# LANL-Bioinformatics/PCRamp

Measured on AMD Instinct MI355X. Metric: primer-pair x target amplification evals/sec, higher is better.
Workload: dtype u32

## Files before the change

pcramp_amd/csrc/pcr_device.hip:

```cpp
#include <hip/hip_runtime.h>
#include <cstring>
#include <rocprim/device/device_radix_sort.hpp>

#include <stdint.h>
#include <string.h>
#include <math.h>
#include <stdlib.h>
#include <string>
#include <vector>
#include <chrono>
#include <algorithm>
#include <unordered_map>
#include <type_traits>
#include <thread>
#include <mutex>
#include <condition_variable>
#include <functional>
#include <memory>
#include <atomic>
#include <cassert>
#include <sched.h>
#include <pthread.h>

#include "../../include/pcramp_hip.h"
// ... 450 lines not shown
	const uint32_t n = min(seq_count[seq], cap);
	uint32_t np2 = 1; while(np2 < n) np2 <<= 1;
	for(uint32_t i = tid;i < np2;i += FINBIG_THREADS){
		uint64_t k = ~0ull;
		if(i < n){
			const Hit h = hits[(size_t)seq*cap + i];
			if constexpr (ALL) k = h.key;
			else if(((epoch << 8) | h.cnt) == best[(size_t)seq*ncand + h.cand]) k = h.key;
		}
		fin_keys[i] = k;
	}
	__syncthreads();
	for(uint32_t k = 2;k <= np2;k <<= 1){
		for(uint32_t j = k >> 1;j > 0;j >>= 1){
			for(uint32_t i = tid;i < np2;i += FINBIG_THREADS){
				const uint32_t l = i ^ j;
				if(l > i){
					const uint64_t a = fin_keys[i], b = fin_keys[l];
					const bool up = ((i & k) == 0);
					if((a > b) == up){ fin_keys[i] = b; fin_keys[l] = a; }
				}
			}
			__syncthreads();
		}
	}
	const uint32_t chunk = (np2 + FINBIG_THREADS - 1)/FINBIG_THREADS;
	const uint32_t lo = min(np2, tid*chunk), hi = min(np2, lo + chunk);
	uint32_t cnt = 0;
	for(uint32_t i = lo;i < hi;++i){
		const uint64_t k = fin_keys[i];
		if(k != ~0ull && (i == 0 || fin_keys[i - 1] != k)) ++cnt;
	}
	part[tid] = cnt;
	__syncthreads();
	if(tid == 0){
		uint32_t run = 0;
		for(int t = 0;t < FINBIG_THREADS;++t){ const uint32_t c = part[t]; part[t] = run; run += c; }
		seg_hi[seq] = seq*cap + run;
	}
	__syncthreads();
	uint32_t rank = part[tid];
	for(uint32_t i = lo;i < hi;++i){
		const uint64_t k = fin_keys[i];
		if(k != ~0ull && (i == 0 || fin_keys[i - 1] != k)){
			DevEntry e;
			materialise_entry(k, planes, blk_off, irr, irr_off, e);
			db[(size_t)seq*cap + rank] = e;
			++rank;
		}
	}
}

#include "pcr_screen.inc"

#include "pcr_sw.inc"
#include "pcr_thermo.inc"

constexpr uint32_t N_TOUCHED_UNKNOWN = 0xFFFFFFFFu;
constexpr uint32_t EPOCH_LIMIT = (1u << 24) - 1;

struct SeqSet {
	uint32_t n = 0;
	std::vector<std::vector<uint8_t> > packed;
	std::vector<uint64_t> len, blk_off, nblk_real;
	std::vector<float> weight; DevBuf<float> d_weight; bool weight_dirty = true;
	std::vector<uint8_t> active;
	std::vector<std::vector<pcrhost::IrrEntry> > irr_host;
	uint64_t total_blocks = 0;
	uint32_t n_tiles = 0, n_irr = 0;
	bool ctrl_clean = false;
	bool touched_from_seg = false;
	uint32_t bucket_cap = 64;
	DevBuf<uint32_t> irr_perm; uint32_t irr_size_count[256];
	DevBuf<uint4> planes;
	DevBuf<uint32_t> valid, nib, tb, blk_seq, tile_seq, tile_pos0, irr_off, degen_tiles;
	uint32_t *valid_d() const { return valid.p + S2_VALID_FRONT; }
	uint32_t *tb_d() const { return tb.p + S2_TB_FRONT; }
	DevBuf<uint8_t> tile_degen; uint32_t n_degen_tiles = 0;
	DevBuf<TileDesc> tile_desc;
	DevBuf<uint64_t> d_len, d_blk_off, d_nblk_real;
	DevBuf<uint8_t> d_active;
	std::vector<uint8_t> has_eos; DevBuf<uint8_t> d_has_eos;
	DevBuf<IrrDev> irr;
	DevBuf<IrrScan> irr_scan;
	DevBuf<uint32_t> irx_first, irx_last, irx_words, irx_sums; bool irx_valid = false, irx_usable = false;
	uint32_t irr_n_multi = 0;
	DevBuf<uint32_t> pix_first, pix_last, pix_sums, blk_info, blk_local, blk_tile0; DevBuf<uint4> pix_ent; std::vector<uint32_t> pix_start_h; uint64_t pix_generation = 0; bool pix_valid = false, pix_usable = false;
	DevBuf<uint8_t> codes; DevBuf<uint64_t> d_code_off; bool have_codes = false;
	bool have_db = false;
	uint32_t n_entries = 0;
	uint32_t db_cap = 0;
	uint64_t n_slots = 0;
	DevBuf<DevEntry> db;
	DevBuf<uint32_t> touched;
	DevBuf<uint32_t> ctrl;
	uint32_t n_touched = 0;
	bool touched_built = false;
	uint32_t *d_seg_hi = nullptr;
};

}

struct HostPool {
	std::vector<std::thread> th;
	std::mutex m; std::condition_variable cv_go, cv_done;
	std::function<void(unsigned)> fn; unsigned n_parts = 0, next = 0, pending = 0; uint64_t gen = 0; bool stop = false;
	explicit HostPool(unsigned n_workers){ for(unsigned i = 0;i < n_workers;++i) th.emplace_back([this]{ work(); }); }
	~HostPool(){ { std::lock_guard<std::mutex> lk(m); stop = true; } cv_go.notify_all(); for(std::thread &t : th) t.join(); }
	unsigned size() const { return (unsigned)th.size(); }
	void work()
	{
		uint64_t seen = 0;
		std::unique_lock<std::mutex> lk(m);
		while(true){
			cv_go.wait(lk, [&]{ return stop || gen != seen; });
			if(stop) return;
			seen = gen;
			while(next < n_parts){ const unsigned p = next++; lk.unlock(); fn(p); lk.lock(); }
			if(--pending == 0) cv_done.notify_one();
		}
	}
	void run(unsigned parts, std::function<void(unsigned)> f)
	{
		std::unique_lock<std::mutex> lk(m);
		fn = std::move(f); n_parts = parts; next = 0; pending = (unsigned)th.size(); ++gen;
		cv_go.notify_all();
		while(next < n_parts){ const unsigned p = next++; lk.unlock(); fn(p); lk.lock(); }
		cv_done.wait(lk, [&]{ return pending == 0; });
	}
};

namespace { struct PassJob; struct Launcher; }

struct pcr_ctx {
	int device = 0;
	std::unique_ptr<HostPool> pool_;
	HostPool &host_pool()
	{
		if(!pool_){ const unsigned hw = std::max(1u, std::thread::hardware_concurrency()); pool_.reset(new HostPool(std::min(hw, 16u) - 1u)); }
		return *pool_;
	}
	Stream stream;
	Stream aux_stream;
	std::string design_text;
	DevBuf<uint64_t> split_where;
	pcr_params params;
	pcrhost::PackFilter filt;
	SeqSet sets[PCR_N_SETS];
	DevBuf<uint32_t> best, counters, mask, status;
	int scan_version = 3;
	bool force_seed1 = false;
	struct S2Key { uint32_t a, c, g, t, floor_; bool operator==(const S2Key &o) const { return a == o.a && c == o.c && g == o.g && t == o.t && floor_ == o.floor_; } };
	struct S2KeyHash { size_t operator()(const S2Key &k) const { uint64_t h = 0x9E3779B97F4A7C15ull; for(uint32_t v : {k.a, k.c, k.g, k.t, k.floor_}){ h ^= v; h *= 0x100000001B3ull; h ^= h >> 29; } return (size_t)h; } };
	struct S2Entry { std::vector<uint32_t> seeds;  uint32_t off_mask; bool seedable; uint4 mask;  };
	std::unordered_map<S2Key, S2Entry, S2KeyHash> s2_cache;
	std::vector<pcrhost::Seed> s2_tmp;
	static constexpr int S3_CHUNK_SETS = 4;
	struct S3Chunks { uint64_t gen = 0; uint32_t total = 0; std::vector<uint32_t> run; };
	struct S3Entry : S2Entry { std::vector<uint8_t> spans;  S3Chunks chunks[S3_CHUNK_SETS]; uint32_t next_slot = 0; };
	std::unordered_map<S2Key, S3Entry, S2KeyHash> s3_cache;
	std::vector<pcrhost::FoldSeed> s3_tmp;
	struct S3Launch { Seed3Slices W; uint32_t n_chunks, per_wg, slice_cap, n_irr_wg; };
	bool no_seed3 = false, s3_attr_set = false;
	bool s3_next = true;
	bool s2_attr_set = false; uint32_t s2_dbg = 0; bool no_irr_index = false;
	std::unordered_map<S2Key, S2Entry, S2KeyHash> s1_cache;
	DevBuf<uint32_t> s1_image, s1_heads, s1_multi, s1_part;
	bool host_seed_tables = false;
	DevBuf<Hit> hits;
	DevBuf<uint64_t> bits_fr, bits_rf;
	DevBuf<OligoDev> oligos;
	DevBuf<SwJob> sw_jobs; DevBuf<SwOut> sw_out; DevBuf<uint8_t> sw_q, sw_qlen, sw_t, entry_codes, entry_lens;
	DevBuf<AmpRec> amp_recs, amp_recs2; DevBuf<BgPairDev> bg_pairs;
	DevBuf<uint64_t> amp_keys; DevBuf<uint32_t> amp_pkeys, amp_pair_start; DevBuf<uint8_t> sort_tmp;
	DevBuf<thermo::Job> th_jobs; DevBuf<thermo::JobOut> th_out; DevBuf<int> th_dg; DevBuf<uint2> th_map; DevBuf<uint32_t> th_bad;
	float th_dg_salt = -1.0f;
	DevBuf<unsigned long long> th_dbg; bool th_attr_set = false;
	std::vector<thermo::Job> th_host_jobs; std::vector<thermo::JobOut> th_host_res;
	MappedBuf<uint8_t> sw_pin; Event sw_done[2];
	DevBuf<pcr_amplicon> mx_amp;
	DevBuf<OligoDev> opt_oligos; DevBuf<uint2> opt_jobs; DevBuf<float> opt_cov; DevBuf<uint32_t> opt_loc, opt_tasks;
	DevBuf<Planes> mx_keys; uint32_t mx_n_keys = 0; DevBuf<uint32_t> mx_count;
	DevBuf<uint8_t> pool_in, pool_tmp; DevBuf<uint32_t> pool_cnt, pool_ord; DevBuf<uint64_t> pool_eoff, pool_ioff, pool_keys; DevBuf<uint2> pool_items; DevBuf<pcr_product> pool_rec;
	DevBuf<uint8_t> site_in, site_tmp; DevBuf<uint32_t> site_cnt, site_ord, site_flag; DevBuf<uint64_t> site_eoff, site_joff, site_keys; DevBuf<uint2> site_items; DevBuf<float4> site_res; DevBuf<pcr_site> site_rec;
	bool site_attr_set = false;
	pcr_comm *shard_comm = nullptr; uint64_t shard_first = 0, shard_n_total = 0; int shard_mode = 0;
	DevBuf<uint64_t> sh_rec, sh_full; DevBuf<uint8_t> sh_stage;
	std::vector<uint64_t> shard_bounds; DevBuf<uint64_t> d_shard_bounds;
	bool design_ready = false; DevBuf<uint64_t> sh_bits;
	std::vector<std::vector<uint8_t> > samp_packed; std::vector<uint64_t> samp_len;
	void drop_shard(){ shard_comm = nullptr; shard_mode = 0; shard_bounds.clear(); design_ready = false; samp_packed.clear(); samp_len.clear(); }
	pcr_comm *trial_comm = nullptr;
	size_t amp_cap = size_t(1) << 20;
	uint32_t n_cu = 256;
	DevBuf<uint64_t> fin_scratch;
	std::vector<uint16_t> seed_count; std::vector<uint8_t> seed_fill, seed_own;
	uint32_t epoch = 0;
	uint32_t debug_epoch = 0;
	bool opt_pm_global = false;
	uint32_t opt_dbg_wg_tasks = 0, opt_dbg_task_cap = 0;
	uint64_t best_seen = 0;
	static constexpr int STAGE_RING = 4;
	struct StageSlot { MappedBuf<uint8_t> buf; Event done; bool busy = false;
	                   uint32_t guard_seq = 0;  };
	StageSlot stage[STAGE_RING]; int stage_next = 0;
	struct DirectSlot { DevBuf<uint8_t> buf{true}; uint32_t guard_seq = 0; };
	DirectSlot dstage[STAGE_RING]; int dstage_next = 0;
	bool direct_ok = false;
	typedef PassMail Mail;
	static constexpr uint32_t MAIL_RING = 8;
	MappedBuf<Mail> mail;
	uint32_t mail_seq = 0;
	MappedBuf<uint8_t> ret;
	MappedBuf<uint8_t> in;
	MappedBuf<uint32_t> ret_flag; uint32_t ret_seq = 0;
	struct Pending {
		uint32_t seq; int which; std::vector<pcr_pair> pairs; int opt5, opt3; float thr; uint32_t min_len;
		pcr_amplify_args args; uint64_t *d_fr, *d_rf;
	};
	std::vector<Pending> pending;
	bool launch_thread = true;
	Launcher *launcher = nullptr; pcrq::Client lq_client; uint64_t n_pipelined = 0;
	std::mutex job_m; std::vector<PassJob *> job_free, job_all;
	DevBuf<uint8_t> arena;
	const uint4 *d_cand_fwd = nullptr, *d_cand_rc = nullptr; const uint32_t *d_cand_floor = nullptr;
	const OligoDev *d_oligos = nullptr;
	bool debug_log = false;
	bool timing = false; double t_host[8] = {0, 0, 0, 0, 0, 0, 0, 0}; uint64_t n_timed = 0;
	bool prof = false; uint32_t prof_stride = 1, prof_pass = 0;
	std::vector<std::pair<Event, Event> > prof_events;
	double prof_ms = 0.0; uint64_t prof_launches = 0;
	std::vector<std::pair<Event, Event> > prof_events_k[PCR_PROF_KERNELS];
	double prof_ms_k[PCR_PROF_KERNELS] = {0.0, 0.0, 0.0}; uint64_t prof_launches_k[PCR_PROF_KERNELS] = {0, 0, 0};
};

namespace {

int drain(pcr_ctx *ctx);
int flush_launcher(pcr_ctx *ctx);
void detach_launcher(pcr_ctx *ctx);
void free_jobs(pcr_ctx *ctx);

struct ProfScope {
	pcr_ctx *ctx; int k; Event e0, e1;
	ProfScope(pcr_ctx *c, int kernel, bool on = true) : ctx(c), k(kernel)
	{
		if(!on || !ctx->prof || k < 0 || k >= PCR_PROF_KERNELS) return;
		if(e0.create() != hipSuccess || e1.create() != hipSuccess){ e0.release(); return; }
		(void)hipEventRecord(e0, ctx->stream);
	}
	void finish()
	{
		if(!e0) return;
		(void)hipEventRecord(e1, ctx->stream);
		((k == PCR_PROF_SCAN) ? ctx->prof_events : ctx->prof_events_k[k]).emplace_back(std::move(e0), std::move(e1));
	}
	~ProfScope() { finish(); }
};
constexpr int PCR_SET_SCRATCH = 3;
inline bool set_ok(pcr_set which) { return (unsigned)which <= (unsigned)PCR_SET_MULTIPLEX; }
#define CHECK_SET(which) do{ if(!set_ok(which)){ g_err = "unknown sequence set (PCR_SET_TARGET, PCR_SET_BACKGROUND or PCR_SET_MULTIPLEX)"; return PCR_ERR_ARG; } }while(0)
#define FLUSH(ctx) do{ if((ctx)->launcher){ const int frc_ = flush_launcher(ctx); if(frc_ != PCR_OK) return frc_; } }while(0)
#define DRAIN(ctx) do{ FLUSH(ctx); if(!(ctx)->pending.empty()){ const int drc_ = drain(ctx); if(drc_ != PCR_OK) return drc_; } }while(0)

struct HostTimer {
	pcr_ctx *ctx; int slot; std::chrono::steady_clock::time_point t0;
	HostTimer(pcr_ctx *c, int s) : ctx(c), slot(s) { if(ctx->timing) t0 = std::chrono::steady_clock::now(); }
	void next(int s)
	{
		if(!ctx->timing) return;
		const auto t1 = std::chrono::steady_clock::now();
		ctx->t_host[slot] += std::chrono::duration<double, std::micro>(t1 - t0).count();
		slot = s; t0 = t1;
	}
	~HostTimer() { next(slot); }
};

__global__ void k_apply_splits(const uint64_t *__restrict__ where, uint32_t n, uint32_t *__restrict__ planes , uint32_t *__restrict__ nib)
{
	const uint32_t i = blockIdx.x*blockDim.x + threadIdx.x;
	if(i >= n) return;
	const uint64_t gb = where[2*(size_t)i];
	const uint32_t bit = (uint32_t)where[2*(size_t)i + 1];
	const uint32_t m = ~(1u << bit);
	for(int k = 0;k < 4;++k) atomicAnd(&planes[gb*4 + k], m);
	atomicAnd(&nib[gb*4 + (bit >> 3)], ~(0xFu << ((bit & 7u)*4u)));
}

int upload_irregular(pcr_ctx *ctx, SeqSet &S)
{
	const auto tu0 = std::chrono::steady_clock::now();
	auto ms_since = [&](){ return std::chrono::duration<double, std::milli>(std::chrono::steady_clock::now() - tu0).count(); };
	double t_flat = 0, t_sort = 0, t_scan = 0, t_copy1 = 0;
	size_t total = 0;
	for(uint32_t s = 0;s < S.n;++s) total += S.irr_host[s].size();
	std::vector<IrrDev> flat(total);
	std::vector<uint32_t> off(S.n + 1, 0);
	for(int k = 0;k < 256;++k) S.irr_size_count[k] = 0;
	{
		size_t at = 0;
		for(uint32_t s = 0;s < S.n;++s){
			off[s] = (uint32_t)at;
			const std::vector<pcrhost::IrrEntry> &v = S.irr_host[s];
			for(size_t k = 0;k < v.size();++k){
				const pcrhost::IrrEntry &e = v[k];
				IrrDev &d = flat[at++];
				d.w = e.w; d.loc = e.loc; d.seq = s;
				d.meta = (uint32_t)e.strand | ((uint32_t)e.cws << 8) | ((uint32_t)e.ord << 16);
				d.local_id = (uint32_t)k;
				++S.irr_size_count[e.cws & 0xFF];
			}
		}
	}
	off[S.n] = (uint32_t)flat.size();
	S.n_irr = (uint32_t)flat.size();
	t_flat = ms_since();
	std::vector<uint32_t> perm(flat.size());
	t_sort = ms_since();
	int rc;
	{
		auto spread = [](uint64_t v) -> uint64_t {
			v = (v | (v << 16)) & 0x0000FFFF0000FFFFull; v = (v | (v << 8)) & 0x00FF00FF00FF00FFull; v = (v | (v << 4)) & 0x0F0F0F0F0F0F0F0Full;
			v = (v | (v << 2)) & 0x3333333333333333ull; v = (v | (v << 1)) & 0x5555555555555555ull; return v;
		};
		uint32_t start[256];
		uint32_t run = 0;
		for(int k = 255;k >= 0;--k){ start[k] = run; run += S.irr_size_count[k]; }
		std::vector<IrrScan> scan(perm.size());
		uint32_t n_multi = 0;
		for(size_t i = 0;i < flat.size();++i){
			const IrrDev &d = flat[i];
			const uint32_t at = start[(d.meta >> 8) & 0xFF]++;
			perm[at] = (uint32_t)i;
			const uint32_t multi = (d.w.a & d.w.c) | (d.w.a & d.w.g) | (d.w.a & d.w.t) | (d.w.c & d.w.g) | (d.w.c & d.w.t) | (d.w.g & d.w.t);
			if(multi) ++n_multi;
			const uint32_t lo = d.w.c | d.w.t, hi = d.w.g | d.w.t;
			const uint64_t code = spread(lo) | (spread(hi) << 1);
			IrrScan r; r.w0 = (uint32_t)code; r.w1 = (uint32_t)(code >> 32); r.idx_flags = (uint32_t)i | (multi ? 0x80000000u : 0u); r.seq = d.seq;
			scan[at] = r;
		}
		S.irr_n_multi = n_multi; S.irx_valid = false;
		t_scan = ms_since();
		if((rc = S.irr_scan.ensure_slack(scan.size() + 1)) != PCR_OK) return rc;
		if(!scan.empty()) HIP_TRY(hipMemcpy(S.irr_scan.p, scan.data(), scan.size()*sizeof(IrrScan), hipMemcpyHostToDevice));
	}
	t_copy1 = ms_since();
	if((rc = S.irr_perm.ensure_slack(perm.size() + 1)) != PCR_OK) return rc;
	if(!perm.empty()) HIP_TRY(hipMemcpyAsync(S.irr_perm.p, perm.data(), perm.size()*sizeof(uint32_t), hipMemcpyHostToDevice, ctx->stream));
	if((rc = S.irr.ensure_slack(flat.size())) != PCR_OK) return rc;
	if((rc = S.irr_off.ensure(off.size())) != PCR_OK) return rc;
	if(!flat.empty()) HIP_TRY(hipMemcpyAsync(S.irr.p, flat.data(), flat.size()*sizeof(IrrDev), hipMemcpyHostToDevice, ctx->stream));
	HIP_TRY(hipMemcpyAsync(S.irr_off.p, off.data(), off.size()*sizeof(uint32_t), hipMemcpyHostToDevice, ctx->stream));
	HIP_TRY(hipStreamSynchronize(ctx->stream));
	if(ctx->timing && flat.size() > 100000) fprintf(stderr, "[pcramp] irregular list of %zu words: flat %.1f  order %.1f  scan records %.1f  first copy %.1f  other copies %.1f ms\n", flat.size(), t_flat, t_sort - t_flat, t_scan - t_sort, t_copy1 - t_scan, ms_since() - t_copy1);
	return PCR_OK;
}

void launch_exclusive_scan(pcr_ctx *ctx, uint32_t *counts, uint32_t *starts, uint32_t n, uint32_t *sums)
{
	const uint32_t n_blocks = (n + 4095u)/4096u;
	hipLaunchKernelGGL(k_scan_blocks, dim3(n_blocks), dim3(1024), 0, ctx->stream, counts, starts, n, sums);
	hipLaunchKernelGGL(k_scan_sums, dim3(1), dim3(1024), 0, ctx->stream, sums, n_blocks);
	hipLaunchKernelGGL(k_scan_add, dim3(n_blocks), dim3(1024), 0, ctx->stream, starts, counts, n, sums);
}

constexpr uint32_t IRX_MAX_RUN = 1024;
int ensure_irr_index(pcr_ctx *ctx, SeqSet &S)
{
	if(S.irx_valid) return PCR_OK;
	int rc;
	if((rc = S.irx_first.ensure(IRX_KEYS + 4)) != PCR_OK) return rc;
	if((rc = S.irx_last.ensure(IRX_KEYS + 4)) != PCR_OK) return rc;
	if((rc = S.irx_words.ensure_slack((size_t)24*S.n_irr + 4)) != PCR_OK) return rc;
	const uint32_t n_blocks = (IRX_KEYS + 4095u)/4096u;
	if((rc = S.irx_sums.ensure(n_blocks + 4)) != PCR_OK) return rc;
	HIP_TRY(hipMemsetAsync(S.irx_last.p, 0, (size_t)IRX_KEYS*sizeof(uint32_t), ctx->stream));
	if(S.n_irr){
		hipLaunchKernelGGL(k_irx_count, dim3((S.n_irr + 255)/256), dim3(256), 0, ctx->stream, S.irr.p, S.n_irr, S.irx_last.p);
		HIP_TRY(hipGetLastError());
	}
	{
// ... 26 lines not shown
	const uint32_t n_blocks = (PIX_KEYS + 4095u)/4096u;
	if((rc = S.pix_sums.ensure(n_blocks + 4)) != PCR_OK) return rc;
	if((rc = S.pix_ent.ensure(S.total_blocks*32 + 64)) != PCR_OK) return rc;
	{
		if(S.n >= (1u << 30)){ return PCR_OK; }
		if((rc = S.blk_info.ensure(S.total_blocks + 1)) != PCR_OK) return rc;
		if((rc = S.blk_local.ensure(S.total_blocks + 1)) != PCR_OK) return rc;
		std::vector<uint32_t> tile0((size_t)S.n + 1);
		uint64_t t0 = 0;
		for(uint32_t q = 0;q < S.n;++q){ tile0[q] = (uint32_t)t0; t0 += (S.len[q] >= 32) ? (S.len[q] - 7 + TILE_POS - 1)/TILE_POS : 0; }
		tile0[S.n] = (uint32_t)t0;
		if(t0 >= (uint64_t(1) << 32)) return PCR_OK;
		if((rc = S.blk_tile0.ensure((size_t)S.n + 1)) != PCR_OK) return rc;
		HIP_TRY(hipMemcpyAsync(S.blk_tile0.p, tile0.data(), ((size_t)S.n + 1)*sizeof(uint32_t), hipMemcpyHostToDevice, ctx->stream));
		hipLaunchKernelGGL(k_blk_info, dim3((unsigned)((S.total_blocks + 255)/256)), dim3(256), 0, ctx->stream, S.blk_seq.p, S.d_blk_off.p, S.d_len.p,
			S.blk_tile0.p, S.tile_degen.p, S.d_active.p, S.total_blocks, S.blk_info.p, S.blk_local.p);
		HIP_TRY(hipGetLastError());
		HIP_TRY(hipStreamSynchronize(ctx->stream));
	}
	HIP_TRY(hipMemsetAsync(S.pix_last.p, 0, (size_t)PIX_KEYS*sizeof(uint32_t), ctx->stream));
	const unsigned grid = (unsigned)((S.total_blocks + 255)/256);
	hipLaunchKernelGGL(k_pix_build<false>, dim3(grid), dim3(256), 0, ctx->stream, S.tb_d(), S.blk_seq.p, S.d_blk_off.p, S.d_len.p, S.total_blocks, S.pix_last.p, (uint4 *)nullptr);
	launch_exclusive_scan(ctx, S.pix_last.p, S.pix_first.p, PIX_KEYS, S.pix_sums.p);
	hipLaunchKernelGGL(k_pix_build<true>, dim3(grid), dim3(256), 0, ctx->stream, S.tb_d(), S.blk_seq.p, S.d_blk_off.p, S.d_len.p, S.total_blocks, S.pix_last.p, S.pix_ent.p);
	HIP_TRY(hipGetLastError());
	{
		S.pix_start_h.resize((size_t)PIX_KEYS + 1);
		HIP_TRY(hipMemcpyAsync(S.pix_start_h.data(), S.pix_first.p, (size_t)PIX_KEYS*sizeof(uint32_t), hipMemcpyDeviceToHost, ctx->stream));
		HIP_TRY(hipMemcpyAsync(S.pix_start_h.data() + PIX_KEYS, S.pix_last.p + (PIX_KEYS - 1), sizeof(uint32_t), hipMemcpyDeviceToHost, ctx->stream));
		HIP_TRY(hipStreamSynchronize(ctx->stream));
		static uint64_t generations = 0;
		S.pix_generation = ++generations;
	}
	S.pix_usable = true;
	return PCR_OK;
}

int run_valid(pcr_ctx *ctx, SeqSet &S, uint64_t first_block, uint64_t n_blocks)
{
	if(n_blocks == 0) return PCR_OK;
	const unsigned threads = 256;
	const unsigned grid = (unsigned)((n_blocks + threads - 1)/threads);
	hipLaunchKernelGGL(k_valid, dim3(grid), dim3(threads), 0, ctx->stream, S.planes.p, S.d_blk_off.p, S.blk_seq.p,
		S.d_nblk_real.p, S.valid_d(), S.total_blocks, ctx->filt.max_degen, ctx->filt.gc_ok, first_block, n_blocks);
	HIP_TRY(hipGetLastError());
	return PCR_OK;
}

int build_tile_desc(pcr_ctx *ctx, SeqSet &S)
{
	if(S.n_tiles == 0) return PCR_OK;
	int rc = S.tile_desc.ensure(S.n_tiles);
	if(rc != PCR_OK) return rc;
	hipLaunchKernelGGL(k_tile_desc, dim3((S.n_tiles + 255)/256), dim3(256), 0, ctx->stream, S.d_blk_off.p, S.d_len.p, S.d_active.p, S.tile_seq.p,
		S.tile_pos0.p, S.tile_degen.p, S.n_tiles, S.tile_desc.p);
	HIP_TRY(hipGetLastError());
	return PCR_OK;
}

void fill_oligo_planes(OligoDev &o, const Planes &m, float thr2)
{
	o.m = m;
	const unsigned size = (unsigned)pcrhost::planes_size(o.m);
	o.floor2 = (unsigned)((float)size*thr2);
	o.norm = (size > 0) ? (float)(1.0/size) : 0.0f;
	o.start = pcrhost::planes_start(o.m);
	o.stop = pcrhost::planes_stop(o.m);
	o.p1 = (o.stop >= 1) ? pcrhost::planes_nibble(o.m, o.stop - 1) : 0;
	o.p2 = (o.stop >= 0) ? pcrhost::planes_nibble(o.m, o.stop) : 0;
}

void fill_oligo(OligoDev &o, const uint64_t w[2], float thr2) { fill_oligo_planes(o, pcrhost::planes_of_word(w), thr2); }

__global__ void k_stage(const uint4 *__restrict__ src, uint4 *__restrict__ dst, uint32_t n16,
	uint4 *__restrict__ z0, uint32_t n0, uint4 *__restrict__ z1, uint32_t n1, uint4 *__restrict__ z2, uint32_t n2)
{
	const uint32_t i = blockIdx.x*blockDim.x + threadIdx.x, stride = gridDim.x*blockDim.x;
	for(uint32_t k = i;k < n16;k += stride) dst[k] = src[k];
	const uint4 zero = make_uint4(0, 0, 0, 0);
	for(uint32_t k = i;k < n0;k += stride) z0[k] = zero;
	for(uint32_t k = i;k < n1;k += stride) z1[k] = zero;
	for(uint32_t k = i;k < n2;k += stride) z2[k] = zero;
}

enum SpinEnd { SPIN_SEEN, SPIN_IDLE, SPIN_ERROR };
template<class Seen> inline SpinEnd spin_until(hipStream_t stream, Seen seen, hipError_t &err)
{
	for(uint64_t spins = 1;!seen();++spins){
		__builtin_ia32_pause();
		if((spins & 0x3FFF) == 0){
			err = hipStreamQuery(stream);
			if(err == hipSuccess) return SPIN_IDLE;
			if(err != hipErrorNotReady) return SPIN_ERROR;
		}
	}
	return SPIN_SEEN;
}

int wait_published(pcr_ctx *ctx, uint32_t seq)
{
	const PassMail *const slot = ctx->mail.host + (seq % pcr_ctx::MAIL_RING);
	hipError_t e = hipSuccess;
	const SpinEnd end = spin_until(ctx->stream, [&]{
		const uint32_t v = __atomic_load_n((const uint32_t *)&slot->seq, __ATOMIC_ACQUIRE);
		return v >= seq && (v - seq) % pcr_ctx::MAIL_RING == 0; }, e);
	if(end == SPIN_ERROR){ g_err = std::string("device pass failed: ") + hipGetErrorString(e); return PCR_ERR_DEVICE; }
	return PCR_OK;
}

struct Stager {
	pcr_ctx *ctx; size_t used = 0; bool direct = false;
	explicit Stager(pcr_ctx *c) : ctx(c) {}
	pcr_ctx::StageSlot *slot = nullptr; pcr_ctx::DirectSlot *dslot = nullptr;
	uint8_t *host = nullptr, *dev = nullptr;
	int begin_direct(size_t bytes)
	{
		direct = true;
		dslot = &ctx->dstage[ctx->dstage_next];
		ctx->dstage_next = (ctx->dstage_next + 1) % pcr_ctx::STAGE_RING;
		if(dslot->guard_seq){ const int grc = wait_published(ctx, dslot->guard_seq); if(grc != PCR_OK) return grc; dslot->guard_seq = 0; }
		if(bytes + 256 > dslot->buf.cap){
			if(dslot->buf.p) HIP_TRY(hipStreamSynchronize(ctx->stream));
			const int rc = dslot->buf.ensure(std::max<size_t>((bytes + 256)*2, 1 << 17));
			if(rc != PCR_OK) return rc;
		}
		host = dev = dslot->buf.p;
		used = 0;
		return PCR_OK;
	}
	void seal(uint32_t pass_seq)
	{
		__builtin_ia32_sfence();
		dslot->guard_seq = pass_seq + 1;
	}
	int begin(size_t bytes)
	{
		slot = &ctx->stage[ctx->stage_next];
		ctx->stage_next = (ctx->stage_next + 1) % pcr_ctx::STAGE_RING;
		if(slot->busy){ HIP_TRY(hipEventSynchronize(slot->done)); slot->busy = false; }
		if(slot->guard_seq){ const int grc = wait_published(ctx, slot->guard_seq); if(grc != PCR_OK) return grc; slot->guard_seq = 0; }
		int rc = slot->buf.ensure(bytes, std::max<size_t>(bytes*2, 1 << 16));
		if(rc != PCR_OK) return rc;
		host = slot->buf.host; dev = slot->buf.dev;
		if(!slot->done) HIP_TRY(slot->done.create(hipEventDisableTiming));
		rc = ctx->arena.ensure(bytes + 256);
		used = 0;
		return rc;
	}
	template<class T> T *put(const T *src, size_t n)
	{
		used = (used + 15) & ~size_t(15);
		memcpy(host + used, src, n*sizeof(T));
		T *at = (T *)((direct ? dev : ctx->arena.p) + used);
		used += n*sizeof(T);
		return at;
	}
	int ship(void *z0 = nullptr, size_t bytes0 = 0, void *z1 = nullptr, size_t bytes1 = 0, void *z2 = nullptr, size_t bytes2 = 0, uint32_t guard_seq = 0)
	{
		const uint32_t n16 = (uint32_t)((used + 15)/16), n0 = (uint32_t)((bytes0 + 15)/16), n1 = (uint32_t)((bytes1 + 15)/16), n2 = (uint32_t)((bytes2 + 15)/16);
		const uint32_t most = std::max(std::max(n16, n2), std::max(n0, n1));
		if(most){
			const unsigned grid = std::min<unsigned>((most + 255)/256, 512u);
			hipLaunchKernelGGL(k_stage, dim3(grid), dim3(256), 0, ctx->stream, (const uint4 *)dev, (uint4 *)ctx->arena.p, n16,
				(uint4 *)z0, n0, (uint4 *)z1, n1, (uint4 *)z2, n2);
			HIP_TRY(hipGetLastError());
		}
		if(guard_seq) slot->guard_seq = guard_seq;
		else{
			HIP_TRY(hipEventRecord(slot->done, ctx->stream));
			slot->busy = true;
		}
		return PCR_OK;
	}
};

__global__ void k_publish(const uint32_t *__restrict__ counters, pcr_ctx::Mail *mail, uint32_t seq)
{
	if(threadIdx.x < 4) mail->counters[threadIdx.x] = counters[threadIdx.x];
	__threadfence_system();
	__syncthreads();
	if(threadIdx.x == 0) __hip_atomic_store((uint32_t *)&mail->seq, seq, __ATOMIC_RELEASE, __HIP_MEMORY_SCOPE_SYSTEM);
}

int mail_wait(pcr_ctx *ctx, uint32_t seq, uint32_t out[4])
{
	pcr_ctx::Mail *const slot = ctx->mail.host + (seq % pcr_ctx::MAIL_RING);
	auto seen = [&]{ return __atomic_load_n((const uint32_t *)&slot->seq, __ATOMIC_ACQUIRE) == seq; };
	hipError_t e = hipSuccess;
	const SpinEnd end = spin_until(ctx->stream, seen, e);
	if(end == SPIN_ERROR){ g_err = std::string("device pass failed: ") + hipGetErrorString(e); return PCR_ERR_DEVICE; }
	if(end == SPIN_IDLE && !seen()){ g_err = "device pass finished without publishing its counters"; return PCR_ERR_DEVICE; }
	for(int i = 0;i < 4;++i) out[i] = slot->counters[i];
	return PCR_OK;
}

__global__ void k_return(const uint4 *__restrict__ s0, uint32_t n0, const uint4 *__restrict__ s1, uint32_t n1,
	const uint4 *__restrict__ s2, uint32_t n2, uint4 *__restrict__ dst)
{
	const uint32_t stride = gridDim.x*blockDim.x, t = blockIdx.x*blockDim.x + threadIdx.x;
	for(uint32_t i = t;i < n0;i += stride) dst[i] = s0[i];
	for(uint32_t i = t;i < n1;i += stride) dst[n0 + i] = s1[i];
	for(uint32_t i = t;i < n2;i += stride) dst[n0 + n1 + i] = s2[i];
}

__global__ void k_return_flag(uint32_t *flag, uint32_t seq)
{
	__threadfence_system();
	__hip_atomic_store(flag, seq, __ATOMIC_RELEASE, __HIP_MEMORY_SCOPE_SYSTEM);
}

int return_to_host(pcr_ctx *ctx, const void *s0, size_t b0, const void *s1, size_t b1, const void *s2, size_t b2, const uint8_t *out[3])
{
	const uint32_t n0 = (uint32_t)((b0 + 15)/16), n1 = (uint32_t)((b1 + 15)/16), n2 = (uint32_t)((b2 + 15)/16);
	const size_t need = ((size_t)n0 + n1 + n2)*16;
	int rc;
	if(!ctx->ret_flag.host){
		if((rc = ctx->ret_flag.ensure(64)) != PCR_OK) return rc;
		*ctx->ret_flag.host = 0;
	}
	if(need > ctx->ret.cap){
		HIP_TRY(hipStreamSynchronize(ctx->stream));
		if((rc = ctx->ret.ensure(need, std::max<size_t>(need*2, 1 << 20))) != PCR_OK) return rc;
	}
	const uint32_t most = std::max(n0, std::max(n1, n2));
	if(most){
		const unsigned grid = std::min<unsigned>((most + 255)/256, 1024u);
		hipLaunchKernelGGL(k_return, dim3(grid), dim3(256), 0, ctx->stream, (const uint4 *)s0, n0, (const uint4 *)s1, n1, (const uint4 *)s2, n2, (uint4 *)ctx->ret.dev);
		HIP_TRY(hipGetLastError());
	}
	const uint32_t seq = ++ctx->ret_seq;
	hipLaunchKernelGGL(k_return_flag, dim3(1), dim3(1), 0, ctx->stream, ctx->ret_flag.dev, seq);
	HIP_TRY(hipGetLastError());
	auto seen = [&]{ return __atomic_load_n((const uint32_t *)ctx->ret_flag.host, __ATOMIC_ACQUIRE) == seq; };
	hipError_t e = hipSuccess;
	const SpinEnd end = spin_until(ctx->stream, seen, e);
	if(end == SPIN_ERROR){ g_err = std::string("device work failed: ") + hipGetErrorString(e); return PCR_ERR_DEVICE; }
	if(end == SPIN_IDLE && !seen()){ g_err = "device work finished without raising the return flag"; return PCR_ERR_DEVICE; }
	out[0] = ctx->ret.host; out[1] = ctx->ret.host + (size_t)n0*16; out[2] = ctx->ret.host + ((size_t)n0 + n1)*16;
	return PCR_OK;
}

int mapped_input(pcr_ctx *ctx, const void *src, size_t bytes, const void **dev_out)
{
	if(bytes > ctx->in.cap){
		HIP_TRY(hipStreamSynchronize(ctx->stream));
		const int rc = ctx->in.ensure(bytes, std::max<size_t>(bytes*2, 1 << 18));
		if(rc != PCR_OK) return rc;
	}
	memcpy(ctx->in.host, src, bytes);
	*dev_out = ctx->in.dev;
	return PCR_OK;
}

struct FusedAmp {
	const pcr_pair *pairs; uint32_t n_pairs; const pcr_amplify_args *a; uint64_t *d_fr, *d_rf;
	bool staged = false; const OligoDev *d_oligos = nullptr; uint32_t pub_seq = 0; const uint32_t *pub_counters = nullptr;
	bool posted = false;
};

void build_oligos(const pcr_pair *pairs, uint32_t n_pairs, const pcr_amplify_args *a, std::vector<OligoDev> &ol)
{
	const float thr2 = a->collect_threshold*a->collect_threshold;
	ol.resize(2*(size_t)n_pairs);
	for(uint32_t i = 0;i < n_pairs;++i){
		fill_oligo(ol[2*i], pairs[i].f.w, thr2);
		fill_oligo(ol[2*i + 1], pairs[i].r.w, thr2);
	}
}

int ensure_touched(pcr_ctx *ctx, SeqSet &S)
{
	if(S.touched_built || !S.have_db || !S.ctrl.p) return PCR_OK;
	if(S.touched_from_seg) hipLaunchKernelGGL(k_touched_seg, dim3((S.n + 255)/256), dim3(256), 0, ctx->stream, S.d_seg_hi, S.n, S.ctrl.p, S.touched.p);
	else hipLaunchKernelGGL(k_touched, dim3((S.n + 255)/256), dim3(256), 0, ctx->stream, S.ctrl.p + 8, S.n, S.ctrl.p, S.touched.p);
	HIP_TRY(hipGetLastError());
	uint32_t n = 0;
	HIP_TRY(hipMemcpyAsync(&n, S.ctrl.p + 3, sizeof(uint32_t), hipMemcpyDeviceToHost, ctx->stream));
	HIP_TRY(hipStreamSynchronize(ctx->stream));
	S.n_touched = n; S.n_entries = n ? 1 : 0; S.touched_built = true;
	return PCR_OK;
}

int amplify_launch(pcr_ctx *ctx, SeqSet &S, const pcr_pair *pairs, uint32_t n_pairs, const pcr_amplify_args *a,
	uint64_t *d_fr, uint64_t *d_rf, const FusedAmp *fa = nullptr)
{
	{ const int erc = ensure_touched(ctx, S); if(erc != PCR_OK) return erc; }
	if(!S.have_db){ g_err = "pcr_amplify: no word DB (call pcr_select_words first)"; return PCR_ERR_STATE; }
	const uint64_t words = (S.n + 63)/64;
	const size_t bits_bytes = (size_t)n_pairs*words*sizeof(uint64_t);
	if(S.n_entries == 0 || n_pairs == 0){
		if(bits_bytes){
			HIP_TRY(hipMemsetAsync(d_fr, 0, bits_bytes, ctx->stream));
			HIP_TRY(hipMemsetAsync(d_rf, 0, bits_bytes, ctx->stream));
		}
		return PCR_OK;
	}
	HostTimer timer(ctx, 4);
	int rc;
	const bool prestaged = fa && fa->staged;
	if(prestaged) ctx->d_oligos = fa->d_oligos;
	else{
		std::vector<OligoDev> ol;
		build_oligos(pairs, n_pairs, a, ol);
		Stager st(ctx);
		if((rc = st.begin(ol.size()*sizeof(OligoDev) + 64)) != PCR_OK) return rc;
		ctx->d_oligos = st.put(ol.data(), ol.size());
// ... 28 lines not shown

template<int NSLOT, int KLO>
int launch_scan2_nw(pcr_ctx *ctx, SeqSet &S, uint32_t nw, uint32_t group0, uint32_t n_groups, uint32_t gw, uint32_t ncand, const HitSink &sink,
	const uint32_t *d_tab, const uint32_t *d_bias, const uint32_t *tile_ids, uint32_t n_tiles, const uint32_t *orient_ids)
{
#define SCAN2_ARGS S.nib.p, S.planes.p, S.valid_d(), S.d_blk_off.p, S.d_len.p, S.d_active.p, S.tile_seq.p, S.tile_pos0.p, \
	d_tab, d_bias, group0, gw, tile_ids, orient_ids, ctx->d_cand_fwd, ctx->d_cand_rc, ctx->d_cand_floor, ncand, sink
	const dim3 grid(n_tiles, n_groups), block(SCAN2_THREADS);
	switch(nw){
		case 1: hipLaunchKernelGGL((k_scan2<1, NSLOT, KLO>), grid, block, 0, ctx->stream, SCAN2_ARGS); break;
		case 2: hipLaunchKernelGGL((k_scan2<2, NSLOT, KLO>), grid, block, 0, ctx->stream, SCAN2_ARGS); break;
		case 3: hipLaunchKernelGGL((k_scan2<3, NSLOT, KLO>), grid, block, 0, ctx->stream, SCAN2_ARGS); break;
		case 4: hipLaunchKernelGGL((k_scan2<4, NSLOT, KLO>), grid, block, 0, ctx->stream, SCAN2_ARGS); break;
		case 5: hipLaunchKernelGGL((k_scan2<5, NSLOT, KLO>), grid, block, 0, ctx->stream, SCAN2_ARGS); break;
		case 6: hipLaunchKernelGGL((k_scan2<6, NSLOT, KLO>), grid, block, 0, ctx->stream, SCAN2_ARGS); break;
		case 7: hipLaunchKernelGGL((k_scan2<7, NSLOT, KLO>), grid, block, 0, ctx->stream, SCAN2_ARGS); break;
		default: hipLaunchKernelGGL((k_scan2<8, NSLOT, KLO>), grid, block, 0, ctx->stream, SCAN2_ARGS); break;
	}
#undef SCAN2_ARGS
	HIP_TRY(hipGetLastError());
	return PCR_OK;
}

int launch_scan2(pcr_ctx *ctx, SeqSet &S, const Scan2Tables &T, uint32_t ncand, const HitSink &sink,
	const uint32_t *d_tab, const uint32_t *d_bias, const uint32_t *tile_ids, uint32_t n_tiles, const uint32_t *orient_ids)
{
	if(n_tiles == 0 || T.n_groups == 0) return PCR_OK;
	const uint32_t full = (T.last_words == T.gw) ? T.n_groups : T.n_groups - 1;
	int rc = PCR_OK;
	if(full){
		rc = (T.nslot == 26) ? launch_scan2_nw<26, 3>(ctx, S, T.gw, 0, full, T.gw, ncand, sink, d_tab, d_bias, tile_ids, n_tiles, orient_ids)
			: launch_scan2_nw<32, 0>(ctx, S, T.gw, 0, full, T.gw, ncand, sink, d_tab, d_bias, tile_ids, n_tiles, orient_ids);
		if(rc != PCR_OK) return rc;
	}
	if(full < T.n_groups){
		rc = (T.nslot == 26) ? launch_scan2_nw<26, 3>(ctx, S, T.last_words, full, 1, T.gw, ncand, sink, d_tab, d_bias, tile_ids, n_tiles, orient_ids)
			: launch_scan2_nw<32, 0>(ctx, S, T.last_words, full, 1, T.gw, ncand, sink, d_tab, d_bias, tile_ids, n_tiles, orient_ids);
	}
	return rc;
}

int count_entries(pcr_ctx *ctx, SeqSet &S)
{
	uint64_t total = 0;
	if(S.n_touched){
		std::vector<uint32_t> hi(S.n);
		HIP_TRY(hipMemcpyAsync(hi.data(), S.d_seg_hi, S.n*sizeof(uint32_t), hipMemcpyDeviceToHost, ctx->stream));
		HIP_TRY(hipStreamSynchronize(ctx->stream));
		for(uint32_t q = 0;q < S.n;++q){ if(hi[q]) total += hi[q] - (uint64_t)q*S.db_cap; }
	}
	S.n_entries = (uint32_t)total;
	return PCR_OK;
}

}

extern "C" {

const char *pcr_last_error(void) { return g_err.c_str(); }

pcr_ctx *pcr_create(int device, void *hip_stream, const pcr_params *params)
{
	int count = 0;
	if(hipGetDeviceCount(&count) != hipSuccess || count <= 0){
		g_err = "pcr_create: no HIP device available (this library has no CPU fallback)";
		return nullptr;
	}
	if(device < 0 || device >= count){ g_err = "pcr_create: bad device index"; return nullptr; }
	if(hipSetDevice(device) != hipSuccess){ g_err = "pcr_create: hipSetDevice failed"; return nullptr; }
	hipDeviceProp_t prop;
	if(hipGetDeviceProperties(&prop, device) != hipSuccess){ g_err = "pcr_create: hipGetDeviceProperties failed"; return nullptr; }
	if(std::string(prop.gcnArchName).find("gfx950") == std::string::npos){
		g_err = std::string("pcr_create: device is ") + prop.gcnArchName + ", this build targets gfx950 only";
		return nullptr;
	}
	pcr_ctx *ctx = new pcr_ctx();
	ctx->device = device;
	if(hip_stream) ctx->stream.borrow((hipStream_t)hip_stream);
	else if(ctx->stream.create() != hipSuccess){ g_err = "pcr_create: hipStreamCreate failed"; delete ctx; return nullptr; }
	if(params){ ctx->params = *params; }
	else{ ctx->params.pack_max_degen = 256; ctx->params.pack_min_gc = 0.0f; ctx->params.pack_max_gc = 1.0f; }
	{ hipDeviceProp_t prop; if(hipGetDeviceProperties(&prop, device) == hipSuccess && prop.multiProcessorCount > 0) ctx->n_cu = (uint32_t)prop.multiProcessorCount; }
	if(const char *v = getenv("PCRAMP_TIMING")) ctx->timing = v[0] == '1';
	ctx->debug_log = getenv("PCRAMP_DEBUG") != nullptr;
	if(const char *v = getenv("PCRAMP_DEBUG_EPOCH")) ctx->debug_epoch = (uint32_t)strtoul(v, nullptr, 0);
	if(const char *v = getenv("PCRAMP_OPT_PM")) ctx->opt_pm_global = v[0] == 'g';
	if(const char *v = getenv("PCRAMP_DEBUG_OPT_TASKS")){ unsigned a = 0, b = 0; if(sscanf(v, "%u,%u", &a, &b) >= 1){ ctx->opt_dbg_wg_tasks = a; ctx->opt_dbg_task_cap = b; } }
	if(const char *v = getenv("PCRAMP_SEED")) ctx->force_seed1 = v[0] == '1';
	if(const char *v = getenv("PCRAMP_SEED_TABLES")) ctx->host_seed_tables = v[0] == 'h';
	if(const char *v = getenv("PCRAMP_S2DBG")) ctx->s2_dbg = (uint32_t)atoi(v);
	if(const char *v = getenv("PCRAMP_IRR_INDEX")) ctx->no_irr_index = v[0] == '0';
	if(const char *v = getenv("PCRAMP_SEED3")) ctx->no_seed3 = v[0] == '0';
	if(const char *v = getenv("PCRAMP_S3_NEXT")) ctx->s3_next = v[0] != '0';
	if(const char *v = getenv("PCRAMP_LAUNCH_THREAD")) ctx->launch_thread = v[0] != '0';
	if(const char *v = getenv("PCRAMP_SCAN")){ if(v[0] == '1') ctx->scan_version = 1; else if(v[0] == '2') ctx->scan_version = 2; }
	{
		const char *v = getenv("PCRAMP_STAGE");
		if(!(v && v[0] == 'k') && prop.isLargeBar){
			DevBuf<uint32_t> probe(true); MappedBuf<uint32_t> back; const std::string err_before = g_err;
			constexpr uint32_t PROBE_WORDS = 1024;
			if(probe.ensure(PROBE_WORDS) == PCR_OK && back.ensure(PROBE_WORDS*sizeof(uint32_t)) == PCR_OK){
				hipPointerAttribute_t at;
				bool ok = hipPointerGetAttributes(&at, probe.p) == hipSuccess;
				for(int round = 0;ok && round < 2;++round){
					volatile uint32_t *w = (volatile uint32_t *)probe.p;
					for(uint32_t i = 0;i < PROBE_WORDS;++i){ w[i] = 0x9E3779B9u*(i + 1) + (uint32_t)round; back.host[i] = 0; }
					__builtin_ia32_sfence();
					hipLaunchKernelGGL(k_stage, dim3(1), dim3(256), 0, ctx->stream, (const uint4 *)probe.p, (uint4 *)back.dev, PROBE_WORDS/4,
						(uint4 *)nullptr, 0u, (uint4 *)nullptr, 0u, (uint4 *)nullptr, 0u);
					ok = hipGetLastError() == hipSuccess && hipStreamSynchronize(ctx->stream) == hipSuccess;
					for(uint32_t i = 0;ok && i < PROBE_WORDS;++i) ok = back.host[i] == 0x9E3779B9u*(i + 1) + (uint32_t)round;
				}
				ctx->direct_ok = ok;
			}
			else{ (void)hipGetLastError(); g_err = err_before; }
		}
	}
	ctx->filt.max_degen = ctx->params.pack_max_degen;
	ctx->filt.set_gc(ctx->params.pack_min_gc, ctx->params.pack_max_gc);
	if(hipMemcpyToSymbol(HIP_SYMBOL(c_taq_mama), h_taq_mama, sizeof(h_taq_mama)) != hipSuccess ||
	   hipMemcpyToSymbol(HIP_SYMBOL(thermo::c_H), PCR_NN_H, sizeof(PCR_NN_H)) != hipSuccess ||
	   hipMemcpyToSymbol(HIP_SYMBOL(thermo::c_S), PCR_NN_S, sizeof(PCR_NN_S)) != hipSuccess ||
	   hipMemcpyToSymbol(HIP_SYMBOL(thermo::c_loop_S), PCR_LOOP_S, sizeof(PCR_LOOP_S)) != hipSuccess ||
	   hipMemcpyToSymbol(HIP_SYMBOL(thermo::c_bulge_S), PCR_BULGE_S, sizeof(PCR_BULGE_S)) != hipSuccess ||
	   hipMemcpyToSymbol(HIP_SYMBOL(thermo::c_hairpin_S), PCR_HAIRPIN_S, sizeof(PCR_HAIRPIN_S)) != hipSuccess ||
	   hipMemcpyToSymbol(HIP_SYMBOL(thermo::c_special_H), PCR_SPECIAL_H, sizeof(PCR_SPECIAL_H)) != hipSuccess ||
	   hipMemcpyToSymbol(HIP_SYMBOL(thermo::c_special_S), PCR_SPECIAL_S, sizeof(PCR_SPECIAL_S)) != hipSuccess ||
	   hipMemcpyToSymbol(HIP_SYMBOL(thermo::c_special_key), PCR_SPECIAL_KEY, sizeof(PCR_SPECIAL_KEY)) != hipSuccess ||
	   hipMemcpyToSymbol(HIP_SYMBOL(thermo::c_wc), PCR_WC, sizeof(PCR_WC)) != hipSuccess){
		g_err = "pcr_create: hipMemcpyToSymbol failed"; delete ctx; return nullptr;
	}
	if(ctx->mail.ensure(sizeof(pcr_ctx::Mail)*pcr_ctx::MAIL_RING) != PCR_OK){ g_err = "pcr_create: mapped host allocation failed"; delete ctx; return nullptr; }
	memset((void *)ctx->mail.host, 0, sizeof(pcr_ctx::Mail)*pcr_ctx::MAIL_RING);
	return ctx;
}

void pcr_destroy(pcr_ctx *ctx)
{
	if(!ctx) return;
	(void)hipSetDevice(ctx->device);
	(void)flush_launcher(ctx);
	detach_launcher(ctx);
	(void)hipStreamSynchronize(ctx->stream);
	if(ctx->aux_stream) (void)hipStreamSynchronize(ctx->aux_stream);
	ctx->pending.clear();
	free_jobs(ctx);
	if(ctx->timing && ctx->n_timed){
		const double n = (double)ctx->n_timed;
		fprintf(stderr, "[pcramp] host us/pass by stage: A (plan, caller's thread) %.1f  B (stage + launch, %s) %.1f  (%llu of %llu passes pipelined, queue depth <= %u)\n",
			ctx->t_host[0]/n, ctx->n_pipelined ? "launcher thread" : "caller's thread", (ctx->t_host[1] + ctx->t_host[2])/n,
			(unsigned long long)ctx->n_pipelined, (unsigned long long)ctx->n_timed, ctx->lq_client.max_depth);
		fprintf(stderr, "[pcramp] host us/pass: plan %.1f  stage %.1f  launch %.1f  wait %.1f | amplify prep %.1f  launch %.1f  (%llu passes)\n",
			ctx->t_host[0]/n, ctx->t_host[1]/n, ctx->t_host[2]/n, ctx->t_host[3]/n, ctx->t_host[4]/n, ctx->t_host[5]/n, (unsigned long long)ctx->n_timed);
	}
	delete ctx;
}

uint32_t pcr_num_sequences(pcr_ctx *ctx, pcr_set which) { return (ctx && set_ok(which)) ? ctx->sets[which].n : 0; }
uint64_t pcr_bitset_words(pcr_ctx *ctx, pcr_set which) { return (ctx && set_ok(which)) ? (ctx->sets[which].n + 63)/64 : 0; }

int pcr_staging_mode(pcr_ctx *ctx) { return (ctx && ctx->direct_ok) ? 1 : 0; }

int pcr_launcher_stats(pcr_ctx *ctx, uint64_t *passes_pipelined, uint32_t *max_queue_depth)
{
	if(!ctx){ g_err = "null ctx"; return PCR_ERR_ARG; }
	if(passes_pipelined) *passes_pipelined = ctx->n_pipelined;
	if(max_queue_depth) *max_queue_depth = ctx->lq_client.max_depth;
	return PCR_OK;
}

int pcr_live_resources(uint64_t out[4])
{
	if(!out){ g_err = "pcr_live_resources: bad argument"; return PCR_ERR_ARG; }
	for(int k = 0;k < 4;++k) out[k] = pcrown::g_live[k].load();
	return PCR_OK;
}

int pcr_synchronize(pcr_ctx *ctx)
{
	if(!ctx){ g_err = "null ctx"; return PCR_ERR_ARG; }
	HIP_TRY(hipSetDevice(ctx->device));
	DRAIN(ctx);
	HIP_TRY(hipStreamSynchronize(ctx->stream));
	return PCR_OK;
}

static int load_sequences_impl(pcr_ctx *ctx, int which, const uint8_t *packed4, const uint64_t *byte_offsets,
	const uint64_t *lengths, const float *weights, uint32_t n);

int pcr_load_sequences(pcr_ctx *ctx, pcr_set which, const uint8_t *packed4, const uint64_t *byte_offsets,
	const uint64_t *lengths, const float *weights, uint32_t n)
{
	if(!set_ok(which)){ g_err = "pcr_load_sequences: unknown sequence set"; return PCR_ERR_ARG; }
	return load_sequences_impl(ctx, (int)which, packed4, byte_offsets, lengths, weights, n);
}

static int load_sequences_impl(pcr_ctx *ctx, int which, const uint8_t *packed4, const uint64_t *byte_offsets,
	const uint64_t *lengths, const float *weights, uint32_t n)
{
	if(!ctx || which < 0 || which >= PCR_N_SETS || (n && (!packed4 || !byte_offsets || !lengths))){
		g_err = "pcr_load_sequences: bad argument"; return PCR_ERR_ARG;
	}
	DRAIN(ctx);
	if(n >= (1u << 24)){ g_err = "pcr_load_sequences: at most 2^24-1 sequences per GPU shard"; return PCR_ERR_CAPACITY; }
	HIP_TRY(hipSetDevice(ctx->device));
	HIP_TRY(hipStreamSynchronize(ctx->stream));
	SeqSet &S = ctx->sets[which];
	S.have_db = false; S.n_entries = 0; S.have_codes = false;
	S.n = n;
	S.packed.assign(n, std::vector<uint8_t>());
	S.len.assign(lengths, lengths + n);
	if(which == PCR_SET_TARGET) ctx->drop_shard();
	if(which == PCR_SET_TARGET || which == PCR_SET_BACKGROUND) ctx->trial_comm = nullptr;
	S.weight.assign(n, 1.0f);
	if(weights) S.weight.assign(weights, weights + n);
	S.weight_dirty = true;
	S.ctrl_clean = false; S.touched_from_seg = false;
	S.active.assign(n, 1);
	S.has_eos.assign(n, 0);
	S.blk_off.assign(n + 1, 0);
	S.nblk_real.assign(n, 0);
	S.irr_host.assign(n, std::vector<pcrhost::IrrEntry>());
	uint64_t total_bytes = 0, total_blocks = 0, n_tiles = 0;
	std::vector<uint64_t> dev_byte_off(n);
	for(uint32_t s = 0;s < n;++s){
		if(lengths[s] >= (uint64_t(1) << 31)){ g_err = "pcr_load_sequences: sequence longer than 2^31-1 bases"; return PCR_ERR_CAPACITY; }
		const uint64_t nb = (lengths[s] + 1)/2;
		S.packed[s].assign(packed4 + byte_offsets[s], packed4 + byte_offsets[s] + nb);
		if((lengths[s] & 1) && nb) S.packed[s][nb - 1] &= 0xF0;
		{
			const std::vector<uint8_t> &b = S.packed[s];
			bool eos = false;
			const uint64_t full = lengths[s]/2;
			for(uint64_t k = 0;k < full && !eos;++k) eos = ((b[k] & 0xF0) == 0) || ((b[k] & 0x0F) == 0);
			if(!eos && (lengths[s] & 1)) eos = ((b[full] & 0xF0) == 0);
			S.has_eos[s] = eos ? 1 : 0;
		}
		dev_byte_off[s] = total_bytes;
		total_bytes += nb;
		S.blk_off[s] = total_blocks;
		S.nblk_real[s] = (lengths[s] + 31)/32;
		total_blocks += S.nblk_real[s] + 2;
		if(lengths[s] >= 32) n_tiles += (lengths[s] - 7 + TILE_POS - 1)/TILE_POS;
	}
	S.blk_off[n] = total_blocks;
	S.total_blocks = total_blocks;
	if(n_tiles >= (uint64_t(1) << 31)){ g_err = "pcr_load_sequences: too many tiles"; return PCR_ERR_CAPACITY; }
	S.n_tiles = (uint32_t)n_tiles;

	std::vector<uint32_t> blk_seq(total_blocks), tile_seq(n_tiles), tile_pos0(n_tiles);
	uint64_t t = 0;
	S.pix_valid = false; S.pix_usable = false;
	for(uint32_t s = 0;s < n;++s){
		for(uint64_t b = S.blk_off[s];b < S.blk_off[s + 1];++b) blk_seq[b] = s;
		if(lengths[s] >= 32){
			const uint64_t nt = (lengths[s] - 7 + TILE_POS - 1)/TILE_POS;
			for(uint64_t k = 0;k < nt;++k, ++t){ tile_seq[t] = s; tile_pos0[t] = (uint32_t)(k*TILE_POS); }
		}
		pcrhost::PackedSeq q; q.buf = S.packed[s].data(); q.len = lengths[s];
		if(!pcrhost::irregular_words(q, ctx->filt, S.irr_host[s])){
			g_err = "pcr_load_sequences: more than 64 irregular words share one (loc, strand)"; return PCR_ERR_CAPACITY;
		}
	}

	int rc;
	DevBuf<uint8_t> d_packed; DevBuf<uint64_t> d_byte_off;
	if((rc = d_packed.ensure(total_bytes)) != PCR_OK) return rc;
	if((rc = d_byte_off.ensure(n)) != PCR_OK) return rc;
	if((rc = S.planes.ensure(total_blocks)) != PCR_OK) return rc;
	if((rc = S.valid.ensure(S2_VALID_FRONT + total_blocks + S2_TAIL_BLOCKS)) != PCR_OK) return rc;
	if((rc = S.nib.ensure(total_blocks*4 + 8)) != PCR_OK) return rc;
	if((rc = S.tb.ensure(S2_TB_FRONT + (total_blocks + S2_TAIL_BLOCKS)*2 + 8)) != PCR_OK) return rc;
	if((rc = S.tile_degen.ensure(n_tiles + 1)) != PCR_OK) return rc;
	if((rc = S.degen_tiles.ensure(n_tiles + 1)) != PCR_OK) return rc;
	if((rc = S.blk_seq.ensure(total_blocks)) != PCR_OK) return rc;
	if((rc = S.tile_seq.ensure(n_tiles)) != PCR_OK) return rc;
	if((rc = S.tile_pos0.ensure(n_tiles)) != PCR_OK) return rc;
	if((rc = S.d_len.ensure(n)) != PCR_OK) return rc;
	if((rc = S.d_blk_off.ensure(n + 1)) != PCR_OK) return rc;
	if((rc = S.d_nblk_real.ensure(n)) != PCR_OK) return rc;
	if((rc = S.d_active.ensure(n)) != PCR_OK) return rc;
	if((rc = S.d_has_eos.ensure(n)) != PCR_OK) return rc;
#define H2D(dst, src, bytes) do{ if((bytes) > 0){ hipError_t e_ = hipMemcpy(dst, src, bytes, hipMemcpyHostToDevice); \
	if(e_ != hipSuccess){ g_err = std::string("hipMemcpy: ") + hipGetErrorString(e_); return PCR_ERR_DEVICE; } } }while(0)
	{
		std::vector<uint8_t> flat(total_bytes);
		for(uint32_t s = 0;s < n;++s){ if(!S.packed[s].empty()) memcpy(flat.data() + dev_byte_off[s], S.packed[s].data(), S.packed[s].size()); }
		H2D(d_packed.p, flat.data(), flat.size());
	}
	H2D(d_byte_off.p, dev_byte_off.data(), n*sizeof(uint64_t));
	H2D(S.blk_seq.p, blk_seq.data(), total_blocks*sizeof(uint32_t));
	H2D(S.tile_seq.p, tile_seq.data(), n_tiles*sizeof(uint32_t));
	H2D(S.tile_pos0.p, tile_pos0.data(), n_tiles*sizeof(uint32_t));
	H2D(S.d_len.p, S.len.data(), n*sizeof(uint64_t));
	H2D(S.d_blk_off.p, S.blk_off.data(), (n + 1)*sizeof(uint64_t));
	H2D(S.d_nblk_real.p, S.nblk_real.data(), n*sizeof(uint64_t));
	H2D(S.d_active.p, S.active.data(), n);
	H2D(S.d_has_eos.p, S.has_eos.data(), n);
#undef H2D
	{
		hipError_t e_ = hipMemsetAsync(S.valid.p, 0, S2_VALID_FRONT*sizeof(uint32_t), ctx->stream);
		if(e_ == hipSuccess) e_ = hipMemsetAsync(S.valid_d() + total_blocks, 0, S2_TAIL_BLOCKS*sizeof(uint32_t), ctx->stream);
		if(e_ == hipSuccess) e_ = hipMemsetAsync(S.tb.p, 0, S2_TB_FRONT*sizeof(uint32_t), ctx->stream);
		if(e_ == hipSuccess) e_ = hipMemsetAsync(S.tb_d() + total_blocks*2, 0, (S2_TAIL_BLOCKS*2 + 8)*sizeof(uint32_t), ctx->stream);
		if(e_ != hipSuccess){ g_err = std::string("load: padding memset: ") + hipGetErrorString(e_); return PCR_ERR_DEVICE; }
	}
// ... 434 lines not shown
```

pcramp_amd/csrc/pcr_host.hpp:

```cpp
#ifndef PCR_HOST_HPP
#define PCR_HOST_HPP

#include <stdint.h>
#include <algorithm>
#include <deque>
#include <vector>

namespace pcrhost {

struct Planes {
	uint32_t a, c, g, t;
};

inline uint32_t bitrev32(uint32_t v)
{
	v = ((v >> 1) & 0x55555555u) | ((v & 0x55555555u) << 1);
	v = ((v >> 2) & 0x33333333u) | ((v & 0x33333333u) << 2);
	v = ((v >> 4) & 0x0F0F0F0Fu) | ((v & 0x0F0F0F0Fu) << 4);
	v = ((v >> 8) & 0x00FF00FFu) | ((v & 0x00FF00FFu) << 8);
	return (v >> 16) | (v << 16);
}

inline unsigned word_get(const uint64_t w[2], int k) { return (unsigned)(w[k >> 4] >> ((15 - (k & 15))*4)) & 0xF; }

inline void word_set(uint64_t w[2], int k, unsigned v)
{
	const int sh = (15 - (k & 15))*4;
	w[k >> 4] = (w[k >> 4] & ~(uint64_t(0xF) << sh)) | (uint64_t(v) << sh);
}

inline uint32_t gather_every_4th(uint64_t x)
{
	x &= 0x1111111111111111ull;
	x = (x | (x >> 3)) & 0x0303030303030303ull;
	x = (x | (x >> 6)) & 0x000F000F000F000Full;
	x = (x | (x >> 12)) & 0x000000FF000000FFull;
	return (uint32_t)((x | (x >> 24)) & 0xFFFFu);
}

inline Planes planes_of_word(const uint64_t w[2])
{
	uint64_t r[2];
	for(int h = 0;h < 2;++h){
		const uint64_t b = __builtin_bswap64(w[h]);
		r[h] = ((b >> 4) & 0x0F0F0F0F0F0F0F0Full) | ((b & 0x0F0F0F0F0F0F0F0Full) << 4);
	}
	Planes p;
	p.a = gather_every_4th(r[0]) | (gather_every_4th(r[1]) << 16);
	p.c = gather_every_4th(r[0] >> 1) | (gather_every_4th(r[1] >> 1) << 16);
	p.g = gather_every_4th(r[0] >> 2) | (gather_every_4th(r[1] >> 2) << 16);
	p.t = gather_every_4th(r[0] >> 3) | (gather_every_4th(r[1] >> 3) << 16);
	return p;
}

inline void word_of_planes(const Planes &p, uint64_t w[2])
{
	w[0] = w[1] = 0;
	for(int k = 0;k < 32;++k){
		const unsigned v = ((p.a >> k) & 1) | (((p.c >> k) & 1) << 1) | (((p.g >> k) & 1) << 2) | (((p.t >> k) & 1) << 3);
		word_set(w, k, v);
	}
}

inline Planes planes_revcomp(const Planes &p)
{
	Planes r;
	r.a = bitrev32(p.t);
	r.t = bitrev32(p.a);
	r.c = bitrev32(p.g);
	r.g = bitrev32(p.c);
	return r;
}

inline uint32_t planes_occupied(const Planes &p) { return p.a | p.c | p.g | p.t; }
inline int planes_size(const Planes &p) { return __builtin_popcount(planes_occupied(p)); }
inline int planes_start(const Planes &p) { const uint32_t o = planes_occupied(p); return o ? __builtin_ctz(o) : 32; }
inline int planes_stop(const Planes &p) { const uint32_t o = planes_occupied(p); return o ? 31 - __builtin_clz(o) : -1; }

inline unsigned planes_nibble(const Planes &p, int k)
{
	return ((p.a >> k) & 1) | (((p.c >> k) & 1) << 1) | (((p.g >> k) & 1) << 2) | (((p.t >> k) & 1) << 3);
}

inline Planes planes_shift_left(const Planes &p) { Planes r = {p.a >> 1, p.c >> 1, p.g >> 1, p.t >> 1}; return r; }
inline Planes planes_shift_right(const Planes &p) { Planes r = {p.a << 1, p.c << 1, p.g << 1, p.t << 1}; return r; }

struct PackFilter {
	uint32_t max_degen;
	uint64_t gc_ok;
	bool gc_on;

	void set_gc(float min_gc, float max_gc)
	{
		gc_on = (min_gc > 0.0f) || (max_gc < 1.0f);
		gc_ok = 0;
		const float norm = 1.0f/32;
		for(unsigned n = 0;n <= 32;++n){
			const float f = n*norm;
			const bool skip = gc_on && ((f < min_gc) || (f > max_gc));
			if(!skip){ gc_ok |= (uint64_t(1) << n); }
		}
	}
};

inline bool degeneracy_exceeds(unsigned n2, unsigned n3, unsigned n4, uint32_t thr)
{
	const unsigned e = n2 + 2*n4;
	if(e >= 33){ return true; }
	uint64_t p3 = 1;
	for(unsigned i = 0;i < n3;++i){ p3 *= 3; }
	return p3 > (uint64_t(thr) >> e);
}

struct IrrEntry {
	Planes w;
	int32_t loc;
	uint8_t strand;
	uint8_t cws;
	uint8_t ord;
	uint8_t pad;
};

struct PackedSeq {
	const uint8_t *buf;
	uint64_t len;
	unsigned at(uint64_t i) const
	{
		if(i >= len){ return 0; }
		const uint8_t v = buf[i >> 1];
		return (i & 1) ? (v & 0xF) : (v >> 4);
	}
};

class PackMachine {
public:
	PackMachine(const PackFilter &f, std::vector<IrrEntry> &out) : filt(f), dst(out) { reset(); }

	void reset()
	{
		for(int k = 0;k < 32;++k){ s[k] = 0; }
		cws = 0;
		gc.clear();
		num_gc = 0;
	}

	void seed_after_regular(const uint8_t bases[32])
	{
		for(int k = 0;k < 32;++k){ s[k] = bases[k]; }
		cws = 31;
		gc.clear();
		num_gc = 0;
		for(int k = 0;k < 32;++k){ gc.push_back(bases[k]); num_gc += ((bases[k] & 6) != 0); }
	}

	void push(unsigned b, int loc, bool record)
	{
		push_back(b);
		cws += (b != 0);
// ... 390 lines not shown
	}
};

inline bool orientation_seeds(const Planes &m, uint32_t floor_, uint32_t orient, std::vector<Seed> &out, int *max_exact_pos = nullptr, int Q = SEED_Q)
{
	if(max_exact_pos) *max_exact_pos = -1;
	const uint32_t occ = m.a | m.c | m.g | m.t;
	const int size = __builtin_popcount(occ);
	if(size == 0 || floor_ == 0 || floor_ > (uint32_t)size) return floor_ > (uint32_t)size;
	const int k = size - (int)floor_;
	const int first = __builtin_ctz(occ);
	if((occ >> first) != ((size == 32) ? 0xFFFFFFFFu : ((1u << size) - 1u))) return false;
	unsigned slot_set[32];
	for(int j = 0;j < first;++j) slot_set[j] = 0;
	for(int j = first;j < first + size;++j) slot_set[j] = planes_nibble(m, j);
	for(int j = first + size;j < 32;++j) slot_set[j] = 0;

	auto window = [&](int pos, int len, unsigned *sets) -> int {
		const int ws = std::min(pos, 32 - Q);
		for(int j = 0;j < Q;++j){ const int sl = ws + j; sets[j] = (sl >= pos && sl < pos + len) ? slot_set[sl] : 15u; }
		return ws;
	};
	SeedLayout best = { 0, 0, 0, 0 }; bool have = false; unsigned best_codes = 0;
	for(int n2 = 0;3*(n2 - 1) < k + 1;++n2){
		for(int n1 = 0;3*n2 + 2*(n1 - 1) < k + 1;++n1){
			const int n0 = std::max(0, k + 1 - 3*n2 - 2*n1);
			if(n0 + n1 + n2 == 0) continue;
			for(int n1s = 0;n1s <= n1;++n1s){
				const int rest = size - Q*(n1 - n1s) - (Q - 1)*n1s - Q*n2;
				if(rest < 0 || (n0 > 0 && rest/n0 < MIN_SEED_BLOCK)) continue;
				const SeedLayout lay = { n0, n1, n1s, n2 };
				unsigned codes = 0;
				lay.each(first, size, Q, [&](int pos, int len, int budget){
					unsigned sets[SEED_Q_MAX];
					window(pos, len, sets);
					if(codes <= MAX_SEED_CODES) codes += seed_block_codes(sets, Q, budget);
				});
				if(codes > MAX_SEED_CODES) continue;
				if(!have || codes < best_codes){ have = true; best = lay; best_codes = codes; }
			}
		}
	}
	if(!have) return false;
	best.each(first, size, Q, [&](int pos, int len, int budget){
		unsigned sets[SEED_Q_MAX];
		const int ws = window(pos, len, sets);
		seed_emit_block(sets, Q, orient, (uint32_t)ws, budget, out);
		if(len < Q && max_exact_pos) *max_exact_pos = std::max(*max_exact_pos, pos);
	});
	return true;
}

struct FoldSeed { uint32_t code; uint8_t off, lo, hi; };

inline unsigned seed_block_fold_cost(const unsigned *sets, int budget, unsigned &n_seeds)
{
	unsigned d[9], n[3] = { 1, 0, 0 };
	for(int j = 0;j < 9;++j){ d[j] = (unsigned)__builtin_popcount(sets[j]); n[0] *= d[j]; }
	if(n[0] == 0 || sets[9] == 0){ n_seeds = 0; return 0; }
	if(budget >= 1){
		for(int j = 0;j < 9;++j){
			if(d[j] == 4) continue;
			const unsigned cj = n[0]/d[j]*(4 - d[j]);
			n[1] += cj;
			if(budget >= 2){ for(int i = j + 1;i < 9;++i){ if(d[i] < 4) n[2] += cj/d[i]*(4 - d[i]); } }
		}
	}
	const unsigned last = sets[9];
	const unsigned span = (unsigned)(32 - __builtin_clz(last)) - (unsigned)__builtin_ctz(last);
	unsigned cost = 0; n_seeds = 0;
	for(int m = 0;m <= budget;++m){ n_seeds += n[m]; cost += n[m]*((m < budget && last != 15u) ? 4u : span); }
	return cost;
}

inline void fold_seeds(const std::vector<Seed> &q10, std::vector<FoldSeed> &out)
{
	std::vector<uint32_t> key(q10.size());
	for(size_t i = 0;i < q10.size();++i) key[i] = ((uint32_t)q10[i].off << 20) | ((q10[i].code & 0x3FFFFu) << 2) | (q10[i].code >> 18);
	std::sort(key.begin(), key.end());
	for(size_t i = 0;i < key.size();){
		unsigned set = 0; size_t j = i;
		for(;j < key.size() && (key[j] >> 2) == (key[i] >> 2);++j) set |= 1u << (key[j] & 3u);
		FoldSeed f; f.code = (key[i] >> 2) & 0x3FFFFu; f.off = (uint8_t)(key[i] >> 20);
		f.lo = (uint8_t)__builtin_ctz(set); f.hi = (uint8_t)(31 - __builtin_clz(set));
		out.push_back(f);
		i = j;
	}
}

inline bool orientation_fold_seeds(const Planes &m, uint32_t floor_, std::vector<FoldSeed> &out, std::vector<Seed> &tmp, unsigned *cost4 = nullptr)
{
	const int Q = 10;
	if(cost4) *cost4 = 0;
	const uint32_t occ = m.a | m.c | m.g | m.t;
	const int size = __builtin_popcount(occ);
	if(size == 0 || floor_ == 0 || floor_ > (uint32_t)size) return floor_ > (uint32_t)size;
	const int k = size - (int)floor_, first = __builtin_ctz(occ);
	if(size < Q || (occ >> first) != ((size == 32) ? 0xFFFFFFFFu : ((1u << size) - 1u))) return false;
	unsigned slot_set[32];
	for(int j = 0;j < 32;++j) slot_set[j] = (j >= first && j < first + size) ? planes_nibble(m, j) : 0u;
	auto window = [&](int pos, int len, unsigned *sets) -> int {
		const int ws = std::min(pos, 32 - Q);
		for(int j = 0;j < Q;++j){ const int sl = ws + j; sets[j] = (sl >= pos && sl < pos + len) ? slot_set[sl] : 15u; }
		return ws;
	};
	SeedLayout best = { 0, 0, 0, 0 }; bool have = false; unsigned best_cost = 0;
	for(int n2 = 0;3*(n2 - 1) < k + 1;++n2){
		for(int n1 = 0;3*n2 + 2*(n1 - 1) < k + 1;++n1){
			const int n0 = std::max(0, k + 1 - 3*n2 - 2*n1);
			if(n0 + n1 + n2 == 0) continue;
			for(int n1s = 0;n1s <= n1;++n1s){
				const int rest = size - Q*(n1 - n1s) - (Q - 1)*n1s - Q*n2;
				if(rest < 0 || (n0 > 0 && rest/n0 < MIN_SEED_BLOCK)) continue;
				const SeedLayout lay = { n0, n1, n1s, n2 };
				unsigned seeds = 0, cost = 0;
				lay.each(first, size, Q, [&](int pos, int len, int budget){
					unsigned sets[SEED_Q_MAX], ns = 0;
					window(pos, len, sets);
					if(seeds <= MAX_SEED_CODES){ cost += seed_block_fold_cost(sets, budget, ns); seeds += ns; }
				});
				if(seeds > MAX_SEED_CODES) continue;
				if(!have || cost < best_cost){ have = true; best = lay; best_cost = cost; }
			}
		}
	}
	if(!have) return false;
	tmp.clear();
	best.each(first, size, Q, [&](int pos, int len, int budget){
		unsigned sets[SEED_Q_MAX];
		const int ws = window(pos, len, sets);
		seed_emit_block(sets, Q, 0, (uint32_t)ws, budget, tmp);
	});
	fold_seeds(tmp, out);
	if(cost4) *cost4 = best_cost;
	return true;
}

inline bool orientation_index_seeds(const Planes &m, uint32_t floor_, bool fold, std::vector<FoldSeed> &out, std::vector<Seed> &tmp, unsigned *cost4 = nullptr)
{
	tmp.clear();
	if(!orientation_seeds(m, floor_, 0, tmp, nullptr, 9)) return false;
	const size_t at = out.size();
	const unsigned plain_cost = 4u*(unsigned)tmp.size();
	for(const Seed &sd : tmp){ FoldSeed f; f.code = sd.code; f.off = sd.off; f.lo = 0; f.hi = 3; out.push_back(f); }
	if(cost4) *cost4 = plain_cost;
	if(!fold || tmp.empty()) return true;
	std::vector<FoldSeed> folded; unsigned c4 = 0;
	if(orientation_fold_seeds(m, floor_, folded, tmp, &c4) && c4 < plain_cost){
		out.resize(at);
		out.insert(out.end(), folded.begin(), folded.end());
		if(cost4) *cost4 = c4;
	}
	return true;
}

inline bool move_trials(const Planes &cur, int move, double max_degen, int primer_min, int primer_max, std::vector<Planes> &out)
{
	const int first = planes_start(cur), last = planes_stop(cur), len = planes_size(cur);
	auto with_nibble = [](Planes w, int k, unsigned v){
		const uint32_t bit = 1u << k;
		w.a = (w.a & ~bit) | ((v & 1u) ? bit : 0u); w.c = (w.c & ~bit) | ((v & 2u) ? bit : 0u);
		w.g = (w.g & ~bit) | ((v & 4u) ? bit : 0u); w.t = (w.t & ~bit) | ((v & 8u) ? bit : 0u);
		return w;
	};
	switch(move){
		case 0:
			if(planes_degeneracy(cur) >= max_degen) return true;
			for(int i = first;i <= last;++i){
				const unsigned c = planes_nibble(cur, i);
				for(unsigned b = 1;b <= 8;b <<= 1){
					if(c & b) continue;
					const Planes w = with_nibble(cur, i, c | b);
					if(planes_degeneracy(w) > max_degen) continue;
					out.push_back(w);
				}
			}
			return true;
		case 1:
			for(int i = first;i <= last;++i){
				const unsigned c = planes_nibble(cur, i);
				for(unsigned b = 1;b <= 8;b <<= 1){
					const unsigned d = c & ~b;
					if(!d || d == c) continue;
					out.push_back(with_nibble(cur, i, d));
				}
			}
			return true;
		case 2: if(len != primer_min){ out.push_back(first < 32 ? with_nibble(cur, first, 0) : cur); } return true;
		case 3: if(len != primer_min){ out.push_back(last >= 0 ? with_nibble(cur, last, 0) : cur); } return true;
		case 4:
			if(len == primer_max) return true;
			for(unsigned b = 1;b <= 8;b <<= 1) out.push_back(first - 1 >= 0 && first < 32 ? with_nibble(cur, first - 1, b) : cur);
			return true;
		case 5:
			if(len == primer_max) return true;
			for(unsigned b = 1;b <= 8;b <<= 1) out.push_back(last + 1 < 32 ? with_nibble(cur, last + 1, b) : cur);
			return true;
		default: return false;
	}
}

}
#endif
```

pcramp_amd/csrc/pcr_scan_seed3.inc:

```

constexpr uint32_t PIX_CODES = 1u << 18;
constexpr uint32_t PIX_KEYS = PIX_CODES << 2;
constexpr uint32_t S3_BATCH = 8;

template<bool SCATTER>
__global__ void k_pix_build(const uint32_t *__restrict__ tb, const uint32_t *__restrict__ blk_seq, const uint64_t *__restrict__ blk_off,
	const uint64_t *__restrict__ len, uint64_t total_blocks, uint32_t *__restrict__ count_or_cursor, uint4 *__restrict__ ent)
{
	const uint64_t b = (uint64_t)blockIdx.x*blockDim.x + threadIdx.x;
	if(b >= total_blocks) return;
	const uint32_t seq = blk_seq[b];
	const int64_t p0 = (int64_t)(b - blk_off[seq])*32, L = (int64_t)len[seq];
	uint32_t w[8];
#pragma unroll
	for(int k = 0;k < 8;++k) w[k] = tb[(int64_t)2*(int64_t)b - 2 + k];
#pragma unroll
	for(int i = 0;i < 32;++i){
		if(p0 + i + 9 > L) break;
		const uint32_t ten = (i < 16) ? funnel(w[2], w[3], 2*i) : funnel(w[3], w[4], 2*(i - 16));
		const uint32_t code = ((ten & S2_CODE_MASK) << 2) | ((ten >> 18) & 3u);
		if(SCATTER){
			const uint32_t at = atomicAdd(&count_or_cursor[code], 1u);
			const int jl = (i + 9) >> 4, sl = 2*((i + 9) & 15);
			const int jr = (i + 41) >> 4, sr = 2*((i + 41) & 15);
			const uint32_t l_lo = funnel(w[jl], w[jl + 1], sl), l_hi = funnel(w[jl + 1], w[jl + 2], sl) & 0x3FFFu;
			const uint32_t r_lo = funnel(w[jr], w[jr + 1], sr), r_hi = funnel(w[jr + 1], w[jr + 2], sr) & 0x3FFFu;
			ent[at] = make_uint4((uint32_t)(b*32 + (uint64_t)i), l_lo, l_hi | (r_lo << 14), (r_lo >> 18) | (r_hi << 14));
		}
		else atomicAdd(&count_or_cursor[code], 1u);
	}
}

struct Seed3Tables {
	const uint32_t *seeds;
	const uint32_t *chunk_prefix;
	const uint8_t *spans;
	const uint4 *masks; const uint8_t *floors;
	uint32_t n_seeds, n_or, or_base;
	const uint32_t *pix_first, *pix_last; const uint4 *pix_ent;
	uint32_t n_chunks, per_wg, slice_cap;
	uint32_t n_irr_wg;
};
constexpr uint32_t S3_MAX_WG = 512;
constexpr uint32_t S3_MAX_OR = 448, S3_MAX_SEEDS = 1u << 16;
struct Seed3Slices { uint32_t start[S3_MAX_WG + 1]; };
struct Seed3Set {
	const uint32_t *valid, *blk_info, *blk_local; const uint8_t *active;
};
constexpr uint32_t BLK_SEQ_MASK = 0x3FFFFFFFu, BLK_INACTIVE = 0x40000000u, BLK_DEGEN = 0x80000000u;

__global__ void k_blk_info(const uint32_t *__restrict__ blk_seq, const uint64_t *__restrict__ blk_off, const uint64_t *__restrict__ len,
	const uint32_t *__restrict__ tile0, const uint8_t *__restrict__ tile_degen, const uint8_t *__restrict__ active, uint64_t total_blocks,
	uint32_t *__restrict__ blk_info, uint32_t *__restrict__ blk_local)
{
	const uint64_t b = (uint64_t)blockIdx.x*blockDim.x + threadIdx.x;
	if(b >= total_blocks) return;
	const uint32_t q = blk_seq[b];
	const uint64_t bl = b - blk_off[q], tile = bl >> 5;
	const uint32_t nt = tile0[q + 1] - tile0[q];
	const bool degen = tile < nt && tile_degen[tile0[q] + tile];
	blk_info[b] = q | (degen ? 0x80000000u : 0u) | (active[q] ? 0u : 0x40000000u);
	blk_local[b] = (uint32_t)bl;
}

__global__ void k_blk_active(uint32_t *__restrict__ blk_info, const uint32_t *__restrict__ blk_seq, const uint8_t *__restrict__ active, uint64_t total_blocks)
{
	const uint64_t b = (uint64_t)blockIdx.x*blockDim.x + threadIdx.x;
	if(b >= total_blocks) return;
	const uint32_t v = blk_info[b] & ~BLK_INACTIVE;
	blk_info[b] = v | (active[blk_seq[b]] ? 0u : BLK_INACTIVE);
}

__device__ __forceinline__ void s3_irregular(const Seed3Tables &T3, const Seed3Set &Q, const IrrArgs2 &IA, const uint4 *__restrict__ cand_fwd,
	const uint32_t *__restrict__ cand_floor, HitSink sink, uint32_t gw, uint32_t n_gw, uint32_t lane)
{
	for(uint32_t i0 = gw*16u;i0 < T3.n_seeds;i0 += n_gw*16u){
		const uint32_t i = i0 + lane;
		const uint32_t sdv = (lane < 16u && i < T3.n_seeds) ? T3.seeds[i] : S2_END;
		const uint32_t orient = T3.or_base + (sdv & 0x1FFu);
		uint32_t first = 0, cnt = 0;
		if(sdv != S2_END && !(orient & 1u)){
			const uint32_t key = (((sdv >> 9) & 31u) << 18) | (sdv >> 14);
			first = IA.ix_first[key]; cnt = IA.ix_last[key] - first;
		}
		const uint32_t incl = s2_scan(cnt);
		const uint32_t total = s2_rl(incl, 63);
		for(uint32_t t0 = 0;t0 < total;t0 += 64u){
			const uint32_t t = t0 + lane;
			uint32_t lo = 0;
#pragma unroll
			for(uint32_t stp = 32u;stp;stp >>= 1){ if((uint32_t)__shfl((int)incl, (int)(lo + stp - 1u)) <= t) lo += stp; }
			const int sl = (int)min(lo, 63u);
			const uint32_t s_incl = (uint32_t)__shfl((int)incl, sl), s_cnt = (uint32_t)__shfl((int)cnt, sl), s_first = (uint32_t)__shfl((int)first, sl);
			const uint32_t c = (uint32_t)__shfl((int)orient, sl) >> 1;
			if(t >= total) continue;
			const IrrDev e = IA.irr[IA.ix_words[s_first + (t - (s_incl - s_cnt))]];
			if(((e.meta >> 8) & 0xFFu) < IA.min_cws || !Q.active[e.seq]) continue;
			const uint32_t n = match_count(e.w.a, e.w.c, e.w.g, e.w.t, cand_fwd[c]);
			if(n >= cand_floor[c]) record_hit(sink, e.seq, c, make_key(e.seq, e.loc, e.meta & 0xFF, 1, (e.meta >> 16) & 0xFF), n);
		}
	}
}

template<uint32_t S3_THREADS>
__global__ __launch_bounds__(S3_THREADS) __attribute__((amdgpu_waves_per_eu(8, 8))) void k_seed3(Seed3Tables T3, Seed3Set Q, IrrArgs2 IA, const uint4 *__restrict__ cand_fwd, const uint32_t *__restrict__ cand_floor,
	HitSink sink, S2Clear Z, Seed3Slices W)
{
	extern __shared__ uint4 s3_dyn[];
	uint4 *const masks = s3_dyn;
	uint32_t *const prefix = (uint32_t *)(masks + T3.n_or);
	uint32_t *const seeds = prefix + T3.slice_cap;
	uint8_t *const floors = (uint8_t *)(seeds + T3.slice_cap);
	uint8_t *const spans = floors + ((T3.n_or + 15u) & ~15u);
	const uint32_t wave = threadIdx.x >> 6, lane = threadIdx.x & 63u;
	for(uint32_t i = blockIdx.x*S3_THREADS + threadIdx.x;i < Z.n0;i += gridDim.x*S3_THREADS) Z.z0[i] = make_uint4(0, 0, 0, 0);
	for(uint32_t i = blockIdx.x*S3_THREADS + threadIdx.x;i < Z.n1;i += gridDim.x*S3_THREADS) Z.z1[i] = make_uint4(0, 0, 0, 0);
	if(Z.ctrl && blockIdx.x == 0 && threadIdx.x == 0){ Z.ctrl[1] = 0; Z.ctrl[3] = 0; }
	for(uint32_t i = threadIdx.x;i < T3.n_or;i += S3_THREADS){ masks[i] = T3.masks[i]; floors[i] = T3.floors[i]; }
	constexpr uint32_t S3_WAVES = S3_THREADS/64;
	if(blockIdx.x < T3.n_irr_wg){
		if(IA.ix_first) s3_irregular(T3, Q, IA, cand_fwd, cand_floor, sink, blockIdx.x*S3_WAVES + wave, T3.n_irr_wg*S3_WAVES, lane);
		return;
	}
	const uint32_t wg = blockIdx.x - T3.n_irr_wg, n_wg = gridDim.x - T3.n_irr_wg;
	const uint32_t s_lo = W.start[wg];
	const uint32_t n_slice = min(min(W.start[wg + 1] + 2u, T3.n_seeds + 1u) - s_lo, T3.slice_cap);
	for(uint32_t i = threadIdx.x;i < n_slice;i += S3_THREADS){ prefix[i] = T3.chunk_prefix[s_lo + i]; const bool in = s_lo + i < T3.n_seeds; seeds[i] = in ? T3.seeds[s_lo + i] : 0u; spans[i] = in ? T3.spans[s_lo + i] : (uint8_t)0; }
	__syncthreads();
	const uint32_t gw = wg*S3_WAVES + wave, n_gw = n_wg*S3_WAVES;
	const uint32_t q_lo = wg*T3.per_wg, q_hi = min(q_lo + T3.per_wg, T3.n_chunks);
	for(uint32_t q0 = q_lo + wave;q0 < q_hi;q0 += S3_WAVES*S3_BATCH){
		uint32_t c_first = 0, c_cnt = 0, c_sd = 0;
		{
			const uint32_t q = q0 + lane*S3_WAVES;
			if(lane < S3_BATCH && q < q_hi){
				uint32_t lo = 0, hi = n_slice - 1u;
				while(hi - lo > 1u){ const uint32_t mid = (lo + hi) >> 1; if(prefix[mid] <= q) lo = mid; else hi = mid; }
				c_sd = seeds[lo];
				const uint32_t key = (c_sd >> 14) << 2, sp = spans[lo];
				const uint32_t f = T3.pix_first[key + (sp & 3u)], e = T3.pix_last[key + (sp >> 2)], j0 = (q - prefix[lo])*64u;
				c_first = f + j0; c_cnt = (e - f) - j0;
			}
		}
		uint4 en[S3_BATCH];
#pragma unroll
		for(int b = 0;b < (int)S3_BATCH;++b){
			const uint32_t first = s2_rl(c_first, b), cnt = s2_rl(c_cnt, b);
			en[b] = make_uint4(0xFFFFFFFFu, 0, 0, 0);
			if(lane < cnt) en[b] = T3.pix_ent[first + lane];
		}
		uint32_t cnt_b[S3_BATCH], g[S3_BATCH]; bool pass_b[S3_BATCH];
#pragma unroll
		for(int b = 0;b < (int)S3_BATCH;++b){
			const uint32_t sdv = s2_rl(c_sd, b);
			const uint32_t off = (sdv >> 9) & 31u, local = sdv & 0x1FFu, code = sdv >> 14;
			g[b] = en[b].x;
			const uint32_t r_lo = funnel(en[b].z, en[b].w, 14);
			const uint4 cx = make_uint4(en[b].y << 2, (funnel(en[b].y, en[b].z, 30) & 0xFFFFu) | (code << 16), (code >> 16) | (r_lo << 2), en[b].w >> 12);
			const uint32_t in = 24u - off, sh = 2u*(in & 15u);
			const uint32_t a0 = (in < 16u) ? funnel(cx.x, cx.y, sh) : funnel(cx.y, cx.z, sh);
			const uint32_t a1 = (in < 16u) ? funnel(cx.y, cx.z, sh) : funnel(cx.z, cx.w, sh);
			cnt_b[b] = (uint32_t)__popc(s2_mux(a0, a1, masks[local]));
			pass_b[b] = g[b] != 0xFFFFFFFFu && cnt_b[b] >= floors[local] && g[b] >= off;
		}
		uint32_t vw[S3_BATCH], info[S3_BATCH], bl[S3_BATCH];
#pragma unroll
		for(int b = 0;b < (int)S3_BATCH;++b){
			vw[b] = 0; info[b] = 0; bl[b] = 0;
			if(pass_b[b]){
				const uint32_t ws = g[b] - ((s2_rl(c_sd, b) >> 9) & 31u);
				vw[b] = Q.valid[ws >> 5]; info[b] = Q.blk_info[ws >> 5]; bl[b] = Q.blk_local[ws >> 5];
			}
		}
#pragma unroll
		for(int b = 0;b < (int)S3_BATCH;++b){
			if(!pass_b[b]) continue;
			const uint32_t sdv = s2_rl(c_sd, b);
			const uint32_t ws = g[b] - ((sdv >> 9) & 31u), seq = info[b] & BLK_SEQ_MASK;
			if(!((vw[b] >> (ws & 31u)) & 1u) || (info[b] & (BLK_DEGEN | BLK_INACTIVE))) continue;
			const uint32_t p_local = bl[b]*32u + (ws & 31u);
			const uint32_t orient = T3.or_base + (sdv & 0x1FFu), c = orient >> 1;
			if(orient & 1u) record_hit(sink, seq, c, make_key(seq, (int32_t)p_local + 31, 2, 0, 0), cnt_b[b]);
			else record_hit(sink, seq, c, make_key(seq, (int32_t)p_local, 1, 0, 0), cnt_b[b]);
		}
	}
	if(IA.ix_first && T3.n_irr_wg == 0) s3_irregular(T3, Q, IA, cand_fwd, cand_floor, sink, gw, n_gw, lane);
}
```

pcramp_amd/csrc/pcr_select.inc:

```
namespace {

struct PlanLists {
	std::vector<uint32_t> s2_seeds; std::vector<uint4> s2_masks; std::vector<uint8_t> s2_floors;
	std::vector<uint32_t> s2_group_end, s2_group_offmask, s2_group_or, s2_group_nor;
	std::vector<pcr_ctx::S3Launch> s3_launch;
	std::vector<uint32_t> s3_prefix;
	std::vector<uint8_t> s3_spans;
	std::vector<uint32_t> s1_seeds;
	void clear()
	{
		s2_seeds.clear(); s2_masks.clear(); s2_floors.clear(); s2_group_end.clear(); s2_group_offmask.clear(); s2_group_or.clear(); s2_group_nor.clear();
		s3_launch.clear(); s3_prefix.clear(); s3_spans.clear(); s1_seeds.clear();
	}
};

inline uint32_t spread16(uint32_t v)
{
	v &= 0xFFFFu;
	v = (v | (v << 8)) & 0x00FF00FFu; v = (v | (v << 4)) & 0x0F0F0F0Fu;
	v = (v | (v << 2)) & 0x33333333u; return (v | (v << 1)) & 0x55555555u;
}

constexpr uint32_t S2_MAX_GROUPS = 4096;
bool plan_seed2(pcr_ctx *ctx, PlanLists &L, const std::vector<pcrhost::Candidate> &cand, std::vector<uint32_t> &or_seed, std::vector<uint32_t> &or_plain, uint32_t &irr_off_mask,
	const SeqSet *S3 = nullptr)
{
	std::vector<uint32_t> &pf = L.s3_prefix;
	pf.clear();
	uint32_t pf_run = 0;
	const uint32_t n_or = 2*(uint32_t)cand.size();
	std::vector<uint32_t> &out = L.s2_seeds;
	out.clear(); L.s2_group_end.clear(); L.s2_group_offmask.clear(); L.s2_group_or.clear(); L.s2_group_nor.clear();
	irr_off_mask = 0;
	L.s2_masks.resize(n_or);
	if(ctx->s2_cache.size() > 16384) ctx->s2_cache.clear();
	size_t group_begin = 0; uint32_t group_mask = 0, group_or0 = 0, group_last = 0;
	auto fits = [&](size_t n, uint32_t g_or){
		if(S3) return g_or <= S3_MAX_OR && n <= S3_MAX_SEEDS;
		return g_or <= S2_MAX_OR && n <= S2_MAX_SEEDS && sizeof(S2Shared) + 17*(size_t)g_or + 8*n + 1024 <= 160*1024;
	};
	auto mask_of = [](const Planes &m){
		return make_uint4(spread16(m.a) | (spread16(m.a >> 16) << 1), spread16(m.c) | (spread16(m.c >> 16) << 1),
		                  spread16(m.g) | (spread16(m.g >> 16) << 1), spread16(m.t) | (spread16(m.t >> 16) << 1));
	};
	std::vector<uint8_t> &spans = L.s3_spans;
	spans.clear();
	if(ctx->s3_cache.size() > 16384) ctx->s3_cache.clear();
	for(uint32_t o = 0;o < n_or;++o){
		const pcrhost::Candidate &c = cand[o >> 1];
		const Planes &m = (o & 1u) ? c.rc : c.fwd;
		const pcr_ctx::S2Key key = {m.a, m.c, m.g, m.t, c.floor_};
		pcr_ctx::S3Entry *e3 = nullptr; const pcr_ctx::S2Entry *e2 = nullptr;
		if(S3){
			auto it = ctx->s3_cache.find(key);
			if(it == ctx->s3_cache.end()){
				pcr_ctx::S3Entry e; e.off_mask = 0;
				ctx->s3_tmp.clear(); ctx->s2_tmp.clear();
				e.seedable = pcrhost::orientation_index_seeds(m, c.floor_, ctx->s3_next, ctx->s3_tmp, ctx->s2_tmp);
				e.mask = mask_of(m);
				e.seeds.reserve(ctx->s3_tmp.size()); e.spans.reserve(ctx->s3_tmp.size());
				for(const pcrhost::FoldSeed &sd : ctx->s3_tmp){
					e.seeds.push_back((sd.code << 14) | ((uint32_t)sd.off << 9)); e.spans.push_back((uint8_t)(sd.lo | (sd.hi << 2))); e.off_mask |= 1u << sd.off;
				}
				it = ctx->s3_cache.emplace(key, std::move(e)).first;
			}
			e3 = &it->second; e2 = e3;
		}
		else{
			auto it = ctx->s2_cache.find(key);
			if(it == ctx->s2_cache.end()){
				pcr_ctx::S2Entry e; e.off_mask = 0;
				ctx->s2_tmp.clear();
				e.seedable = pcrhost::orientation_seeds(m, c.floor_, 0, ctx->s2_tmp, nullptr, S2_Q);
				e.mask = mask_of(m);
				e.seeds.reserve(ctx->s2_tmp.size());
				for(const pcrhost::Seed &sd : ctx->s2_tmp){ e.seeds.push_back((sd.code << 14) | ((uint32_t)sd.off << 9)); e.off_mask |= 1u << sd.off; }
				it = ctx->s2_cache.emplace(key, std::move(e)).first;
			}
			e2 = &it->second;
		}
		const pcr_ctx::S2Entry &e = *e2;
		L.s2_masks[o] = e.mask;
		if(!e.seedable){ or_plain.push_back(o); continue; }
		or_seed.push_back(o);
		if(!fits(out.size() - group_begin + e.seeds.size(), o - group_or0 + 1)){
			if(!fits(e.seeds.size(), 1) || L.s2_group_end.size() + 1 >= S2_MAX_GROUPS) return false;
			L.s2_group_end.push_back((uint32_t)out.size()); L.s2_group_offmask.push_back(group_mask); L.s2_group_or.push_back(group_or0); L.s2_group_nor.push_back(group_last - group_or0 + 1);
			group_begin = out.size(); group_mask = 0; group_or0 = o;
			if(S3){ pf.push_back(pf_run); pf_run = 0; }
		}
		group_last = o;
		const size_t at = out.size();
		out.resize(at + e.seeds.size());
		for(size_t k = 0;k < e.seeds.size();++k) out[at + k] = e.seeds[k] | (o - group_or0);
		if(S3){
			spans.insert(spans.end(), e3->spans.begin(), e3->spans.end());
			pcr_ctx::S3Chunks *ch = nullptr;
			for(pcr_ctx::S3Chunks &x : e3->chunks){ if(x.gen == S3->pix_generation){ ch = &x; break; } }
			if(!ch){
				ch = &e3->chunks[e3->next_slot]; e3->next_slot = (e3->next_slot + 1u) % pcr_ctx::S3_CHUNK_SETS;
				ch->run.resize(e.seeds.size());
				const uint32_t *const start = S3->pix_start_h.data();
				uint32_t run = 0;
				for(size_t k = 0;k < e.seeds.size();++k){
					const uint32_t key4 = (e.seeds[k] >> 14) << 2, sp = e3->spans[k];
					ch->run[k] = run; run += (start[key4 + (sp >> 2) + 1u] - start[key4 + (sp & 3u)] + 63u) >> 6;
				}
				ch->total = run; ch->gen = S3->pix_generation;
			}
			const size_t pa = pf.size();
			pf.resize(pa + ch->run.size());
			for(size_t k = 0;k < ch->run.size();++k) pf[pa + k] = pf_run + ch->run[k];
			pf_run += ch->total;
		}
		if(!(o & 1u)){ irr_off_mask |= e.off_mask; group_mask |= e.off_mask; }
	}
	L.s2_group_end.push_back((uint32_t)out.size()); L.s2_group_offmask.push_back(group_mask); L.s2_group_or.push_back(group_or0);
	L.s2_group_nor.push_back(or_seed.empty() ? 0u : group_last - group_or0 + 1);
	if(S3) pf.push_back(pf_run);
	return true;
}

constexpr size_t S3_LDS_BUDGET = 120*1024;
constexpr uint32_t S3_WG_THREADS = 1024;
uint32_t seed3_grid(const pcr_ctx *ctx) { return std::min<uint32_t>(2*ctx->n_cu, S3_MAX_WG); }
bool plan_seed3_slices(pcr_ctx *ctx, PlanLists &PL, bool with_irr)
{
	const uint32_t G_all = seed3_grid(ctx), seeds_per_turn = 16u*(S3_WG_THREADS/64);
	PL.s3_launch.resize(PL.s2_group_end.size());
	size_t g_begin = 0, g_prefix = 0;
	for(size_t g = 0;g < PL.s2_group_end.size();++g){
		const uint32_t ns = PL.s2_group_end[g] - (uint32_t)g_begin;
		g_begin = PL.s2_group_end[g];
		const uint32_t *P = PL.s3_prefix.data() + g_prefix;
		g_prefix += (size_t)ns + 1;
		pcr_ctx::S3Launch &L = PL.s3_launch[g];
		L.n_irr_wg = with_irr ? std::min<uint32_t>((ns + seeds_per_turn - 1u)/seeds_per_turn, G_all/4u) : 0u;
		const uint32_t G = G_all - L.n_irr_wg;
		L.n_chunks = P[ns]; L.per_wg = std::max<uint32_t>(1u, (L.n_chunks + G - 1u)/G); L.slice_cap = 2;
		if(ns == 0) continue;
		uint32_t at = 0;
		for(uint32_t w = 0;w <= G;++w){
			const uint64_t target = (uint64_t)w*L.per_wg;
			while(at + 1u < ns && P[at + 1u] <= target) ++at;
			L.W.start[w] = at;
		}
		for(uint32_t w = G + 1;w <= S3_MAX_WG;++w) L.W.start[w] = at;
		for(uint32_t w = 0;w < G;++w) L.slice_cap = std::max(L.slice_cap, std::min(L.W.start[w + 1] + 2u, ns + 1u) - L.W.start[w]);
		if(17*(size_t)PL.s2_group_nor[g] + 9*(size_t)L.slice_cap + 64 > S3_LDS_BUDGET) return false;
	}
	return true;
}

void plan_seed1(pcr_ctx *ctx, PlanLists &L, const std::vector<pcrhost::Candidate> &cand, std::vector<uint32_t> &or_seed, std::vector<uint32_t> &or_plain, uint32_t &irr_off_mask)
{
	const uint32_t n_or = 2*(uint32_t)cand.size();
	std::vector<uint32_t> &out = L.s1_seeds;
	out.clear();
	irr_off_mask = 0;
	if(ctx->s1_cache.size() > 16384) ctx->s1_cache.clear();
	std::vector<const pcr_ctx::S2Entry *> ent(n_or);
	size_t total = 0;
	for(uint32_t o = 0;o < n_or;++o){
		const pcrhost::Candidate &c = cand[o >> 1];
		const Planes &m = (o & 1u) ? c.rc : c.fwd;
		const pcr_ctx::S2Key key = {m.a, m.c, m.g, m.t, c.floor_};
		auto it = ctx->s1_cache.find(key);
		if(it == ctx->s1_cache.end()){
			pcr_ctx::S2Entry e; e.off_mask = 0;
			ctx->s2_tmp.clear();
			e.seedable = pcrhost::orientation_seeds(m, c.floor_, 0, ctx->s2_tmp);
			e.seeds.reserve(ctx->s2_tmp.size());
			for(const pcrhost::Seed &sd : ctx->s2_tmp){ e.seeds.push_back(sd.code | ((uint32_t)sd.off << 16)); e.off_mask |= 1u << sd.off; }
			it = ctx->s1_cache.emplace(key, std::move(e)).first;
		}
		ent[o] = &it->second;
		if(ent[o]->seedable) total += ent[o]->seeds.size();
	}
	std::vector<uint8_t> drop(n_or, 0);
	if(total > S1_MAX_SEEDS){
		std::vector<uint32_t> by_len;
		for(uint32_t o = 0;o < n_or;++o){ if(ent[o]->seedable) by_len.push_back(o); }
		std::stable_sort(by_len.begin(), by_len.end(), [&](uint32_t x, uint32_t y){ return ent[x]->seeds.size() > ent[y]->seeds.size(); });
		for(size_t i = 0;i < by_len.size() && total > S1_MAX_SEEDS;++i){ drop[by_len[i]] = 1; total -= ent[by_len[i]]->seeds.size(); }
	}
	out.resize(total);
	size_t at = 0;
	for(uint32_t o = 0;o < n_or;++o){
		const pcr_ctx::S2Entry &e = *ent[o];
		if(!e.seedable || drop[o]){ or_plain.push_back(o); continue; }
		or_seed.push_back(o);
		const uint32_t tag = o << 21;
		for(size_t k = 0;k < e.seeds.size();++k) out[at + k] = e.seeds[k] | tag;
		at += e.seeds.size();
		if(!(o & 1u)) irr_off_mask |= e.off_mask;
	}
}

struct HostSeedPlan {
	std::vector<pcrhost::Seed> seeds;
	std::vector<std::vector<std::pair<uint16_t, int8_t> > > inheritors;
	size_t n_inherited = 0;
	std::vector<uint32_t> image, heads, multi;
};

int plan_seed_host(pcr_ctx *ctx, const std::vector<pcrhost::Candidate> &cand, HostSeedPlan &H, std::vector<uint32_t> &or_seed, std::vector<uint32_t> &or_plain,
	uint32_t &irr_off_mask)
{
	const uint32_t n_or = 2*(uint32_t)cand.size();
	struct OrientInfo { uint32_t begin, end; int max_exact_pos; bool seeded; };
	std::vector<OrientInfo> info;
	std::vector<pcrhost::Seed> &seeds = H.seeds;
	std::vector<std::vector<std::pair<uint16_t, int8_t> > > &inheritors = H.inheritors;
	size_t &n_inherited = H.n_inherited;
	std::vector<uint32_t> &image = H.image, &heads = H.heads, &multi = H.multi;
	info.assign(n_or, OrientInfo());
	inheritors.assign(n_or, std::vector<std::pair<uint16_t, int8_t> >());
	seeds.reserve((size_t)n_or*32);
	for(uint32_t o = 0;o < n_or;++o){
		const pcrhost::Candidate &c = cand[o >> 1];
		OrientInfo &me = info[o];
		me.begin = (uint32_t)seeds.size(); me.max_exact_pos = -1;
		const uint32_t bo = 2*c.base + (o & 1u);
		const int32_t sh = (o & 1u) ? -c.shift : c.shift;
		if(c.base != (o >> 1) && info[bo].seeded && info[bo].max_exact_pos <= 24 && info[bo].max_exact_pos + sh <= 24){
			inheritors[bo].push_back(std::make_pair((uint16_t)o, (int8_t)sh));
			n_inherited += info[bo].end - info[bo].begin;
			me.seeded = true; me.max_exact_pos = (info[bo].max_exact_pos < 0) ? -1 : info[bo].max_exact_pos + sh;
		}
		else me.seeded = pcrhost::orientation_seeds((o & 1) ? c.rc : c.fwd, c.floor_, o, seeds, &me.max_exact_pos);
		me.end = (uint32_t)seeds.size();
		if(me.seeded) or_seed.push_back(o); else or_plain.push_back(o);
	}
	if(or_seed.empty()) return PCR_OK;
	if(ctx->seed_count.size() != 65536){ ctx->seed_count.assign(65536, 0); ctx->seed_own.assign(65536, 0); }
	std::vector<uint16_t> &count = ctx->seed_count;
	bool overflow = false;
	uint32_t distinct = 0;
	std::vector<uint8_t> &own = ctx->seed_own;
	for(;;){
		image.assign(SEED_IMAGE_WORDS, 0u);
		overflow = false; distinct = 0;
		for(const pcrhost::Seed &sd : seeds){
			uint16_t &c = count[sd.code];
			if(c == 0){ image[sd.code >> 5] |= 1u << (sd.code & 31); ++distinct; }
			c = (uint16_t)(c + 1 + (inheritors.empty() ? 0 : inheritors[sd.orient].size()));
			if(c > 255){ overflow = true; break; }
			++own[sd.code];
		}
		if(distinct > SEED_MAX_DISTINCT) overflow = true;
		if(!overflow || n_inherited || or_seed.size() < 2) break;
		for(const pcrhost::Seed &sd : seeds){ count[sd.code] = 0; own[sd.code] = 0; }
		std::vector<uint32_t> by_len(or_seed);
		std::stable_sort(by_len.begin(), by_len.end(), [&](uint32_t x, uint32_t y){ return info[x].end - info[x].begin > info[y].end - info[y].begin; });
		const size_t n_drop = (by_len.size() + 3)/4;
		std::vector<uint8_t> drop(n_or, 0);
		for(size_t i = 0;i < n_drop;++i) drop[by_len[i]] = 1;
		std::vector<pcrhost::Seed> kept; kept.reserve(seeds.size());
		for(uint32_t o = 0;o < n_or;++o){
			const uint32_t b = info[o].begin, e = info[o].end;
			info[o].begin = (uint32_t)kept.size();
			if(!drop[o]) kept.insert(kept.end(), seeds.begin() + b, seeds.begin() + e);
			info[o].end = (uint32_t)kept.size();
			if(drop[o]) info[o].seeded = false;
		}
		seeds.swap(kept);
		or_seed.clear(); or_plain.clear();
		for(uint32_t o = 0;o < n_or;++o){ if(info[o].seeded) or_seed.push_back(o); else or_plain.push_back(o); }
	}
	for(const pcrhost::Seed &sd : seeds){
		if(sd.orient & 1u) continue;
		irr_off_mask |= 1u << sd.off;
		if(!inheritors.empty()){ for(const std::pair<uint16_t, int8_t> &in : inheritors[sd.orient]) irr_off_mask |= 1u << (sd.off + in.second); }
	}
	if(overflow){
		or_plain.clear(); or_seed.clear(); image.clear();
		for(uint32_t o = 0;o < n_or;++o) or_plain.push_back(o);
	}
	else{
		uint16_t *rank16 = (uint16_t *)(image.data() + SEED_BITMAP_WORDS);
		uint32_t run = 0;
		for(uint32_t w = 0;w < SEED_BITMAP_WORDS;++w){ rank16[w] = (uint16_t)run; run += (uint32_t)__builtin_popcount(image[w]); }
		heads.assign(distinct, 0u);
		uint32_t n_multi = 0;
		for(const pcrhost::Seed &sd : seeds){
			const uint32_t h = rank16[sd.code >> 5] + (uint32_t)__builtin_popcount(image[sd.code >> 5] & ((1u << (sd.code & 31)) - 1u));
			if(count[sd.code] == 1){ heads[h] = SEED_SINGLE | ((uint32_t)sd.orient << 8) | sd.off; continue; }
			if(heads[h] == 0){ heads[h] = 0x40000000u | n_multi; n_multi += own[sd.code]; }
		}
		std::vector<uint32_t> raw(n_multi, 0u);
		std::vector<uint8_t> &fill = ctx->seed_fill; fill.assign(distinct, 0);
		for(const pcrhost::Seed &sd : seeds){
			if(count[sd.code] == 1) continue;
			const uint32_t h = rank16[sd.code >> 5] + (uint32_t)__builtin_popcount(image[sd.code >> 5] & ((1u << (sd.code & 31)) - 1u));
			const uint32_t start = heads[h] & 0x3FFFFFFFu;
			raw[start + fill[h]++] = (uint32_t)sd.orient | ((uint32_t)sd.off << 24);
		}
		multi.clear(); multi.reserve(n_multi + n_multi/2 + 16);
		for(uint32_t h = 0;h < distinct;++h){
			if(heads[h] & SEED_SINGLE) continue;
			const uint32_t start = heads[h] & 0x3FFFFFFFu, n = fill[h];
			const uint32_t out0 = (uint32_t)multi.size();
			uint32_t header_at = 0, members = 0, cur_base = 0xFFFFFFFFu; int32_t cur_boff = -1;
			for(uint32_t e = 0;e < n;++e){
				const uint32_t sd = raw[start + e], orient = sd & 0xFFFFu, off = sd >> 24;
				const pcrhost::Candidate &c = cand[orient >> 1];
				const int32_t sh = (orient & 1u) ? -c.shift : c.shift;
				int32_t boff = (int32_t)off - sh;
				uint32_t base_orient = 2*c.base + (orient & 1u);
				if(boff < 0 || boff > 24){ boff = (int32_t)off; base_orient = orient; }
				if(members && base_orient == cur_base && boff == cur_boff && members < 256){
					multi.push_back(sd); ++members;
					multi[header_at] = SEED_GROUP | cur_base | ((uint32_t)cur_boff << 16) | ((members - 1) << 21);
				}
				else{
					header_at = (uint32_t)multi.size(); members = 1; cur_base = base_orient; cur_boff = boff;
					multi.push_back(SEED_GROUP | cur_base | ((uint32_t)cur_boff << 16));
					multi.push_back(sd);
				}
				if(!inheritors.empty()){
					for(const std::pair<uint16_t, int8_t> &in : inheritors[orient]){
						if(members == 256){
							header_at = (uint32_t)multi.size(); members = 0;
							multi.push_back(SEED_GROUP | cur_base | ((uint32_t)cur_boff << 16));
						}
						multi.push_back((uint32_t)in.first | ((uint32_t)((int32_t)off + in.second) << 24)); ++members;
						multi[header_at] = SEED_GROUP | cur_base | ((uint32_t)cur_boff << 16) | ((members - 1) << 21);
					}
				}
			}
			heads[h] = (out0 << 9) | ((uint32_t)multi.size() - out0);
		}
		n_multi = (uint32_t)multi.size();
		if(n_multi >= (1u << 22)){ ctx->seed_count.clear(); g_err = "pcr_select_words: seed table too large"; return PCR_ERR_CAPACITY; }
	}
	return PCR_OK;
}


enum class ScanForm { Popcount, BitSliced, Seed1Host, Seed1Dev, Seed2, Seed3 };
inline const char *form_name(ScanForm f)
{
	static const char *const names[] = { "popcount", "bitsliced", "seed1-host", "seed1-dev", "seed2", "seed3" };
	return names[(int)f];
}
inline bool is_seed1(ScanForm f) { return f == ScanForm::Seed1Host || f == ScanForm::Seed1Dev; }
inline bool is_seed2(ScanForm f) { return f == ScanForm::Seed2 || f == ScanForm::Seed3; }

struct ScanPlan {
	ScanForm form = ScanForm::BitSliced;
	std::vector<uint32_t> or_seed, or_plain;
	uint32_t irr_off_mask = 0;
	HostSeedPlan H;
	bool s3_with_irr = false;
	bool need_plain = false, need_seedset = false;
	size_t n_seeds = 0;
	uint32_t n_live = 0, min_len = 0;
	void reset()
	{
		form = ScanForm::BitSliced; or_seed.clear(); or_plain.clear(); irr_off_mask = 0;
		H.seeds.clear(); H.inheritors.clear(); H.n_inherited = 0; H.image.clear(); H.heads.clear(); H.multi.clear();
		s3_with_irr = need_plain = need_seedset = false; n_seeds = 0; n_live = min_len = 0;
	}
};

inline uint32_t live_irregular(const SeqSet &S, uint32_t min_oligo_length)
{
	uint32_t n_live = 0;
	for(uint32_t k = std::min<uint32_t>(min_oligo_length, 256);k < 256;++k) n_live += S.irr_size_count[k];
	return n_live;
}

int irr_index_usable(pcr_ctx *ctx, SeqSet &S, bool &usable)
{
	usable = false;
	if(S.irr_n_multi != 0 || (uint64_t)24*S.n_irr >= (uint64_t(1) << 32)) return PCR_OK;
	const int rc = ensure_irr_index(ctx, S);
	usable = rc == PCR_OK && S.irx_usable;
	return rc;
}

int choose_scan_form(pcr_ctx *ctx, SeqSet &S, const std::vector<pcrhost::Candidate> &cand, int optimize_5, int optimize_3, uint32_t min_oligo_length, ScanPlan &P, PlanLists &L)
{
	const uint32_t n_or = 2*(uint32_t)cand.size();
	std::vector<uint32_t> &or_seed = P.or_seed, &or_plain = P.or_plain;
	P.min_len = min_oligo_length; P.n_live = live_irregular(S, min_oligo_length);
	int rc;
	const bool no_shifts = ctx->scan_version == 3 && !optimize_5 && !optimize_3;
	const bool seed2_ok = no_shifts && !ctx->force_seed1 && n_or <= 65535;
	bool want_seed3 = false;
	if(seed2_ok && !ctx->no_seed3 && !ctx->no_irr_index && ctx->s2_dbg == 0){
		bool worth = true;
		if(!S.pix_valid){
			std::vector<uint32_t> os, op; uint32_t om = 0;
			worth = plan_seed2(ctx, L, cand, os, op, om, nullptr) && op.empty() && !os.empty();
		}
		if(worth){
			if((rc = ensure_pos_index(ctx, S)) != PCR_OK) return rc;
			bool irr_ok = P.n_live == 0;
			if(S.pix_usable && !irr_ok && (rc = irr_index_usable(ctx, S, irr_ok)) != PCR_OK) return rc;
			want_seed3 = S.pix_usable && irr_ok; P.s3_with_irr = P.n_live > 0;
		}
	}
	bool use_seed2 = false;
	if(seed2_ok){
		use_seed2 = plan_seed2(ctx, L, cand, or_seed, or_plain, P.irr_off_mask, want_seed3 ? &S : nullptr);
		if(want_seed3 && !(use_seed2 && or_plain.empty() && !or_seed.empty() && plan_seed3_slices(ctx, L, P.s3_with_irr))){
			or_seed.clear(); or_plain.clear();
			use_seed2 = plan_seed2(ctx, L, cand, or_seed, or_plain, P.irr_off_mask, nullptr);
		}
		if(use_seed2 && !or_plain.empty() && (n_or <= S1_MAX_OR || or_seed.empty())) use_seed2 = false;
		if(!use_seed2){ or_seed.clear(); or_plain.clear(); P.irr_off_mask = 0; }
	}
	const bool use_seed3 = use_seed2 && want_seed3 && or_plain.empty() && !or_seed.empty()
		&& L.s3_prefix.size() == L.s2_seeds.size() + L.s2_group_end.size() && L.s3_spans.size() == L.s2_seeds.size();
	if(use_seed2){ P.form = use_seed3 ? ScanForm::Seed3 : ScanForm::Seed2; P.n_seeds = L.s2_seeds.size(); }
	else if(no_shifts && !ctx->host_seed_tables && n_or <= S1_MAX_OR){
		plan_seed1(ctx, L, cand, or_seed, or_plain, P.irr_off_mask);
		P.form = ScanForm::Seed1Dev; P.n_seeds = L.s1_seeds.size();
	}
	else if(ctx->scan_version == 3 && n_or <= 65535){
		const int prc = plan_seed_host(ctx, cand, P.H, or_seed, or_plain, P.irr_off_mask);
		if(ctx->seed_count.size() == 65536){ for(const pcrhost::Seed &sd : P.H.seeds){ ctx->seed_count[sd.code] = 0; ctx->seed_own[sd.code] = 0; } }
		if(prc != PCR_OK) return prc;
		P.form = ScanForm::Seed1Host; P.n_seeds = P.H.seeds.size() + P.H.n_inherited;
	}
	else{
		for(uint32_t o = 0;o < n_or;++o) or_plain.push_back(o);
		P.form = (ctx->scan_version == 1) ? ScanForm::Popcount : ScanForm::BitSliced;
	}
	if(or_seed.empty() && P.form != ScanForm::Popcount) P.form = ScanForm::BitSliced;
	P.need_plain = (ctx->scan_version != 1) && !or_plain.empty();
	P.need_seedset = !or_seed.empty() && S.n_degen_tiles > 0;
	return PCR_OK;
}

struct PassJob {
	pcr_ctx *ctx = nullptr; int which = 0, opt5 = 0, opt3 = 0; float thr = 0.0f; uint32_t min_len = 0; bool async = false;
	pcr_amplify_args args = {}; FusedAmp fa = {}; bool has_fa = false;
	uint32_t seq = 0;
	bool begun = false, ctrl_was_clean = false;
	std::vector<pcrhost::Candidate> cand; ScanPlan P; PlanLists L;
	std::vector<uint4> hf, hr; std::vector<uint32_t> hfl;
	std::vector<OligoDev> ol;
	bool fuse = false; size_t bits_bytes = 0;
	void reset()
	{
		seq = 0; begun = ctrl_was_clean = false; has_fa = false; fa = FusedAmp(); async = false;
		cand.clear(); P.reset(); L.clear(); hf.clear(); hr.clear(); hfl.clear(); ol.clear(); fuse = false; bits_bytes = 0;
	}
};

struct Scan2Staged { Scan2Tables T; const uint32_t *d_tab = nullptr, *d_bias = nullptr, *d_map = nullptr; };
struct StagedTables {
	SeedTables ST = {};
	Seed2Tables ST2 = {};
	const uint32_t *d_s3_prefix = nullptr; const uint8_t *d_s3_spans = nullptr;
	Scan2Staged plain, seedset;
	bool lean = false, fuse = false;
	size_t bits_bytes = 0;
};

void stage_scan2(Stager &st, const std::vector<uint32_t> &orients, Scan2Staged &B)
{
	B.d_tab = st.put(B.T.tab.data(), B.T.tab.size());
	B.d_bias = st.put(B.T.bias.data(), B.T.bias.size());
	std::vector<uint32_t> m(orients);
	m.resize((m.size() + 255) & ~size_t(255), 0xFFFFFFFFu);
	B.d_map = st.put(m.data(), m.size());
}

void prepare_tables(const SeqSet &S, PassJob &J, FusedAmp *fa)
{
	const std::vector<pcrhost::Candidate> &cand = J.cand;
	const uint32_t ncand = (uint32_t)cand.size(), n_or = 2*ncand;
	J.hf.resize(ncand); J.hr.resize(ncand); J.hfl.resize(ncand);
	for(uint32_t c = 0;c < ncand;++c){
		J.hf[c] = make_uint4(cand[c].fwd.a, cand[c].fwd.c, cand[c].fwd.g, cand[c].fwd.t);
		J.hr[c] = make_uint4(cand[c].rc.a, cand[c].rc.c, cand[c].rc.g, cand[c].rc.t);
		J.hfl[c] = cand[c].floor_;
	}
	if(is_seed2(J.P.form)){
		std::vector<uint8_t> &floors2 = J.L.s2_floors;
		floors2.assign(((size_t)n_or + 15) & ~size_t(15), 0);
		for(uint32_t o = 0;o < n_or;++o) floors2[o] = (uint8_t)std::min<uint32_t>(cand[o >> 1].floor_, 255u);
	}
	J.fuse = false; J.bits_bytes = 0; J.ol.clear();
	if(fa && fa->n_pairs){
		J.bits_bytes = (size_t)fa->n_pairs*((S.n + 63)/64)*sizeof(uint64_t);
		J.fuse = ((uintptr_t)fa->d_fr % 16 == 0) && ((uintptr_t)fa->d_rf % 16 == 0) && (J.bits_bytes % 16 == 0);
		if(J.fuse) build_oligos(fa->pairs, fa->n_pairs, fa->a, J.ol);
	}
}

int stage_tables(pcr_ctx *ctx, SeqSet &S, const PassJob &J, FusedAmp *fa, bool async, bool ctrl_was_clean, StagedTables &T)
{
	const std::vector<pcrhost::Candidate> &cand = J.cand;
	const ScanPlan &P = J.P; const PlanLists &L = J.L;
	const uint32_t ncand = (uint32_t)cand.size(), n_or = 2*ncand;
	const bool seed2 = is_seed2(P.form), seed3 = P.form == ScanForm::Seed3;
	const bool build_tables = P.form == ScanForm::Seed1Dev;
	const HostSeedPlan &H = P.H;
	int rc;
	if(P.need_plain) build_scan2_tables(cand, P.or_plain, T.plain.T);
	if(P.need_seedset) build_scan2_tables(cand, P.or_seed, T.seedset.T);
	size_t bytes = ncand*(2*sizeof(uint4) + sizeof(uint32_t)) + 1024;
	bytes += (T.plain.T.tab.size() + T.plain.T.bias.size() + P.or_plain.size() + 256)*sizeof(uint32_t);
	bytes += (T.seedset.T.tab.size() + T.seedset.T.bias.size() + P.or_seed.size() + 256)*sizeof(uint32_t);
	bytes += (H.image.size() + H.heads.size() + H.multi.size() + 64)*sizeof(uint32_t);
	if(seed2){
		bytes += L.s2_masks.size()*sizeof(uint4) + L.s2_floors.size() + L.s2_seeds.size()*sizeof(uint32_t) + 512;
		if(seed3) bytes += L.s3_prefix.size()*sizeof(uint32_t) + L.s3_spans.size() + 128;
	}
	if(build_tables) bytes += L.s1_seeds.size()*sizeof(uint32_t) + 256;
	T.bits_bytes = J.bits_bytes; T.fuse = J.fuse;
	if(T.fuse) bytes += J.ol.size()*sizeof(OligoDev) + 64;
	const uint32_t guard_seq = J.seq ? J.seq : ctx->mail_seq + 1;
	const uint64_t gen = S.ctrl.generation;
	if((rc = S.ctrl.ensure(8 + 2*(size_t)S.n + 4)) != PCR_OK) return rc;
	T.lean = ctx->direct_ok && async && T.fuse && seed2 && !P.or_seed.empty() && ctrl_was_clean && gen == S.ctrl.generation
		&& S.bucket_cap == POST_CAP && 2*fa->n_pairs <= 32*POST_MASK_WORDS;
	if(ctx->debug_log) fprintf(stderr, "[pcramp] staging: %s\n", T.lean ? "lean (tables written into device memory, no staging launch)" : "k_stage");
	Stager st(ctx);
	if((rc = T.lean ? st.begin_direct(bytes) : st.begin(bytes)) != PCR_OK) return rc;
	ctx->d_cand_fwd = st.put(J.hf.data(), ncand);
	ctx->d_cand_rc = st.put(J.hr.data(), ncand);
	ctx->d_cand_floor = st.put(J.hfl.data(), ncand);
	if(P.need_plain) stage_scan2(st, P.or_plain, T.plain);
	if(P.need_seedset) stage_scan2(st, P.or_seed, T.seedset);
	if(!H.image.empty()){
		T.ST.image = st.put(H.image.data(), H.image.size());
		T.ST.heads = st.put(H.heads.data(), H.heads.size());
		T.ST.multi = H.multi.empty() ? T.ST.heads : st.put(H.multi.data(), H.multi.size());
	}
	const uint32_t *d_s1_seeds = nullptr;
	if(build_tables){
		d_s1_seeds = st.put(L.s1_seeds.data(), L.s1_seeds.size());
		if((rc = ctx->s1_image.ensure(SEED_IMAGE_WORDS)) != PCR_OK) return rc;
		if((rc = ctx->s1_heads.ensure(2*(size_t)S1_MAX_SEEDS)) != PCR_OK) return rc;
		if((rc = ctx->s1_multi.ensure(S1_MAX_SEEDS)) != PCR_OK) return rc;
		T.ST.image = ctx->s1_image.p; T.ST.heads = ctx->s1_heads.p; T.ST.multi = ctx->s1_multi.p; T.ST.flat = 1;
	}
	if(seed2){
		T.ST2.seeds = st.put(L.s2_seeds.data(), L.s2_seeds.size());
		T.ST2.masks = st.put(L.s2_masks.data(), L.s2_masks.size());
		T.ST2.floors = st.put(L.s2_floors.data(), L.s2_floors.size());
		T.ST2.n_seeds = (uint32_t)L.s2_seeds.size(); T.ST2.n_or = n_or;
		if(seed3){ T.d_s3_prefix = st.put(L.s3_prefix.data(), L.s3_prefix.size()); T.d_s3_spans = st.put(L.s3_spans.data(), L.s3_spans.size()); }
	}
	const size_t ctrl_bytes = (8 + 2*(size_t)S.n)*sizeof(uint32_t);
	if(T.fuse){
		fa->d_oligos = st.put(J.ol.data(), J.ol.size());
		fa->staged = true;
		if(T.lean) st.seal(guard_seq);
		else if((rc = st.ship(S.ctrl.p, ctrl_bytes, fa->d_fr, T.bits_bytes, fa->d_rf, T.bits_bytes, guard_seq)) != PCR_OK) return rc;
	}
	else if((rc = st.ship(S.ctrl.p, ctrl_bytes, nullptr, 0, nullptr, 0, guard_seq)) != PCR_OK) return rc;
	if(build_tables){
		if((rc = ctx->s1_part.ensure(2*S1_GROUPS)) != PCR_OK) return rc;
		hipLaunchKernelGGL(k_seed_tables<false>, dim3(S1_GROUPS), dim3(S1_BUILD_THREADS), 0, ctx->stream, d_s1_seeds, (uint32_t)L.s1_seeds.size(),
			ctx->s1_part.p, ctx->s1_image.p, ctx->s1_heads.p, ctx->s1_multi.p);
		hipLaunchKernelGGL(k_seed_tables<true>, dim3(S1_GROUPS), dim3(S1_BUILD_THREADS), 0, ctx->stream, d_s1_seeds, (uint32_t)L.s1_seeds.size(),
			ctx->s1_part.p, ctx->s1_image.p, ctx->s1_heads.p, ctx->s1_multi.p);
		HIP_TRY(hipGetLastError());
	}
	return PCR_OK;
}


int launch_popcount(pcr_ctx *ctx, SeqSet &S, const HitSink &sink)
{
	hipLaunchKernelGGL(k_scan, dim3(S.n_tiles), dim3(SCAN_THREADS), 0, ctx->stream, S.planes.p, S.valid_d(),
		S.d_blk_off.p, S.d_len.p, S.d_active.p, S.tile_seq.p, S.tile_pos0.p, ctx->d_cand_fwd, ctx->d_cand_rc,
		ctx->d_cand_floor, sink.ncand, sink);
	HIP_TRY(hipGetLastError());
	return PCR_OK;
}

int launch_seed1(pcr_ctx *ctx, SeqSet &S, const ScanPlan &P, const StagedTables &T, const HitSink &sink)
{
	const uint32_t ncand = sink.ncand;
	const bool cand_lds = ncand <= SEED_CAND_LDS;
	const auto kernel = cand_lds ? k_seed<true> : k_seed<false>;
	const size_t dyn = cand_lds ? (size_t)ncand*(2*sizeof(uint4) + sizeof(uint32_t)) : 0;
	int per_cu = 0;
	const hipError_t oe = hipOccupancyMaxActiveBlocksPerMultiprocessor(&per_cu, kernel, SEED_THREADS, dyn);
	const size_t lds_wg = ((sizeof(SeedShared) + dyn + 4095)/4096)*4096;
	per_cu = std::max(1, std::min<int>(per_cu, (int)((160*1024)/lds_wg)));
	const uint32_t resident = (oe == hipSuccess) ? (uint32_t)per_cu*ctx->n_cu : SEED_MAX_GRID;
	const uint32_t tiles_per_wg = SEED_WAVES*SEED_TILES_PER_WAVE;
	const dim3 sgrid(std::min<uint32_t>((S.n_tiles + tiles_per_wg - 1)/tiles_per_wg, resident)), sblock(SEED_THREADS);
	IrrArgs IA; IA.irr = S.irr.p; IA.perm = S.irr_perm.p; IA.n_live = P.n_live; IA.off_mask = P.or_plain.empty() ? P.irr_off_mask : 0u;
	const uint32_t irr_wgs = (P.n_live + IRR_THREADS*IRR_PER_LANE - 1)/(IRR_THREADS*IRR_PER_LANE);
	const dim3 fgrid(sgrid.x + irr_wgs);
	if(ctx->debug_log) fprintf(stderr, "[pcramp] k_seed: %d workgroups per CU x %u CUs\n", per_cu, ctx->n_cu);
	hipLaunchKernelGGL(kernel, fgrid, sblock, dyn, ctx->stream, S.tb_d(), S.planes.p, S.valid_d(), S.d_blk_off.p, S.d_nblk_real.p, S.d_len.p, S.d_active.p,
		S.tile_seq.p, S.tile_pos0.p, S.tile_degen.p, S.n_tiles, T.ST, ctx->d_cand_fwd, ctx->d_cand_rc, ctx->d_cand_floor, ncand, IA, sgrid.x, sink);
	HIP_TRY(hipGetLastError());
	return PCR_OK;
}

int launch_seed3_group(pcr_ctx *ctx, SeqSet &S, const Seed2Tables &Tg, const uint32_t *d_chunk_prefix, const uint8_t *d_spans, const pcr_ctx::S3Launch &L3, const IrrArgs2 &IA,
	const HitSink &sink, const S2Clear &Z)
{
	Seed3Tables T3; T3.seeds = Tg.seeds; T3.spans = d_spans; T3.chunk_prefix = d_chunk_prefix; T3.masks = Tg.masks; T3.floors = Tg.floors;
	T3.n_seeds = Tg.n_seeds; T3.n_or = Tg.n_or; T3.or_base = Tg.or_base;
	T3.pix_first = S.pix_first.p; T3.pix_last = S.pix_last.p; T3.pix_ent = S.pix_ent.p;
	Seed3Set Q3 = { S.valid_d(), S.blk_info.p, S.blk_local.p, S.d_active.p };
	T3.n_chunks = L3.n_chunks; T3.per_wg = L3.per_wg; T3.slice_cap = L3.slice_cap;
	T3.n_irr_wg = IA.ix_first ? L3.n_irr_wg : 0u;
	const size_t dyn3 = (size_t)Tg.n_or*sizeof(uint4) + 2*(size_t)T3.slice_cap*sizeof(uint32_t) + (((size_t)Tg.n_or + 15) & ~size_t(15)) + (((size_t)T3.slice_cap + 15) & ~size_t(15)) + 16;
	if(!ctx->s3_attr_set){
		HIP_TRY(hipFuncSetAttribute((const void *)k_seed3<S3_WG_THREADS>, hipFuncAttributeMaxDynamicSharedMemorySize, 128*1024));
		ctx->s3_attr_set = true;
	}
	hipLaunchKernelGGL(k_seed3<S3_WG_THREADS>, dim3(seed3_grid(ctx)), dim3(S3_WG_THREADS), dyn3, ctx->stream, T3, Q3, IA, ctx->d_cand_fwd, ctx->d_cand_floor, sink, Z, L3.W);
	return PCR_OK;
}

int launch_seed_groups(pcr_ctx *ctx, SeqSet &S, const ScanPlan &P, const PlanLists &L, const StagedTables &T, const FusedAmp *fa, const HitSink &sink)
{
	const bool seed3 = P.form == ScanForm::Seed3;
	const uint32_t tiles_per_wg = S2_WAVES*2;
	const dim3 sgrid(std::max<uint32_t>(1u, std::min<uint32_t>((S.n_tiles + tiles_per_wg - 1)/tiles_per_wg, ctx->n_cu))), sblock(S2_THREADS);
	int rc;
	if(!ctx->s2_attr_set){
		HIP_TRY(hipFuncSetAttribute((const void *)k_seed2<false>, hipFuncAttributeMaxDynamicSharedMemorySize, (int)(160*1024 - sizeof(S2Shared))));
		HIP_TRY(hipFuncSetAttribute((const void *)k_seed2<true>, hipFuncAttributeMaxDynamicSharedMemorySize, (int)(160*1024 - sizeof(S2Shared))));
		ctx->s2_attr_set = true;
	}
	const auto k_seed2_of_ctx = ctx->s2_dbg ? k_seed2<true> : k_seed2<false>;
	bool irr_by_index = P.s3_with_irr;
	if(!seed3){
		irr_by_index = P.or_plain.empty() && P.n_live > 0 && !ctx->no_irr_index;
		for(size_t g = 0, b = 0;g < L.s2_group_end.size();++g){ if((size_t)L.s2_group_end[g] - b > (size_t)sgrid.x*S2_THREADS) irr_by_index = false; b = L.s2_group_end[g]; }
		if(irr_by_index && (rc = irr_index_usable(ctx, S, irr_by_index)) != PCR_OK) return rc;
	}
	uint32_t g_begin = 0, g_prefix = 0;
	bool first_launch = true;
	for(size_t g = 0;g < L.s2_group_end.size();++g){
		Seed2Tables Tg = T.ST2;
		const uint32_t or0 = L.s2_group_or[g], g_or = L.s2_group_nor[g];
		const uint8_t *const d_spans = seed3 ? T.d_s3_spans + g_begin : nullptr;
		Tg.seeds = T.ST2.seeds + g_begin; Tg.n_seeds = L.s2_group_end[g] - g_begin;
		Tg.masks = T.ST2.masks + (size_t)or0; Tg.floors = T.ST2.floors + or0; Tg.n_or = g_or; Tg.or_base = or0;
		g_begin = L.s2_group_end[g];
		if(Tg.n_seeds == 0){ g_prefix += 1u; continue; }
		const size_t dyn = (size_t)g_or*sizeof(uint4) + (((size_t)g_or + 15) & ~size_t(15)) + 8*((size_t)Tg.n_seeds + 64) + 16;
		IrrArgs2 IA; IA.scan = S.irr_scan.p; IA.irr = S.irr.p; IA.n_live = P.n_live;
		IA.off_mask = L.s2_group_offmask[g];
		IA.exhaustive = first_launch ? 1u : 0u;
		IA.ix_first = IA.ix_last = IA.ix_words = nullptr; IA.min_cws = std::min<uint32_t>(P.min_len, 255u);
		if(!P.or_plain.empty()){
			IA.off_mask = 0;
			if(!first_launch) IA.n_live = 0;
		}
		else if(irr_by_index){
			IA.ix_first = S.irx_first.p; IA.ix_last = S.irx_last.p; IA.ix_words = S.irx_words.p; IA.n_live = 0;
		}
		if(ctx->debug_log) fprintf(stderr, "[pcramp] k_seed2: %u workgroups, %u seeds of orientations %u..%u (group %zu of %zu), %zu + %zu B of LDS\n", sgrid.x, Tg.n_seeds,
			or0, or0 + g_or - 1, g + 1, L.s2_group_end.size(), sizeof(S2Shared), dyn);
		S2Clear Z = { nullptr, 0u, nullptr, 0u, nullptr };
		if(T.lean && first_launch){
			Z.z0 = (uint4 *)fa->d_fr; Z.z1 = (uint4 *)fa->d_rf; Z.n0 = Z.n1 = (uint32_t)(T.bits_bytes/16); Z.ctrl = sink.counters;
		}
		if(seed3){
			if((rc = launch_seed3_group(ctx, S, Tg, T.d_s3_prefix + g_prefix, d_spans, L.s3_launch[g], IA, sink, Z)) != PCR_OK) return rc;
			g_prefix += Tg.n_seeds + 1u;
		}
		else hipLaunchKernelGGL(k_seed2_of_ctx, sgrid, sblock, dyn, ctx->stream, S.tb_d(), S.valid_d(), S.tile_desc.p, S.n_tiles, Tg, S.d_active.p, ctx->d_cand_fwd, ctx->d_cand_floor,
			sink.ncand, IA, sink, ctx->s2_dbg, Z);
		HIP_TRY(hipGetLastError());
		first_launch = false;
	}
	return PCR_OK;
}

int launch_irregular(pcr_ctx *ctx, SeqSet &S, const ScanPlan &P, const HitSink &sink)
{
	const unsigned irr_grid = (P.n_live + IRR_THREADS*IRR_PER_LANE - 1)/(IRR_THREADS*IRR_PER_LANE);
	hipLaunchKernelGGL(k_scan_irr, dim3(irr_grid), dim3(IRR_THREADS), 0, ctx->stream, S.irr.p, S.irr_perm.p, P.n_live,
		S.d_active.p, ctx->d_cand_fwd, ctx->d_cand_floor, sink.ncand, sink);
	HIP_TRY(hipGetLastError());
	return PCR_OK;
}

int launch_scans(pcr_ctx *ctx, SeqSet &S, const ScanPlan &P, const PlanLists &L, const StagedTables &T, const FusedAmp *fa, const HitSink &sink)
{
	int rc = PCR_OK;
	const uint32_t ncand = sink.ncand;
	if(S.n_tiles){
		ProfScope scan_prof(ctx, PCR_PROF_SCAN, ctx->prof && (ctx->prof_pass++ % ctx->prof_stride) == 0);
		if(P.need_plain && (rc = launch_scan2(ctx, S, T.plain.T, ncand, sink, T.plain.d_tab, T.plain.d_bias, nullptr, S.n_tiles, T.plain.d_map)) != PCR_OK) return rc;
		if(P.form == ScanForm::Popcount) rc = launch_popcount(ctx, S, sink);
		else if(is_seed1(P.form)) rc = launch_seed1(ctx, S, P, T, sink);
		else if(is_seed2(P.form)) rc = launch_seed_groups(ctx, S, P, L, T, fa, sink);
		if(rc != PCR_OK) return rc;
		if(P.need_seedset && (rc = launch_scan2(ctx, S, T.seedset.T, ncand, sink, T.seedset.d_tab, T.seedset.d_bias, S.degen_tiles.p, S.n_degen_tiles,
			T.seedset.d_map)) != PCR_OK) return rc;
		scan_prof.finish();
	}
	const bool irr_taken = S.n_tiles && (is_seed1(P.form) || is_seed2(P.form));
	if(P.n_live && !irr_taken) rc = launch_irregular(ctx, S, P, sink);
	return rc;
}


template<class K>
void launch_post(K kernel, uint32_t waves, pcr_ctx *ctx, SeqSet &S, const HitSink &sink, const FusedAmp *fa, uint32_t seq)
{
	hipLaunchKernelGGL(kernel, dim3((S.n + waves - 1)/waves), dim3(64*waves), 0, ctx->stream, sink.hits, sink.seq_count, sink.best, sink.ncand, S.planes.p,
		S.d_blk_off.p, S.irr.p, S.irr_off.p, S.db.p, S.d_seg_hi, sink.counters, sink.epoch, S.n,
		fa->d_oligos, fa->n_pairs, (2*fa->n_pairs + 31)/32, S.d_len.p, S.d_active.p, fa->a->amp_min, fa->a->amp_max,
		fa->a->ident_threshold, fa->a->use_taq_mama, fa->d_fr, fa->d_rf, (uint64_t)((S.n + 63)/64), ctx->mail.dev + (seq % pcr_ctx::MAIL_RING), seq);
}
int fused_tail(pcr_ctx *ctx, SeqSet &S, const HitSink &sink, FusedAmp *fa, uint32_t reserved_seq)
{
	const uint32_t seq = reserved_seq ? reserved_seq : ++ctx->mail_seq;
	if(sink.cap == POST_CAP){
		launch_post(k_post<8>, 8, ctx, S, sink, fa, seq);
		S.ctrl_clean = true; S.touched_from_seg = true;
	}
	else if(sink.cap == 128) launch_post(k_post_big<128, 4>, 4, ctx, S, sink, fa, seq);
	else launch_post(k_post_big<256, 4>, 4, ctx, S, sink, fa, seq);
	HIP_TRY(hipGetLastError());
	fa->posted = true;
	S.touched_built = false;
	return PCR_OK;
}

template<class K, class... Extra>
void launch_finalize(K kernel, dim3 grid, dim3 block, size_t lds, pcr_ctx *ctx, SeqSet &S, const HitSink &sink, Extra... extra)
{
	hipLaunchKernelGGL(kernel, grid, block, lds, ctx->stream, sink.hits, sink.seq_count, sink.cap, sink.best, sink.ncand, S.planes.p, S.d_blk_off.p, S.irr.p,
		S.irr_off.p, S.db.p, S.d_seg_hi, sink.counters, sink.epoch, S.touched.p, extra...);
}
template<bool ALL = false>
int plain_tail(pcr_ctx *ctx, SeqSet &S, const HitSink &sink, bool async, FusedAmp *fa)
{
	int rc;
	hipLaunchKernelGGL(k_touched, dim3((S.n + 255)/256), dim3(256), 0, ctx->stream, sink.seq_count, S.n, sink.counters, S.touched.p);
	HIP_TRY(hipGetLastError());
	S.touched_built = true;
	uint32_t np2 = 1; while(np2 < sink.cap) np2 <<= 1;
	if(np2 <= 1024) launch_finalize(k_finalize<FIN_WAVES, ALL>, dim3((S.n + FIN_WAVES - 1)/FIN_WAVES), dim3(64*FIN_WAVES), (size_t)FIN_WAVES*np2*sizeof(uint64_t), ctx, S, sink);
	else if(np2 <= MAX_BUCKET_CAP) launch_finalize(k_finalize<1, ALL>, dim3(S.n), dim3(64), (size_t)np2*sizeof(uint64_t), ctx, S, sink);
	else{
		if((rc = ctx->fin_scratch.ensure((size_t)S.n*np2)) != PCR_OK) return rc;
		launch_finalize(k_finalize_big<ALL>, dim3(S.n), dim3(FINBIG_THREADS), 0, ctx, S, sink, ctx->fin_scratch.p);
	}
	HIP_TRY(hipGetLastError());
	++ctx->mail_seq;
	if(async && fa && fa->staged){ fa->pub_seq = ctx->mail_seq; fa->pub_counters = sink.counters; }
	else{
		hipLaunchKernelGGL(k_publish, dim3(1), dim3(64), 0, ctx->stream, sink.counters, ctx->mail.dev + (ctx->mail_seq % pcr_ctx::MAIL_RING), ctx->mail_seq);
		HIP_TRY(hipGetLastError());
	}
	return PCR_OK;
}

uint32_t resized_buckets(bool overflowed, uint32_t cap, uint32_t largest_fill, int attempt)
{
	if(overflowed){
		uint32_t want = cap*2;
		while(want < largest_fill && want < MAX_BUCKET_CAP_GLOBAL) want *= 2;
		return want;
	}
	if(cap <= 64 || attempt >= 12) return 0;
	uint32_t want = 64;
	while(want < largest_fill + largest_fill/16) want *= 2;
	return (want*4 <= cap) ? want : 0;
}

inline bool fused_tail_fits(uint32_t cap, uint32_t n_pairs) { return (cap == POST_CAP || cap == 128 || cap == 256) && 2*n_pairs <= 32*POST_MASK_WORDS; }
inline bool buckets_fit(uint64_t n_slots) { return n_slots < (uint64_t(1) << 32) && n_slots*(sizeof(Hit) + sizeof(DevEntry)) <= (uint64_t(96) << 30); }

inline bool begin_pass(SeqSet &S)
{
	S.have_db = false; S.n_entries = 0;
	const bool ctrl_was_clean = S.ctrl_clean;
	S.ctrl_clean = false; S.touched_from_seg = false;
	return ctrl_was_clean;
}

int plan_pass(pcr_ctx *ctx, PassJob &J, const pcr_pair *pairs, uint32_t n_pairs)
{
	SeqSet &S = ctx->sets[J.which];
	HostTimer timer(ctx, 0);
	if(ctx->timing) ++ctx->n_timed;
	pcrhost::build_candidates((const uint64_t *)pairs, n_pairs, J.opt5 != 0, J.opt3 != 0, J.thr, J.cand);
	const uint32_t ncand = (uint32_t)J.cand.size();
	if(S.n == 0 || ncand == 0) return PCR_OK;
	int rc;
	if((rc = choose_scan_form(ctx, S, J.cand, J.opt5, J.opt3, J.min_len, J.P, J.L)) != PCR_OK) return rc;
	if(ctx->debug_log) fprintf(stderr, "[pcramp] scan plan: form=%s, %u candidates, %zu seeded orientations (%zu seeds), %zu plain, %u/%u IUPAC tiles, %u-slot buckets\n",
		form_name(J.P.form), ncand, J.P.or_seed.size(), J.P.n_seeds, J.P.or_plain.size(), S.n_degen_tiles, S.n_tiles, S.bucket_cap);
	prepare_tables(S, J, J.has_fa ? &J.fa : nullptr);
	return PCR_OK;
}

bool plans_without_device_work(const pcr_ctx *ctx, const SeqSet &S, int opt5, int opt3, uint32_t min_len)
{
	if(ctx->scan_version != 3 || opt5 || opt3 || ctx->force_seed1) return false;
	const bool may_want_seed3 = !ctx->no_seed3 && !ctx->no_irr_index && ctx->s2_dbg == 0;
	if(may_want_seed3 && !S.pix_valid) return false;
	if(live_irregular(S, min_len) == 0 || ctx->no_irr_index) return true;
	return S.irr_n_multi != 0 || (uint64_t)24*S.n_irr >= (uint64_t(1) << 32) || S.irx_valid;
}

bool pass_is_pipelinable(const pcr_ctx *ctx, const PassJob &J)
{
	const SeqSet &S = ctx->sets[J.which];
	return J.async && J.has_fa && J.fuse && S.n != 0 && !J.cand.empty() && is_seed2(J.P.form)
		&& fused_tail_fits(S.bucket_cap, J.fa.n_pairs) && buckets_fit((uint64_t)S.n*S.bucket_cap);
}

int run_pass(pcr_ctx *ctx, PassJob &J, uint64_t *n_entries_out)
{
	SeqSet &S = ctx->sets[J.which];
	FusedAmp *const fa = J.has_fa ? &J.fa : nullptr;
	const bool async = J.async;
	const bool ctrl_was_clean = J.begun ? J.ctrl_was_clean : begin_pass(S);
	const ScanPlan &P = J.P;
	const uint32_t ncand = (uint32_t)J.cand.size();
	if(S.n == 0 || ncand == 0){ S.have_db = true; S.n_touched = 0; return PCR_OK; }
	HostTimer timer(ctx, 1);
	int rc;
	if((rc = ctx->best.ensure((size_t)S.n*ncand)) != PCR_OK) return rc;
	if(ctx->best.generation != ctx->best_seen){
		HIP_TRY(hipMemsetAsync(ctx->best.p, 0, ctx->best.cap*sizeof(uint32_t), ctx->stream));
		ctx->best_seen = ctx->best.generation; ctx->epoch = std::min(ctx->debug_epoch, EPOCH_LIMIT);
	}
	StagedTables T;
	if((rc = stage_tables(ctx, S, J, fa, async, ctrl_was_clean, T)) != PCR_OK) return rc;

	timer.next(2);
	uint32_t h_counters[4];
	if((rc = S.touched.ensure(S.n)) != PCR_OK) return rc;
	S.d_seg_hi = S.ctrl.p + 8 + S.n;
	for(int attempt = 0;;++attempt){
		const uint32_t cap = S.bucket_cap;
		const uint64_t n_slots = (uint64_t)S.n*cap;
		if(!buckets_fit(n_slots)){
			assert(J.seq == 0);
			S.bucket_cap = 64;
			g_err = "pcr_select_words: the per-sequence hit buckets would not fit (too many tied sites per sequence)"; return PCR_ERR_CAPACITY;
		}
		if((rc = ctx->hits.ensure(n_slots)) != PCR_OK) return rc;
		if((rc = S.db.ensure(n_slots)) != PCR_OK) return rc;
		if(attempt > 0) HIP_TRY(hipMemsetAsync(S.ctrl.p, 0, (8 + 2*(size_t)S.n)*sizeof(uint32_t), ctx->stream));
		if(ctx->epoch >= EPOCH_LIMIT){
			HIP_TRY(hipMemsetAsync(ctx->best.p, 0, ctx->best.cap*sizeof(uint32_t), ctx->stream));
			ctx->epoch = 0;
		}
		++ctx->epoch;
		HitSink sink; sink.best = ctx->best.p; sink.hits = ctx->hits.p; sink.seq_count = S.ctrl.p + 8;
		sink.counters = S.ctrl.p; sink.cap = cap; sink.ncand = ncand; sink.epoch = ctx->epoch;
		const bool fused = async && fa && fa->staged && fused_tail_fits(cap, fa->n_pairs);
		if(J.seq && !fused){ g_err = "pcr_screen_device: a pipelined pass lost its fused tail"; return PCR_ERR_STATE; }
		if((rc = launch_scans(ctx, S, P, J.L, T, fa, sink)) != PCR_OK) return rc;
		if((rc = fused ? fused_tail(ctx, S, sink, fa, J.seq) : plain_tail(ctx, S, sink, async, fa)) != PCR_OK) return rc;
		if(async){
			S.db_cap = cap; S.n_slots = n_slots;
			S.n_touched = N_TOUCHED_UNKNOWN; S.n_entries = 1; S.have_db = true;
			return PCR_OK;
		}
		timer.next(3);
		if((rc = mail_wait(ctx, ctx->mail_seq, h_counters)) != PCR_OK) return rc;
		timer.next(2);
		S.db_cap = cap; S.n_slots = n_slots;
		const bool overflowed = (h_counters[0] & 1u) != 0;
		if(overflowed && (attempt >= 12 || cap >= MAX_BUCKET_CAP_GLOBAL)){ g_err = "pcr_select_words: more than 65536 candidate sites in one sequence (per-sequence bucket limit)"; return PCR_ERR_CAPACITY; }
		const uint32_t want = resized_buckets(overflowed, cap, h_counters[2], attempt);
		if(!want) break;
		S.bucket_cap = want;
	}
	if(ctx->debug_log) fprintf(stderr, "[pcramp] pass done: %u-slot buckets, largest fill %u, %u sequences with entries\n", S.db_cap, h_counters[2], h_counters[3]);
	S.n_touched = h_counters[3];
	S.n_entries = S.n_touched ? 1 : 0;
	S.have_db = true;
	if(n_entries_out){
		if((rc = count_entries(ctx, S)) != PCR_OK) return rc;
		*n_entries_out = S.n_entries;
	}
	return PCR_OK;
}

void fill_job(pcr_ctx *ctx, PassJob &J, pcr_set which, int optimize_5, int optimize_3, float threshold, uint32_t min_oligo_length, bool async, const FusedAmp *fa)
{
	J.ctx = ctx; J.which = (int)which; J.opt5 = optimize_5; J.opt3 = optimize_3; J.thr = threshold; J.min_len = min_oligo_length; J.async = async;
	J.has_fa = fa != nullptr;
	if(fa){ J.fa = *fa; J.args = *fa->a; J.fa.a = &J.args; }
}

int select_impl(pcr_ctx *ctx, pcr_set which, const pcr_pair *pairs, uint32_t n_pairs, int optimize_5, int optimize_3,
	float threshold, uint32_t min_oligo_length, uint64_t *n_entries_out, bool async, FusedAmp *fa = nullptr)
{
	if(!ctx || (n_pairs && !pairs)){ g_err = "pcr_select_words: bad argument"; return PCR_ERR_ARG; }
	if(min_oligo_length < 1 || min_oligo_length > 32){ g_err = "pcr_select_words: min_oligo_length must be in [1,32]"; return PCR_ERR_ARG; }
	HIP_TRY(hipSetDevice(ctx->device));
	if(n_entries_out) *n_entries_out = 0;
	assert(ctx->lq_client.queued.load() == 0);
	PassJob J;
	fill_job(ctx, J, which, optimize_5, optimize_3, threshold, min_oligo_length, async, fa);
	J.ctrl_was_clean = begin_pass(ctx->sets[which]); J.begun = true;
	int rc = plan_pass(ctx, J, pairs, n_pairs);
	if(rc == PCR_OK) rc = run_pass(ctx, J, n_entries_out);
	if(fa){ const pcr_amplify_args *a = fa->a; *fa = J.fa; fa->a = a; }
	return rc;
}


struct Launcher {
	int device; hipStream_t stream; unsigned refs = 0;
	cpu_set_t near; bool have_near = false;
	pcrq::LaunchQueue q;
	Launcher(int dev, hipStream_t st, unsigned spin_us);
};
std::mutex g_launchers_m;
std::vector<Launcher *> g_launchers;

PassJob *acquire_job(pcr_ctx *ctx)
{
	PassJob *J = nullptr;
	{
		std::lock_guard<std::mutex> lk(ctx->job_m);
		if(!ctx->job_free.empty()){ J = ctx->job_free.back(); ctx->job_free.pop_back(); }
	}
	if(!J){ J = new PassJob(); ctx->job_all.push_back(J); }
	return J;
}
void release_job(pcr_ctx *ctx, PassJob *J)
{
	J->reset();
	std::lock_guard<std::mutex> lk(ctx->job_m);
	ctx->job_free.push_back(J);
}
void free_jobs(pcr_ctx *ctx)
{
	for(PassJob *J : ctx->job_all) delete J;
	ctx->job_all.clear(); ctx->job_free.clear();
}

constexpr unsigned LAUNCH_SPIN_US = 200;

bool read_cpu_list(const std::string &path, cpu_set_t &set)
{
	CPU_ZERO(&set);
	FILE *f = fopen(path.c_str(), "r");
	if(!f) return false;
	char buf[4096]; const bool got = fgets(buf, sizeof(buf), f) != nullptr;
	fclose(f);
	if(!got) return false;
	for(const char *p = buf;*p && *p != '\n';){
		char *e; const long a = strtol(p, &e, 10);
		if(e == p) return false;
		long b = a;
		if(*e == '-'){ p = e + 1; b = strtol(p, &e, 10); if(e == p) return false; }
		for(long c = a;c <= b && c < CPU_SETSIZE;++c) CPU_SET((int)c, &set);
		p = (*e == ',') ? e + 1 : e;
	}
	return true;
}
bool near_cpus(cpu_set_t &out)
{
	const int cpu = sched_getcpu();
	if(cpu < 0) return false;
	const std::string base = "/sys/devices/system/cpu/cpu" + std::to_string(cpu);
	cpu_set_t llc, core, allowed;
	if(!read_cpu_list(base + "/cache/index3/shared_cpu_list", llc)) return false;
	if(!read_cpu_list(base + "/topology/thread_siblings_list", core)) CPU_ZERO(&core);
	CPU_SET(cpu, &core);
	if(sched_getaffinity(0, sizeof(allowed), &allowed) != 0) return false;
	CPU_ZERO(&out);
	for(int c = 0;c < CPU_SETSIZE;++c){ if(CPU_ISSET(c, &llc) && CPU_ISSET(c, &allowed) && !CPU_ISSET(c, &core)) CPU_SET(c, &out); }
	return CPU_COUNT(&out) > 0;
}

Launcher::Launcher(int dev, hipStream_t st, unsigned spin_us) : device(dev), stream(st),
	q([](void *job, std::string &err) -> int {
		PassJob &J = *(PassJob *)job;
		assert(J.seq != 0 && J.ctx->launcher);
		const int rc = run_pass(J.ctx, J, nullptr);
		if(rc != PCR_OK) err = g_err;
		return rc;
	},
	[](void *job){ PassJob *J = (PassJob *)job; release_job(J->ctx, J); },
	[this]{
		if(have_near) (void)pthread_setaffinity_np(pthread_self(), sizeof(near), &near);
		(void)hipSetDevice(device);
	},
	spin_us)
{
	const char *v = getenv("PCRAMP_LAUNCH_PIN");
	have_near = !(v && v[0] == '0') && near_cpus(near);
}

Launcher *attach_launcher(pcr_ctx *ctx)
{
	if(ctx->launcher) return ctx->launcher;
	std::lock_guard<std::mutex> lk(g_launchers_m);
	for(Launcher *L : g_launchers){ if(L->device == ctx->device && L->stream == ctx->stream){ ++L->refs; return ctx->launcher = L; } }
	unsigned spin = LAUNCH_SPIN_US;
	if(const char *v = getenv("PCRAMP_LAUNCH_SPIN_US")) spin = (unsigned)std::min<unsigned long>(strtoul(v, nullptr, 0), 10000ul);
	Launcher *L = new Launcher(ctx->device, ctx->stream, spin);
	if(ctx->debug_log || ctx->timing) fprintf(stderr, "[pcramp] launcher thread for stream %p: caller on cpu %d, launcher %s (%d cpus), spin %u us\n", (void *)ctx->stream,
		sched_getcpu(), L->have_near ? "pinned beside it" : "not pinned", L->have_near ? CPU_COUNT(&L->near) : 0, spin);
	L->refs = 1;
	g_launchers.push_back(L);
	return ctx->launcher = L;
}
void detach_launcher(pcr_ctx *ctx)
{
	Launcher *L = ctx->launcher;
	if(!L) return;
	ctx->launcher = nullptr;
	{
		std::lock_guard<std::mutex> lk(g_launchers_m);
		if(--L->refs) return;
		g_launchers.erase(std::find(g_launchers.begin(), g_launchers.end(), L));
	}
	L->q.stop();
	delete L;
}

int flush_launcher(pcr_ctx *ctx)
{
	if(!ctx->launcher) return PCR_OK;
	ctx->launcher->q.flush(&ctx->lq_client);
	int code; std::string msg; uint32_t seq;
	if(!ctx->lq_client.take_error(code, msg, seq)) return PCR_OK;
	std::vector<pcr_ctx::Pending> &pd = ctx->pending;
	pd.erase(std::remove_if(pd.begin(), pd.end(), [&](const pcr_ctx::Pending &q){ return (int32_t)(q.seq - seq) >= 0; }), pd.end());
	g_err = msg;
	return code;
}

int screen_pass(pcr_ctx *ctx, pcr_set which, const pcr_pair *pairs, uint32_t n_pairs, int optimize_5, int optimize_3,
	float select_threshold, uint32_t min_oligo_length, const pcr_amplify_args *args, uint64_t *d_bits_fr, uint64_t *d_bits_rf)
{
	if(min_oligo_length < 1 || min_oligo_length > 32){ g_err = "pcr_select_words: min_oligo_length must be in [1,32]"; return PCR_ERR_ARG; }
	int rc;
	if(ctx->lq_client.poisoned.load(std::memory_order_acquire) && (rc = flush_launcher(ctx)) != PCR_OK) return rc;
	HIP_TRY(hipSetDevice(ctx->device));
	SeqSet &S = ctx->sets[which];
	FusedAmp fa; fa.pairs = pairs; fa.n_pairs = n_pairs; fa.a = args; fa.d_fr = d_bits_fr; fa.d_rf = d_bits_rf;
	PassJob *J = acquire_job(ctx);
	fill_job(ctx, *J, which, optimize_5, optimize_3, select_threshold, min_oligo_length, true, &fa);
	bool inline_pass = !ctx->launch_thread || !plans_without_device_work(ctx, S, optimize_5, optimize_3, min_oligo_length);
	if(inline_pass){
		if((rc = flush_launcher(ctx)) != PCR_OK){ release_job(ctx, J); return rc; }
		J->ctrl_was_clean = begin_pass(S); J->begun = true;
	}
	rc = plan_pass(ctx, *J, pairs, n_pairs);
	if(rc == PCR_OK && !inline_pass && !pass_is_pipelinable(ctx, *J)){
		inline_pass = true;
		rc = flush_launcher(ctx);
	}
	if(rc != PCR_OK){
		if(!J->begun){ (void)flush_launcher(ctx); (void)begin_pass(S); }
		release_job(ctx, J);
		return rc;
	}
	pcr_ctx::Pending p;
	p.which = (int)which; p.pairs.assign(pairs, pairs + n_pairs); p.opt5 = optimize_5; p.opt3 = optimize_3;
	p.thr = select_threshold; p.min_len = min_oligo_length; p.args = *args; p.d_fr = d_bits_fr; p.d_rf = d_bits_rf;
	if(!inline_pass){
		Launcher *L = attach_launcher(ctx);
		p.seq = J->seq = ++ctx->mail_seq;
		J->fa.pairs = nullptr;
		ctx->pending.push_back(std::move(p));
		++ctx->n_pipelined;
		L->q.push(&ctx->lq_client, J, J->seq);
		return PCR_OK;
	}
	assert(ctx->lq_client.queued.load() == 0);
	const uint32_t seq0 = ctx->mail_seq;
	rc = run_pass(ctx, *J, nullptr);
	if(rc == PCR_OK && !J->fa.posted) rc = amplify_launch(ctx, S, pairs, n_pairs, args, d_bits_fr, d_bits_rf, &J->fa);
	release_job(ctx, J);
	if(rc != PCR_OK) return rc;
	if(ctx->mail_seq != seq0){
		p.seq = ctx->mail_seq;
		ctx->pending.push_back(std::move(p));
	}
	return PCR_OK;
}

int drain(pcr_ctx *ctx)
{
	{ const int frc = flush_launcher(ctx); if(frc != PCR_OK) return frc; }
	if(ctx->pending.empty()) return PCR_OK;
	std::vector<pcr_ctx::Pending> pend;
	pend.swap(ctx->pending);
	int rc;
	for(size_t i = 0;i < pend.size();++i){
		uint32_t c[4];
		if((rc = mail_wait(ctx, pend[i].seq, c)) != PCR_OK) return rc;
		SeqSet &S = ctx->sets[pend[i].which];
		if(!(c[0] & 1u)){
			if(c[3] == N_TOUCHED_UNKNOWN_DEV){ S.n_touched = N_TOUCHED_UNKNOWN; S.n_entries = 1; }
			else{ S.n_touched = c[3]; S.n_entries = c[3] ? 1 : 0; }
			continue;
		}
		uint32_t want = S.bucket_cap*2;
		while(want < c[2] && want < MAX_BUCKET_CAP_GLOBAL) want *= 2;
		S.bucket_cap = std::min(want, MAX_BUCKET_CAP_GLOBAL);
		for(size_t j = i;j < pend.size();++j){
			const pcr_ctx::Pending &q = pend[j];
			if((rc = select_impl(ctx, (pcr_set)q.which, q.pairs.data(), (uint32_t)q.pairs.size(), q.opt5, q.opt3, q.thr, q.min_len, nullptr, false)) != PCR_OK) return rc;
			if((rc = amplify_launch(ctx, ctx->sets[q.which], q.pairs.data(), (uint32_t)q.pairs.size(), &q.args, q.d_fr, q.d_rf)) != PCR_OK) return rc;
		}
		break;
	}
	return PCR_OK;
}

}
```

Before: 23.66 billion.

## Precompute per-seed index ranges on host into packed 16-byte seed records

Replaces the separate seed, chunk-prefix and span arrays for the seed3 scan with one packed record per seed (seed, chunk offset, first index, count). The records are resolved on the host against the position-index start table and cached per index generation, so the kernel no longer reads pix_first/pix_last during the binary search. Staging writes the records directly into the pinned buffer, avoiding intermediate vectors. It adds a generation check between plan and launch, plus extra host timers. The cost is more LDS per slice entry and host work to emit the records.

```diff
diff --git a/pcramp_amd/csrc/pcr_device.hip b/pcramp_amd/csrc/pcr_device.hip
--- a/pcramp_amd/csrc/pcr_device.hip
+++ b/pcramp_amd/csrc/pcr_device.hip
@@ -626,14 +626,10 @@
 	bool force_seed1 = false;
 	struct S2Key { uint32_t a, c, g, t, floor_; bool operator==(const S2Key &o) const { return a == o.a && c == o.c && g == o.g && t == o.t && floor_ == o.floor_; } };
 	struct S2KeyHash { size_t operator()(const S2Key &k) const { uint64_t h = 0x9E3779B97F4A7C15ull; for(uint32_t v : {k.a, k.c, k.g, k.t, k.floor_}){ h ^= v; h *= 0x100000001B3ull; h ^= h >> 29; } return (size_t)h; } };
-	struct S2Entry { std::vector<uint32_t> seeds;  uint32_t off_mask; bool seedable; uint4 mask;  };
+	struct S2Entry { std::vector<uint32_t> seeds;  uint32_t off_mask; bool seedable; pcrhost::MaskEntry mask;  };
 	std::unordered_map<S2Key, S2Entry, S2KeyHash> s2_cache;
 	std::vector<pcrhost::Seed> s2_tmp;
-	static constexpr int S3_CHUNK_SETS = 4;
-	struct S3Chunks { uint64_t gen = 0; uint32_t total = 0; std::vector<uint32_t> run; };
-	struct S3Entry : S2Entry { std::vector<uint8_t> spans;  S3Chunks chunks[S3_CHUNK_SETS]; uint32_t next_slot = 0; };
-	std::unordered_map<S2Key, S3Entry, S2KeyHash> s3_cache;
-	std::vector<pcrhost::FoldSeed> s3_tmp;
+	pcrhost::SeedCache s3_cache;
 	struct S3Launch { Seed3Slices W; uint32_t n_chunks, per_wg, slice_cap, n_irr_wg; };
 	bool no_seed3 = false, s3_attr_set = false;
 	bool s3_next = true;
@@ -700,7 +696,7 @@
 	const uint4 *d_cand_fwd = nullptr, *d_cand_rc = nullptr; const uint32_t *d_cand_floor = nullptr;
 	const OligoDev *d_oligos = nullptr;
 	bool debug_log = false;
-	bool timing = false; double t_host[8] = {0, 0, 0, 0, 0, 0, 0, 0}; uint64_t n_timed = 0;
+	bool timing = false; double t_host[12] = {0, 0, 0, 0, 0, 0, 0, 0, 0, 0, 0, 0}; uint64_t n_timed = 0;
 	bool prof = false; uint32_t prof_stride = 1, prof_pass = 0;
 	std::vector<std::pair<Event, Event> > prof_events;
 	double prof_ms = 0.0; uint64_t prof_launches = 0;
@@ -1033,6 +1029,14 @@
 		used = (used + 15) & ~size_t(15);
 		memcpy(host + used, src, n*sizeof(T));
 		T *at = (T *)((direct ? dev : ctx->arena.p) + used);
+		used += n*sizeof(T);
+		return at;
+	}
+	template<class T> const T *alloc(size_t n, T *&h)
+	{
+		used = (used + 15) & ~size_t(15);
+		h = (T *)(host + used);
+		const T *at = (const T *)((direct ? dev : ctx->arena.p) + used);
 		used += n*sizeof(T);
 		return at;
 	}
@@ -1367,6 +1371,8 @@
 			(unsigned long long)ctx->n_pipelined, (unsigned long long)ctx->n_timed, ctx->lq_client.max_depth);
 		fprintf(stderr, "[pcramp] host us/pass: plan %.1f  stage %.1f  launch %.1f  wait %.1f | amplify prep %.1f  launch %.1f  (%llu passes)\n",
 			ctx->t_host[0]/n, ctx->t_host[1]/n, ctx->t_host[2]/n, ctx->t_host[3]/n, ctx->t_host[4]/n, ctx->t_host[5]/n, (unsigned long long)ctx->n_timed);
+		fprintf(stderr, "[pcramp] host us/pass, stage A by part: candidates %.2f  seed listing %.2f  slices %.2f  tables %.2f | rest of screen_pass (job, pending, enqueue) %.2f\n",
+			ctx->t_host[6]/n, (ctx->t_host[7] - ctx->t_host[8])/n, ctx->t_host[8]/n, ctx->t_host[9]/n, ctx->t_host[10]/n);
 	}
 	delete ctx;
 }
diff --git a/pcramp_amd/csrc/pcr_host.hpp b/pcramp_amd/csrc/pcr_host.hpp
--- a/pcramp_amd/csrc/pcr_host.hpp
+++ b/pcramp_amd/csrc/pcr_host.hpp
@@ -4,6 +4,7 @@
 #include <stdint.h>
 #include <algorithm>
 #include <deque>
+#include <unordered_map>
 #include <vector>
 
 namespace pcrhost {
@@ -700,6 +701,140 @@
 		if(cost4) *cost4 = c4;
 	}
 	return true;
+}
+
+struct SeedRec {
+	uint32_t seed, chunk0, first, count;
+	SeedRec() {}
+	SeedRec(uint32_t s, uint32_t c, uint32_t f, uint32_t n) : seed(s), chunk0(c), first(f), count(n) {}
+};
+static_assert(sizeof(SeedRec) == 16, "a seed record is 16 bytes");
+struct alignas(16) MaskEntry { uint32_t x, y, z, w; };
+
+inline uint32_t spread16(uint32_t v)
+{
+	v &= 0xFFFFu;
+	v = (v | (v << 8)) & 0x00FF00FFu; v = (v | (v << 4)) & 0x0F0F0F0Fu;
+	v = (v | (v << 2)) & 0x33333333u; return (v | (v << 1)) & 0x55555555u;
+}
+inline MaskEntry mask_entry(const Planes &m)
+{
+	MaskEntry e = { spread16(m.a) | (spread16(m.a >> 16) << 1), spread16(m.c) | (spread16(m.c >> 16) << 1),
+	                spread16(m.g) | (spread16(m.g >> 16) << 1), spread16(m.t) | (spread16(m.t >> 16) << 1) };
+	return e;
+}
+
+struct OligoKey { uint32_t a, c, g, t, floor_; bool operator==(const OligoKey &o) const { return a == o.a && c == o.c && g == o.g && t == o.t && floor_ == o.floor_; } };
+struct OligoKeyHash { size_t operator()(const OligoKey &k) const { uint64_t h = 0x9E3779B97F4A7C15ull; for(uint32_t v : {k.a, k.c, k.g, k.t, k.floor_}){ h ^= v; h *= 0x100000001B3ull; h ^= h >> 29; } return (size_t)h; } };
+
+constexpr int S3_CHUNK_SETS = 4;
+struct SeedRuns { uint64_t gen = 0; uint32_t total = 0; std::vector<SeedRec> recs; };
+struct SeedEntry {
+	std::vector<uint32_t> seeds;
+	std::vector<uint8_t> spans;
+	uint32_t off_mask = 0; bool seedable = false; MaskEntry mask = {0, 0, 0, 0};
+	SeedRuns runs[S3_CHUNK_SETS]; uint32_t next_slot = 0, last_slot = 0;
+};
+struct SeedCache {
+	struct Slot { OligoKey key; SeedEntry *entry; };
+	std::unordered_map<OligoKey, SeedEntry, OligoKeyHash> map;
+	std::vector<Slot> memo;
+	std::vector<std::vector<SeedRec> > retired;
+	std::vector<FoldSeed> tmp3; std::vector<Seed> tmp2;
+	bool full() const { return map.size() > 16384; }
+	void release_retired() { retired.clear(); }
+	void clear() { map.clear(); memo.clear(); retired.clear(); }
+};
+struct SeedLimits { uint32_t max_or, max_seeds, max_groups; };
+
+inline const SeedRuns &seed_runs(SeedCache &cache, SeedEntry &e, const uint32_t *start, uint64_t gen)
+{
+	if(e.runs[e.last_slot].gen == gen) return e.runs[e.last_slot];
+	for(uint32_t i = 0;i < (uint32_t)S3_CHUNK_SETS;++i){ if(e.runs[i].gen == gen){ e.last_slot = i; return e.runs[i]; } }
+	SeedRuns &r = e.runs[e.next_slot];
+	e.last_slot = e.next_slot; e.next_slot = (e.next_slot + 1u) % (uint32_t)S3_CHUNK_SETS;
+	if(!r.recs.empty()){ cache.retired.push_back(std::move(r.recs)); r.recs = std::vector<SeedRec>(); }
+	r.recs.resize(e.seeds.size());
+	uint32_t run = 0;
+	for(size_t k = 0;k < e.seeds.size();++k){
+		const uint32_t key4 = (e.seeds[k] >> 14) << 2, sp = e.spans[k];
+		const uint32_t first = start[key4 + (sp & 3u)], count = start[key4 + (sp >> 2) + 1u] - first;
+		r.recs[k] = SeedRec(e.seeds[k], run, first, count);
+		run += (count + 63u) >> 6;
+	}
+	r.total = run; r.gen = gen;
+	return r;
+}
+
+struct SeedPart { const SeedRec *src; uint32_t n, id, chunk0; bool end; };
+
+inline bool list_index_seeds(const std::vector<Candidate> &cand, SeedCache &cache, bool fold, const uint32_t *start, uint64_t gen, const SeedLimits &lim,
+	std::vector<SeedPart> &parts, std::vector<MaskEntry> &masks, std::vector<uint32_t> &group_end, std::vector<uint32_t> &group_offmask,
+	std::vector<uint32_t> &group_or, std::vector<uint32_t> &group_nor, std::vector<uint32_t> &or_seed, std::vector<uint32_t> &or_plain, uint32_t &irr_off_mask)
+{
+	const uint32_t n_or = 2*(uint32_t)cand.size();
+	parts.clear(); group_end.clear(); group_offmask.clear(); group_or.clear(); group_nor.clear();
+	irr_off_mask = 0;
+	masks.resize(n_or);
+	if(cache.full()) cache.clear();
+	if(cache.memo.size() < n_or){ const SeedCache::Slot none = { {0, 0, 0, 0, 0}, nullptr }; cache.memo.resize(n_or, none); }
+	uint32_t n_seeds = 0, group_seeds = 0, group_mask = 0, group_or0 = 0, group_last = 0, run = 0;
+	for(uint32_t o = 0;o < n_or;++o){
+		const Candidate &c = cand[o >> 1];
+		const Planes &m = (o & 1u) ? c.rc : c.fwd;
+		const OligoKey key = {m.a, m.c, m.g, m.t, c.floor_};
+		SeedCache::Slot &slot = cache.memo[o];
+		if(!slot.entry || !(slot.key == key)){
+			auto it = cache.map.find(key);
+			if(it == cache.map.end()){
+				SeedEntry e;
+				cache.tmp3.clear(); cache.tmp2.clear();
+				e.seedable = orientation_index_seeds(m, c.floor_, fold, cache.tmp3, cache.tmp2);
+				e.mask = mask_entry(m);
+				e.seeds.reserve(cache.tmp3.size()); e.spans.reserve(cache.tmp3.size());
+				for(const FoldSeed &sd : cache.tmp3){
+					e.seeds.push_back((sd.code << 14) | ((uint32_t)sd.off << 9)); e.spans.push_back((uint8_t)(sd.lo | (sd.hi << 2))); e.off_mask |= 1u << sd.off;
+				}
+				it = cache.map.emplace(key, std::move(e)).first;
+			}
+			slot.key = key; slot.entry = &it->second;
+		}
+		SeedEntry &e = *slot.entry;
+		masks[o] = e.mask;
+		if(!e.seedable){ or_plain.push_back(o); continue; }
+		or_seed.push_back(o);
+		const uint32_t ns = (uint32_t)e.seeds.size();
+		if(o - group_or0 + 1 > lim.max_or || (size_t)group_seeds + ns > lim.max_seeds){
+			if(ns > lim.max_seeds || lim.max_or < 1 || group_end.size() + 1 >= lim.max_groups) return false;
+			const SeedPart end = { nullptr, 0, 0, run, true };
+			parts.push_back(end);
+			group_end.push_back(n_seeds); group_offmask.push_back(group_mask); group_or.push_back(group_or0); group_nor.push_back(group_last - group_or0 + 1);
+			group_seeds = 0; group_mask = 0; group_or0 = o; run = 0;
+		}
+		group_last = o;
+		if(ns){
+			const SeedRuns &r = seed_runs(cache, e, start, gen);
+			const SeedPart part = { r.recs.data(), ns, o - group_or0, run, false };
+			parts.push_back(part);
+			run += r.total; n_seeds += ns; group_seeds += ns;
+		}
+		if(!(o & 1u)){ irr_off_mask |= e.off_mask; group_mask |= e.off_mask; }
+	}
+	const SeedPart end = { nullptr, 0, 0, run, true };
+	parts.push_back(end);
+	group_end.push_back(n_seeds); group_offmask.push_back(group_mask); group_or.push_back(group_or0);
+	group_nor.push_back(or_seed.empty() ? 0u : group_last - group_or0 + 1);
+	return true;
+}
+
+inline void emit_seed_records(const std::vector<SeedPart> &parts, SeedRec *dst)
+{
+	for(const SeedPart &p : parts){
+		if(p.end){ *dst++ = SeedRec(0, p.chunk0, 0, 0); continue; }
+		const SeedRec *const s = p.src;
+		for(uint32_t k = 0;k < p.n;++k) dst[k] = SeedRec(s[k].seed + p.id, s[k].chunk0 + p.chunk0, s[k].first, s[k].count);
+		dst += p.n;
+	}
 }
 
 inline bool move_trials(const Planes &cur, int move, double max_degen, int primer_min, int primer_max, std::vector<Planes> &out)
diff --git a/pcramp_amd/csrc/pcr_scan_seed3.inc b/pcramp_amd/csrc/pcr_scan_seed3.inc
--- a/pcramp_amd/csrc/pcr_scan_seed3.inc
+++ b/pcramp_amd/csrc/pcr_scan_seed3.inc
@@ -32,12 +32,10 @@
 }
 
 struct Seed3Tables {
-	const uint32_t *seeds;
-	const uint32_t *chunk_prefix;
-	const uint8_t *spans;
+	const uint4 *recs;
 	const uint4 *masks; const uint8_t *floors;
 	uint32_t n_seeds, n_or, or_base;
-	const uint32_t *pix_first, *pix_last; const uint4 *pix_ent;
+	const uint4 *pix_ent;
 	uint32_t n_chunks, per_wg, slice_cap;
 	uint32_t n_irr_wg;
 };
@@ -76,7 +74,7 @@
 {
 	for(uint32_t i0 = gw*16u;i0 < T3.n_seeds;i0 += n_gw*16u){
 		const uint32_t i = i0 + lane;
-		const uint32_t sdv = (lane < 16u && i < T3.n_seeds) ? T3.seeds[i] : S2_END;
+		const uint32_t sdv = (lane < 16u && i < T3.n_seeds) ? T3.recs[i].x : S2_END;
 		const uint32_t orient = T3.or_base + (sdv & 0x1FFu);
 		uint32_t first = 0, cnt = 0;
 		if(sdv != S2_END && !(orient & 1u)){
@@ -108,10 +106,8 @@
 {
 	extern __shared__ uint4 s3_dyn[];
 	uint4 *const masks = s3_dyn;
-	uint32_t *const prefix = (uint32_t *)(masks + T3.n_or);
-	uint32_t *const seeds = prefix + T3.slice_cap;
-	uint8_t *const floors = (uint8_t *)(seeds + T3.slice_cap);
-	uint8_t *const spans = floors + ((T3.n_or + 15u) & ~15u);
+	uint4 *const recs = masks + T3.n_or;
+	uint8_t *const floors = (uint8_t *)(recs + T3.slice_cap);
 	const uint32_t wave = threadIdx.x >> 6, lane = threadIdx.x & 63u;
 	for(uint32_t i = blockIdx.x*S3_THREADS + threadIdx.x;i < Z.n0;i += gridDim.x*S3_THREADS) Z.z0[i] = make_uint4(0, 0, 0, 0);
 	for(uint32_t i = blockIdx.x*S3_THREADS + threadIdx.x;i < Z.n1;i += gridDim.x*S3_THREADS) Z.z1[i] = make_uint4(0, 0, 0, 0);
@@ -125,7 +121,7 @@
 	const uint32_t wg = blockIdx.x - T3.n_irr_wg, n_wg = gridDim.x - T3.n_irr_wg;
 	const uint32_t s_lo = W.start[wg];
 	const uint32_t n_slice = min(min(W.start[wg + 1] + 2u, T3.n_seeds + 1u) - s_lo, T3.slice_cap);
-	for(uint32_t i = threadIdx.x;i < n_slice;i += S3_THREADS){ prefix[i] = T3.chunk_prefix[s_lo + i]; const bool in = s_lo + i < T3.n_seeds; seeds[i] = in ? T3.seeds[s_lo + i] : 0u; spans[i] = in ? T3.spans[s_lo + i] : (uint8_t)0; }
+	for(uint32_t i = threadIdx.x;i < n_slice;i += S3_THREADS) recs[i] = T3.recs[s_lo + i];
 	__syncthreads();
 	const uint32_t gw = wg*S3_WAVES + wave, n_gw = n_wg*S3_WAVES;
 	const uint32_t q_lo = wg*T3.per_wg, q_hi = min(q_lo + T3.per_wg, T3.n_chunks);
@@ -135,11 +131,10 @@
 			const uint32_t q = q0 + lane*S3_WAVES;
 			if(lane < S3_BATCH && q < q_hi){
 				uint32_t lo = 0, hi = n_slice - 1u;
-				while(hi - lo > 1u){ const uint32_t mid = (lo + hi) >> 1; if(prefix[mid] <= q) lo = mid; else hi = mid; }
-				c_sd = seeds[lo];
-				const uint32_t key = (c_sd >> 14) << 2, sp = spans[lo];
-				const uint32_t f = T3.pix_first[key + (sp & 3u)], e = T3.pix_last[key + (sp >> 2)], j0 = (q - prefix[lo])*64u;
-				c_first = f + j0; c_cnt = (e - f) - j0;
+				while(hi - lo > 1u){ const uint32_t mid = (lo + hi) >> 1; if(recs[mid].y <= q) lo = mid; else hi = mid; }
+				const uint4 r = recs[lo];
+				const uint32_t j0 = (q - r.y)*64u;
+				c_sd = r.x; c_first = r.z + j0; c_cnt = r.w - j0;
 			}
 		}
 		uint4 en[S3_BATCH];
diff --git a/pcramp_amd/csrc/pcr_select.inc b/pcramp_amd/csrc/pcr_select.inc
--- a/pcramp_amd/csrc/pcr_select.inc
+++ b/pcramp_amd/csrc/pcr_select.inc
@@ -1,85 +1,56 @@
 namespace {
 
 struct PlanLists {
-	std::vector<uint32_t> s2_seeds; std::vector<uint4> s2_masks; std::vector<uint8_t> s2_floors;
+	std::vector<uint32_t> s2_seeds; std::vector<pcrhost::MaskEntry> s2_masks; std::vector<uint8_t> s2_floors;
 	std::vector<uint32_t> s2_group_end, s2_group_offmask, s2_group_or, s2_group_nor;
 	std::vector<pcr_ctx::S3Launch> s3_launch;
-	std::vector<uint32_t> s3_prefix;
-	std::vector<uint8_t> s3_spans;
+	std::vector<pcrhost::SeedPart> s3_parts; std::vector<uint32_t> s3_chunk0; bool s3_listed = false; uint64_t s3_generation = 0;
+	size_t s3_n_recs() const { return (size_t)s2_group_end.back() + s2_group_end.size(); }
 	std::vector<uint32_t> s1_seeds;
 	void clear()
 	{
 		s2_seeds.clear(); s2_masks.clear(); s2_floors.clear(); s2_group_end.clear(); s2_group_offmask.clear(); s2_group_or.clear(); s2_group_nor.clear();
-		s3_launch.clear(); s3_prefix.clear(); s3_spans.clear(); s1_seeds.clear();
+		s3_launch.clear(); s3_parts.clear(); s3_listed = false; s3_generation = 0; s1_seeds.clear();
 	}
 };
-
-inline uint32_t spread16(uint32_t v)
-{
-	v &= 0xFFFFu;
-	v = (v | (v << 8)) & 0x00FF00FFu; v = (v | (v << 4)) & 0x0F0F0F0Fu;
-	v = (v | (v << 2)) & 0x33333333u; return (v | (v << 1)) & 0x55555555u;
-}
 
 constexpr uint32_t S2_MAX_GROUPS = 4096;
 bool plan_seed2(pcr_ctx *ctx, PlanLists &L, const std::vector<pcrhost::Candidate> &cand, std::vector<uint32_t> &or_seed, std::vector<uint32_t> &or_plain, uint32_t &irr_off_mask,
 	const SeqSet *S3 = nullptr)
 {
-	std::vector<uint32_t> &pf = L.s3_prefix;
-	pf.clear();
-	uint32_t pf_run = 0;
+	L.s3_parts.clear(); L.s3_listed = false; L.s2_seeds.clear();
+	if(S3){
+		const pcrhost::SeedLimits lim = { S3_MAX_OR, S3_MAX_SEEDS, S2_MAX_GROUPS };
+		L.s3_generation = S3->pix_generation;
+		L.s3_listed = pcrhost::list_index_seeds(cand, ctx->s3_cache, ctx->s3_next, S3->pix_start_h.data(), S3->pix_generation, lim, L.s3_parts, L.s2_masks,
+			L.s2_group_end, L.s2_group_offmask, L.s2_group_or, L.s2_group_nor, or_seed, or_plain, irr_off_mask);
+		return L.s3_listed;
+	}
 	const uint32_t n_or = 2*(uint32_t)cand.size();
 	std::vector<uint32_t> &out = L.s2_seeds;
-	out.clear(); L.s2_group_end.clear(); L.s2_group_offmask.clear(); L.s2_group_or.clear(); L.s2_group_nor.clear();
+	L.s2_group_end.clear(); L.s2_group_offmask.clear(); L.s2_group_or.clear(); L.s2_group_nor.clear();
 	irr_off_mask = 0;
 	L.s2_masks.resize(n_or);
 	if(ctx->s2_cache.size() > 16384) ctx->s2_cache.clear();
 	size_t group_begin = 0; uint32_t group_mask = 0, group_or0 = 0, group_last = 0;
 	auto fits = [&](size_t n, uint32_t g_or){
-		if(S3) return g_or <= S3_MAX_OR && n <= S3_MAX_SEEDS;
 		return g_or <= S2_MAX_OR && n <= S2_MAX_SEEDS && sizeof(S2Shared) + 17*(size_t)g_or + 8*n + 1024 <= 160*1024;
 	};
-	auto mask_of = [](const Planes &m){
-		return make_uint4(spread16(m.a) | (spread16(m.a >> 16) << 1), spread16(m.c) | (spread16(m.c >> 16) << 1),
-		                  spread16(m.g) | (spread16(m.g >> 16) << 1), spread16(m.t) | (spread16(m.t >> 16) << 1));
-	};
-	std::vector<uint8_t> &spans = L.s3_spans;
-	spans.clear();
-	if(ctx->s3_cache.size() > 16384) ctx->s3_cache.clear();
 	for(uint32_t o = 0;o < n_or;++o){
 		const pcrhost::Candidate &c = cand[o >> 1];
 		const Planes &m = (o & 1u) ? c.rc : c.fwd;
 		const pcr_ctx::S2Key key = {m.a, m.c, m.g, m.t, c.floor_};
-		pcr_ctx::S3Entry *e3 = nullptr; const pcr_ctx::S2Entry *e2 = nullptr;
-		if(S3){
-			auto it = ctx->s3_cache.find(key);
-			if(it == ctx->s3_cache.end()){
-				pcr_ctx::S3Entry e; e.off_mask = 0;
-				ctx->s3_tmp.clear(); ctx->s2_tmp.clear();
-				e.seedable = pcrhost::orientation_index_seeds(m, c.floor_, ctx->s3_next, ctx->s3_tmp, ctx->s2_tmp);
-				e.mask = mask_of(m);
-				e.seeds.reserve(ctx->s3_tmp.size()); e.spans.reserve(ctx->s3_tmp.size());
-				for(const pcrhost::FoldSeed &sd : ctx->s3_tmp){
-					e.seeds.push_back((sd.code << 14) | ((uint32_t)sd.off << 9)); e.spans.push_back((uint8_t)(sd.lo | (sd.hi << 2))); e.off_mask |= 1u << sd.off;
-				}
-				it = ctx->s3_cache.emplace(key, std::move(e)).first;
-			}
-			e3 = &it->second; e2 = e3;
-		}
-		else{
-			auto it = ctx->s2_cache.find(key);
-			if(it == ctx->s2_cache.end()){
-				pcr_ctx::S2Entry e; e.off_mask = 0;
-				ctx->s2_tmp.clear();
-				e.seedable = pcrhost::orientation_seeds(m, c.floor_, 0, ctx->s2_tmp, nullptr, S2_Q);
-				e.mask = mask_of(m);
-				e.seeds.reserve(ctx->s2_tmp.size());
-				for(const pcrhost::Seed &sd : ctx->s2_tmp){ e.seeds.push_back((sd.code << 14) | ((uint32_t)sd.off << 9)); e.off_mask |= 1u << sd.off; }
-				it = ctx->s2_cache.emplace(key, std::move(e)).first;
-			}
-			e2 = &it->second;
-		}
-		const pcr_ctx::S2Entry &e = *e2;
+		auto it = ctx->s2_cache.find(key);
+		if(it == ctx->s2_cache.end()){
+			pcr_ctx::S2Entry e; e.off_mask = 0;
+			ctx->s2_tmp.clear();
+			e.seedable = pcrhost::orientation_seeds(m, c.floor_, 0, ctx->s2_tmp, nullptr, S2_Q);
+			e.mask = pcrhost::mask_entry(m);
+			e.seeds.reserve(ctx->s2_tmp.size());
+			for(const pcrhost::Seed &sd : ctx->s2_tmp){ e.seeds.push_back((sd.code << 14) | ((uint32_t)sd.off << 9)); e.off_mask |= 1u << sd.off; }
+			it = ctx->s2_cache.emplace(key, std::move(e)).first;
+		}
+		const pcr_ctx::S2Entry &e = it->second;
 		L.s2_masks[o] = e.mask;
 		if(!e.seedable){ or_plain.push_back(o); continue; }
 		or_seed.push_back(o);
@@ -87,53 +58,39 @@
 			if(!fits(e.seeds.size(), 1) || L.s2_group_end.size() + 1 >= S2_MAX_GROUPS) return false;
 			L.s2_group_end.push_back((uint32_t)out.size()); L.s2_group_offmask.push_back(group_mask); L.s2_group_or.push_back(group_or0); L.s2_group_nor.push_back(group_last - group_or0 + 1);
 			group_begin = out.size(); group_mask = 0; group_or0 = o;
-			if(S3){ pf.push_back(pf_run); pf_run = 0; }
 		}
 		group_last = o;
 		const size_t at = out.size();
 		out.resize(at + e.seeds.size());
 		for(size_t k = 0;k < e.seeds.size();++k) out[at + k] = e.seeds[k] | (o - group_or0);
-		if(S3){
-			spans.insert(spans.end(), e3->spans.begin(), e3->spans.end());
-			pcr_ctx::S3Chunks *ch = nullptr;
-			for(pcr_ctx::S3Chunks &x : e3->chunks){ if(x.gen == S3->pix_generation){ ch = &x; break; } }
-			if(!ch){
-				ch = &e3->chunks[e3->next_slot]; e3->next_slot = (e3->next_slot + 1u) % pcr_ctx::S3_CHUNK_SETS;
-				ch->run.resize(e.seeds.size());
-				const uint32_t *const start = S3->pix_start_h.data();
-				uint32_t run = 0;
-				for(size_t k = 0;k < e.seeds.size();++k){
-					const uint32_t key4 = (e.seeds[k] >> 14) << 2, sp = e3->spans[k];
-					ch->run[k] = run; run += (start[key4 + (sp >> 2) + 1u] - start[key4 + (sp & 3u)] + 63u) >> 6;
-				}
-				ch->total = run; ch->gen = S3->pix_generation;
-			}
-			const size_t pa = pf.size();
-			pf.resize(pa + ch->run.size());
-			for(size_t k = 0;k < ch->run.size();++k) pf[pa + k] = pf_run + ch->run[k];
-			pf_run += ch->total;
-		}
 		if(!(o & 1u)){ irr_off_mask |= e.off_mask; group_mask |= e.off_mask; }
 	}
 	L.s2_group_end.push_back((uint32_t)out.size()); L.s2_group_offmask.push_back(group_mask); L.s2_group_or.push_back(group_or0);
 	L.s2_group_nor.push_back(or_seed.empty() ? 0u : group_last - group_or0 + 1);
-	if(S3) pf.push_back(pf_run);
 	return true;
 }
 
 constexpr size_t S3_LDS_BUDGET = 120*1024;
 constexpr uint32_t S3_WG_THREADS = 1024;
 uint32_t seed3_grid(const pcr_ctx *ctx) { return std::min<uint32_t>(2*ctx->n_cu, S3_MAX_WG); }
+inline size_t seed3_lds(uint32_t n_or, uint32_t slice_cap) { return 16*((size_t)n_or + slice_cap) + (((size_t)n_or + 15) & ~size_t(15)) + 16; }
 bool plan_seed3_slices(pcr_ctx *ctx, PlanLists &PL, bool with_irr)
 {
+	HostTimer timer(ctx, 8);
 	const uint32_t G_all = seed3_grid(ctx), seeds_per_turn = 16u*(S3_WG_THREADS/64);
 	PL.s3_launch.resize(PL.s2_group_end.size());
-	size_t g_begin = 0, g_prefix = 0;
+	size_t g_begin = 0, part = 0;
 	for(size_t g = 0;g < PL.s2_group_end.size();++g){
 		const uint32_t ns = PL.s2_group_end[g] - (uint32_t)g_begin;
 		g_begin = PL.s2_group_end[g];
-		const uint32_t *P = PL.s3_prefix.data() + g_prefix;
-		g_prefix += (size_t)ns + 1;
+		PL.s3_chunk0.resize((size_t)ns + 1);
+		uint32_t *const P = PL.s3_chunk0.data();
+		for(uint32_t at = 0;;++part){
+			const pcrhost::SeedPart &p = PL.s3_parts[part];
+			if(p.end){ P[at] = p.chunk0; ++part; break; }
+			for(uint32_t k = 0;k < p.n;++k) P[at + k] = p.src[k].chunk0 + p.chunk0;
+			at += p.n;
+		}
 		pcr_ctx::S3Launch &L = PL.s3_launch[g];
 		L.n_irr_wg = with_irr ? std::min<uint32_t>((ns + seeds_per_turn - 1u)/seeds_per_turn, G_all/4u) : 0u;
 		const uint32_t G = G_all - L.n_irr_wg;
@@ -147,7 +104,7 @@
 		}
 		for(uint32_t w = G + 1;w <= S3_MAX_WG;++w) L.W.start[w] = at;
 		for(uint32_t w = 0;w < G;++w) L.slice_cap = std::max(L.slice_cap, std::min(L.W.start[w + 1] + 2u, ns + 1u) - L.W.start[w]);
-		if(17*(size_t)PL.s2_group_nor[g] + 9*(size_t)L.slice_cap + 64 > S3_LDS_BUDGET) return false;
+		if(seed3_lds(PL.s2_group_nor[g], L.slice_cap) > S3_LDS_BUDGET) return false;
 	}
 	return true;
 }
@@ -404,6 +361,10 @@
 	}
 	bool use_seed2 = false;
 	if(seed2_ok){
+		if(want_seed3 && (ctx->s3_cache.full() || ctx->s3_cache.retired.size() > 1024)){
+			if((rc = flush_launcher(ctx)) != PCR_OK) return rc;
+			if(ctx->s3_cache.full()) ctx->s3_cache.clear(); else ctx->s3_cache.release_retired();
+		}
 		use_seed2 = plan_seed2(ctx, L, cand, or_seed, or_plain, P.irr_off_mask, want_seed3 ? &S : nullptr);
 		if(want_seed3 && !(use_seed2 && or_plain.empty() && !or_seed.empty() && plan_seed3_slices(ctx, L, P.s3_with_irr))){
 			or_seed.clear(); or_plain.clear();
@@ -413,8 +374,8 @@
 		if(!use_seed2){ or_seed.clear(); or_plain.clear(); P.irr_off_mask = 0; }
 	}
 	const bool use_seed3 = use_seed2 && want_seed3 && or_plain.empty() && !or_seed.empty()
-		&& L.s3_prefix.size() == L.s2_seeds.size() + L.s2_group_end.size() && L.s3_spans.size() == L.s2_seeds.size();
-	if(use_seed2){ P.form = use_seed3 ? ScanForm::Seed3 : ScanForm::Seed2; P.n_seeds = L.s2_seeds.size(); }
+		&& L.s3_listed;
+	if(use_seed2){ P.form = use_seed3 ? ScanForm::Seed3 : ScanForm::Seed2; P.n_seeds = use_seed3 ? L.s2_group_end.back() : L.s2_seeds.size(); }
 	else if(no_shifts && !ctx->host_seed_tables && n_or <= S1_MAX_OR){
 		plan_seed1(ctx, L, cand, or_seed, or_plain, P.irr_off_mask);
 		P.form = ScanForm::Seed1Dev; P.n_seeds = L.s1_seeds.size();
@@ -455,7 +416,7 @@
 struct StagedTables {
 	SeedTables ST = {};
 	Seed2Tables ST2 = {};
-	const uint32_t *d_s3_prefix = nullptr; const uint8_t *d_s3_spans = nullptr;
+	const uint4 *d_s3_recs = nullptr;
 	Scan2Staged plain, seedset;
 	bool lean = false, fuse = false;
 	size_t bits_bytes = 0;
@@ -510,7 +471,7 @@
 	bytes += (H.image.size() + H.heads.size() + H.multi.size() + 64)*sizeof(uint32_t);
 	if(seed2){
 		bytes += L.s2_masks.size()*sizeof(uint4) + L.s2_floors.size() + L.s2_seeds.size()*sizeof(uint32_t) + 512;
-		if(seed3) bytes += L.s3_prefix.size()*sizeof(uint32_t) + L.s3_spans.size() + 128;
+		if(seed3) bytes += L.s3_n_recs()*sizeof(pcrhost::SeedRec) + 128;
 	}
 	if(build_tables) bytes += L.s1_seeds.size()*sizeof(uint32_t) + 256;
 	T.bits_bytes = J.bits_bytes; T.fuse = J.fuse;
@@ -542,11 +503,16 @@
 		T.ST.image = ctx->s1_image.p; T.ST.heads = ctx->s1_heads.p; T.ST.multi = ctx->s1_multi.p; T.ST.flat = 1;
 	}
 	if(seed2){
-		T.ST2.seeds = st.put(L.s2_seeds.data(), L.s2_seeds.size());
-		T.ST2.masks = st.put(L.s2_masks.data(), L.s2_masks.size());
+		static_assert(sizeof(pcrhost::MaskEntry) == sizeof(uint4) && alignof(pcrhost::MaskEntry) == alignof(uint4) && sizeof(pcrhost::SeedRec) == sizeof(uint4), "the device reads both as uint4");
+		T.ST2.seeds = seed3 ? nullptr : st.put(L.s2_seeds.data(), L.s2_seeds.size());
+		T.ST2.masks = (const uint4 *)st.put(L.s2_masks.data(), L.s2_masks.size());
 		T.ST2.floors = st.put(L.s2_floors.data(), L.s2_floors.size());
-		T.ST2.n_seeds = (uint32_t)L.s2_seeds.size(); T.ST2.n_or = n_or;
-		if(seed3){ T.d_s3_prefix = st.put(L.s3_prefix.data(), L.s3_prefix.size()); T.d_s3_spans = st.put(L.s3_spans.data(), L.s3_spans.size()); }
+		T.ST2.n_seeds = seed3 ? L.s2_group_end.back() : (uint32_t)L.s2_seeds.size(); T.ST2.n_or = n_or;
+		if(seed3){
+			pcrhost::SeedRec *h_recs = nullptr;
+			T.d_s3_recs = (const uint4 *)st.alloc(L.s3_n_recs(), h_recs);
+			pcrhost::emit_seed_records(L.s3_parts, h_recs);
+		}
 	}
 	const size_t ctrl_bytes = (8 + 2*(size_t)S.n)*sizeof(uint32_t);
 	if(T.fuse){
@@ -600,16 +566,16 @@
 	return PCR_OK;
 }
 
-int launch_seed3_group(pcr_ctx *ctx, SeqSet &S, const Seed2Tables &Tg, const uint32_t *d_chunk_prefix, const uint8_t *d_spans, const pcr_ctx::S3Launch &L3, const IrrArgs2 &IA,
+int launch_seed3_group(pcr_ctx *ctx, SeqSet &S, const Seed2Tables &Tg, const uint4 *d_recs, const pcr_ctx::S3Launch &L3, const IrrArgs2 &IA,
 	const HitSink &sink, const S2Clear &Z)
 {
-	Seed3Tables T3; T3.seeds = Tg.seeds; T3.spans = d_spans; T3.chunk_prefix = d_chunk_prefix; T3.masks = Tg.masks; T3.floors = Tg.floors;
+	Seed3Tables T3; T3.recs = d_recs; T3.masks = Tg.masks; T3.floors = Tg.floors;
 	T3.n_seeds = Tg.n_seeds; T3.n_or = Tg.n_or; T3.or_base = Tg.or_base;
-	T3.pix_first = S.pix_first.p; T3.pix_last = S.pix_last.p; T3.pix_ent = S.pix_ent.p;
+	T3.pix_ent = S.pix_ent.p;
 	Seed3Set Q3 = { S.valid_d(), S.blk_info.p, S.blk_local.p, S.d_active.p };
 	T3.n_chunks = L3.n_chunks; T3.per_wg = L3.per_wg; T3.slice_cap = L3.slice_cap;
 	T3.n_irr_wg = IA.ix_first ? L3.n_irr_wg : 0u;
-	const size_t dyn3 = (size_t)Tg.n_or*sizeof(uint4) + 2*(size_t)T3.slice_cap*sizeof(uint32_t) + (((size_t)Tg.n_or + 15) & ~size_t(15)) + (((size_t)T3.slice_cap + 15) & ~size_t(15)) + 16;
+	const size_t dyn3 = seed3_lds(Tg.n_or, T3.slice_cap);
 	if(!ctx->s3_attr_set){
 		HIP_TRY(hipFuncSetAttribute((const void *)k_seed3<S3_WG_THREADS>, hipFuncAttributeMaxDynamicSharedMemorySize, 128*1024));
 		ctx->s3_attr_set = true;
@@ -636,16 +602,16 @@
 		for(size_t g = 0, b = 0;g < L.s2_group_end.size();++g){ if((size_t)L.s2_group_end[g] - b > (size_t)sgrid.x*S2_THREADS) irr_by_index = false; b = L.s2_group_end[g]; }
 		if(irr_by_index && (rc = irr_index_usable(ctx, S, irr_by_index)) != PCR_OK) return rc;
 	}
-	uint32_t g_begin = 0, g_prefix = 0;
+	uint32_t g_begin = 0;
 	bool first_launch = true;
 	for(size_t g = 0;g < L.s2_group_end.size();++g){
 		Seed2Tables Tg = T.ST2;
 		const uint32_t or0 = L.s2_group_or[g], g_or = L.s2_group_nor[g];
-		const uint8_t *const d_spans = seed3 ? T.d_s3_spans + g_begin : nullptr;
-		Tg.seeds = T.ST2.seeds + g_begin; Tg.n_seeds = L.s2_group_end[g] - g_begin;
+		const uint4 *const d_recs = seed3 ? T.d_s3_recs + g_begin + g : nullptr;
+		Tg.seeds = seed3 ? nullptr : T.ST2.seeds + g_begin; Tg.n_seeds = L.s2_group_end[g] - g_begin;
 		Tg.masks = T.ST2.masks + (size_t)or0; Tg.floors = T.ST2.floors + or0; Tg.n_or = g_or; Tg.or_base = or0;
 		g_begin = L.s2_group_end[g];
-		if(Tg.n_seeds == 0){ g_prefix += 1u; continue; }
+		if(Tg.n_seeds == 0) continue;
 		const size_t dyn = (size_t)g_or*sizeof(uint4) + (((size_t)g_or + 15) & ~size_t(15)) + 8*((size_t)Tg.n_seeds + 64) + 16;
 		IrrArgs2 IA; IA.scan = S.irr_scan.p; IA.irr = S.irr.p; IA.n_live = P.n_live;
 		IA.off_mask = L.s2_group_offmask[g];
@@ -665,8 +631,7 @@
 			Z.z0 = (uint4 *)fa->d_fr; Z.z1 = (uint4 *)fa->d_rf; Z.n0 = Z.n1 = (uint32_t)(T.bits_bytes/16); Z.ctrl = sink.counters;
 		}
 		if(seed3){
-			if((rc = launch_seed3_group(ctx, S, Tg, T.d_s3_prefix + g_prefix, d_spans, L.s3_launch[g], IA, sink, Z)) != PCR_OK) return rc;
-			g_prefix += Tg.n_seeds + 1u;
+			if((rc = launch_seed3_group(ctx, S, Tg, d_recs, L.s3_launch[g], IA, sink, Z)) != PCR_OK) return rc;
 		}
 		else hipLaunchKernelGGL(k_seed2_of_ctx, sgrid, sblock, dyn, ctx->stream, S.tb_d(), S.valid_d(), S.tile_desc.p, S.n_tiles, Tg, S.d_active.p, ctx->d_cand_fwd, ctx->d_cand_floor,
 			sink.ncand, IA, sink, ctx->s2_dbg, Z);
@@ -788,13 +753,16 @@
 	SeqSet &S = ctx->sets[J.which];
 	HostTimer timer(ctx, 0);
 	if(ctx->timing) ++ctx->n_timed;
+	HostTimer part(ctx, 6);
 	pcrhost::build_candidates((const uint64_t *)pairs, n_pairs, J.opt5 != 0, J.opt3 != 0, J.thr, J.cand);
 	const uint32_t ncand = (uint32_t)J.cand.size();
 	if(S.n == 0 || ncand == 0) return PCR_OK;
 	int rc;
+	part.next(7);
 	if((rc = choose_scan_form(ctx, S, J.cand, J.opt5, J.opt3, J.min_len, J.P, J.L)) != PCR_OK) return rc;
 	if(ctx->debug_log) fprintf(stderr, "[pcramp] scan plan: form=%s, %u candidates, %zu seeded orientations (%zu seeds), %zu plain, %u/%u IUPAC tiles, %u-slot buckets\n",
 		form_name(J.P.form), ncand, J.P.or_seed.size(), J.P.n_seeds, J.P.or_plain.size(), S.n_degen_tiles, S.n_tiles, S.bucket_cap);
+	part.next(9);
 	prepare_tables(S, J, J.has_fa ? &J.fa : nullptr);
 	return PCR_OK;
 }
@@ -830,6 +798,9 @@
 	if(ctx->best.generation != ctx->best_seen){
 		HIP_TRY(hipMemsetAsync(ctx->best.p, 0, ctx->best.cap*sizeof(uint32_t), ctx->stream));
 		ctx->best_seen = ctx->best.generation; ctx->epoch = std::min(ctx->debug_epoch, EPOCH_LIMIT);
+	}
+	if(P.form == ScanForm::Seed3 && (!S.pix_valid || J.L.s3_generation != S.pix_generation)){
+		g_err = "pcr_select_words: the position index changed between the planning and the launch of a pass"; return PCR_ERR_STATE;
 	}
 	StagedTables T;
 	if((rc = stage_tables(ctx, S, J, fa, async, ctrl_was_clean, T)) != PCR_OK) return rc;
@@ -1041,6 +1012,7 @@
 {
 	if(min_oligo_length < 1 || min_oligo_length > 32){ g_err = "pcr_select_words: min_oligo_length must be in [1,32]"; return PCR_ERR_ARG; }
 	int rc;
+	HostTimer rest(ctx, 10);
 	if(ctx->lq_client.poisoned.load(std::memory_order_acquire) && (rc = flush_launcher(ctx)) != PCR_OK) return rc;
 	HIP_TRY(hipSetDevice(ctx->device));
 	SeqSet &S = ctx->sets[which];
@@ -1052,7 +1024,9 @@
 		if((rc = flush_launcher(ctx)) != PCR_OK){ release_job(ctx, J); return rc; }
 		J->ctrl_was_clean = begin_pass(S); J->begun = true;
 	}
+	rest.next(11);
 	rc = plan_pass(ctx, *J, pairs, n_pairs);
+	rest.next(10);
 	if(rc == PCR_OK && !inline_pass && !pass_is_pipelinable(ctx, *J)){
 		inline_pass = true;
 		rc = flush_launcher(ctx);
@@ -1076,8 +1050,10 @@
 	}
 	assert(ctx->lq_client.queued.load() == 0);
 	const uint32_t seq0 = ctx->mail_seq;
+	rest.next(11);
 	rc = run_pass(ctx, *J, nullptr);
 	if(rc == PCR_OK && !J->fa.posted) rc = amplify_launch(ctx, S, pairs, n_pairs, args, d_bits_fr, d_bits_rf, &J->fa);
+	rest.next(10);
 	release_job(ctx, J);
 	if(rc != PCR_OK) return rc;
 	if(ctx->mail_seq != seq0){
```

Result: no change. 23.69 billion, median of 3 (+0.2%).
